# prime-slam/octreelib

Hardware: AMD Instinct MI355X
Metric: Mpoints/s insert+subdivide+RANSAC (higher is better)
Workload: dtype f64; 1 GPU; BASELINE config 3: Grid 1 m voxels, 10000000 planar points per GPU (scene 32x32x32 voxels), insert + subdivide(len>64) + map_leaf_points_cuda_ransac(H=1024, k=6, thr=0.01, poses_per_batch=10) incl. apply_mask; points_per_gpu=10000000, K=64, hypotheses=1024, leaves=575543

## Files before the change

### include/octreelib_hip.h

```cpp
#ifndef OCTREELIB_HIP_H
#define OCTREELIB_HIP_H

#include <stdint.h>

#ifdef __cplusplus
extern "C" {
#endif

#define OCTL_ABI_VERSION 1

enum {
  OCTL_OK = 0,
  OCTL_E_INVALID = -1,
  OCTL_E_HIP = -2,
  OCTL_E_NOMEM = -3,
  OCTL_E_DOMAIN = -4,
  OCTL_E_DEPTH = -5,
  OCTL_E_STATE = -6,
  OCTL_E_COMM = -7
};

typedef struct octl_ctx octl_ctx;
typedef struct octl_forest octl_forest;

// ... 145 lines not shown
                                           const double origin[3], int32_t min_points, double max_variance,
                                           double max_distance, double huber_delta, double* sys_dev,
                                           int64_t* counts_dev, int32_t* node_dev, int32_t* row_dev,
                                           double* residual_dev);
int octl_forest_point_registration_system(octl_forest* f, const double* xyz, int64_t n, const double T[12],
                                          const double origin[3], double max_distance, double huber_delta,
                                          const uint8_t* slot_sel, int32_t n_sel, double sys[28], int64_t counts[2],
                                          int32_t* slot, int64_t* index, double* distance2);
int octl_forest_point_registration_system_device(octl_forest* f, const double* xyz_dev, int64_t n, const double T[12],
                                                 const double origin[3], double max_distance, double huber_delta,
                                                 const uint8_t* slot_sel, int32_t n_sel, double* sys_dev,
                                                 int64_t* counts_dev, int32_t* slot_dev, int64_t* index_dev,
                                                 double* distance2_dev);
int octl_forest_nearest_plane_registration_system(octl_forest* f, const double* xyz, int64_t n, const double T[12],
                                                  const double origin[3], double max_distance, double huber_delta,
                                                  const uint8_t* slot_sel, int32_t n_sel, int32_t min_points,
                                                  double max_variance, double sys[28], int64_t counts[2],
                                                  int32_t* slot, int64_t* index, double* distance2, int32_t* node,
                                                  int32_t* row, double* residual);
int octl_forest_nearest_plane_registration_system_device(octl_forest* f, const double* xyz_dev, int64_t n,
                                                         const double T[12], const double origin[3],
                                                         double max_distance, double huber_delta,
                                                         const uint8_t* slot_sel, int32_t n_sel, int32_t min_points,
                                                         double max_variance, double* sys_dev, int64_t* counts_dev,
                                                         int32_t* slot_dev, int64_t* index_dev, double* distance2_dev,
                                                         int32_t* node_dev, int32_t* row_dev, double* residual_dev);
int octl_forest_adjustment_system(octl_forest* f, const uint8_t* slot_sel, int32_t n_sel, const double* transforms,
                                  const double origin[3], int32_t min_points, int32_t min_poses, double max_variance,
                                  double* sums, int64_t* counts, int64_t n_leaves[2]);
int octl_forest_adjustment_tables(octl_forest* f, int64_t cap_leaves, int32_t* node, int64_t* count, double* mean,
                                  double* normal, double* lambda0, uint8_t* used, int64_t* n_leaves,
                                  int64_t cap_blocks, int32_t* blk_node, int32_t* blk_slot, double* blk_moments,
                                  int64_t* n_blocks);
int octl_forest_transform_poses(octl_forest* f, const uint8_t* slot_sel, int32_t n_sel, const double* transforms);
int octl_forest_remove_poses(octl_forest* f, const uint8_t* slot_sel, int32_t n_sel, int32_t* new_slot,
                             int64_t* n_removed);
int octl_forest_store_size(octl_forest* f, int64_t* n_store, int64_t* n_alive, int32_t* n_poses);
typedef struct {
  int64_t nodes_before, nodes_after, voxels_before, voxels_after, internal_after, collapsed;
} octl_prune_info;
int octl_forest_prune(octl_forest* f, int64_t cap_nodes, int32_t* node_map, int32_t* old_node, octl_prune_info* info);
int octl_debug_sym3_eigen(octl_ctx* ctx, const double* cov6, int64_t n, double* eigval, double* eigvec);


int octl_forest_ransac(octl_forest* f, const int32_t* block_order, int64_t nb,
                       const double* hypotheses, int32_t H, int32_t k, double threshold,
                       float* plane, int32_t* best_count, int32_t* best_index);
int octl_forest_reference_order(octl_forest* f, const int32_t* e0, int32_t n_e0, int64_t cap,
                                int32_t* order, int64_t* n_blocks);
int octl_forest_ransac_all(octl_forest* f, int32_t poses_per_batch, const int32_t* e0,
                           int32_t n_e0, const double* hypotheses, int32_t H, int32_t k,
                           double threshold);
int octl_forest_get_mask(octl_forest* f, int64_t cap, uint8_t* mask, int64_t* n);
int octl_forest_apply_mask(octl_forest* f, int64_t* n_alive);
int octl_forest_apply_mask_async(octl_forest* f);
int octl_forest_settle(octl_forest* f, int64_t* n_alive);
int octl_forest_filter_count(octl_forest* f, const uint8_t* slot_sel, int32_t n_sel, int64_t lo,
                             int64_t hi, int64_t* n_alive);
int octl_forest_apply_host_mask(octl_forest* f, const uint8_t* mask, int64_t n,
                                int64_t* n_alive);


int octl_ransac_evaluate(octl_ctx* ctx, const double* point_cloud, int64_t M,
                         const int32_t* block_sizes, int64_t B, const double* hypotheses,
                         int32_t H, int32_t k, double threshold, uint8_t* mask_out,
                         float* planes_out, int32_t* best_count_out, int32_t* best_index_out);


int32_t octl_voxel_owner(int64_t qx, int64_t qy, int64_t qz, int32_t n_ranks);
#define OCTL_UNIQUE_ID_BYTES 128
int octl_comm_unique_id(uint8_t id[OCTL_UNIQUE_ID_BYTES]);
int octl_comm_init(octl_ctx* ctx, int32_t n_ranks, int32_t rank,
                   const uint8_t id[OCTL_UNIQUE_ID_BYTES]);
int octl_comm_destroy(octl_ctx* ctx);
int octl_route_points(octl_ctx* ctx, const double* xyz_dev, const int64_t* gidx_dev,
                      int64_t n, int64_t index_base, const double corner[3], double L,
                      int64_t* n_recv, int64_t* send_counts );
int octl_forest_add_pose_routed(octl_forest* f, int32_t* slot);
int octl_forest_add_pose_routed_from(octl_forest* f, octl_ctx* route_ctx, int32_t* slot);
int octl_route_get_gidx(octl_ctx* ctx, int64_t cap, int64_t* gidx, int64_t* n);
int octl_debug_host_syncs(uint64_t* count);
int octl_debug_launches(uint64_t* count);
int octl_debug_spec_finish(uint64_t* held, uint64_t* missed);

int octl_debug_route_partition(octl_ctx* ctx, const double* xyz, int64_t n, int64_t index_base,
                               double L, int32_t n_ranks, int64_t* counts, double* xyz_out,
                               int64_t* gidx_out);
int octl_comm_allreduce_i64(octl_ctx* ctx, int64_t* inout_host, int32_t n);

int octl_dev_alloc(octl_ctx* ctx, int64_t bytes, void** dptr);
int octl_dev_free(octl_ctx* ctx, void* dptr);
int octl_dev_upload(octl_ctx* ctx, void* dptr, const void* src, int64_t bytes);
int octl_dev_download(octl_ctx* ctx, void* dst, const void* dptr, int64_t bytes);
int octl_host_alloc(octl_ctx* ctx, int64_t bytes, void** p);
int octl_host_free(octl_ctx* ctx, void* p);
int octl_dev_upload_async(octl_ctx* ctx, void* dptr, const void* src, int64_t bytes);
int octl_ctx_sync_uploads(octl_ctx* ctx);
int octl_dev_copy_bandwidth(octl_ctx* ctx, int64_t bytes, int iters, double* bytes_per_s);

int octl_debug_fail_alloc(int64_t nth, int64_t* seen);

int octl_comm_info(octl_ctx* ctx, int32_t* n_ranks, int32_t* user_rank, int32_t* version);
int octl_device_identity(octl_ctx* ctx, char pci_bus_id[32], uint8_t uuid[16], int32_t* cus);

int octl_debug_set_option(octl_ctx* ctx, const char* name, int64_t value);

int octl_debug_key_geometry(const int32_t tb[6], uint64_t want, int64_t n_alive, uint32_t target, int32_t margin,
                            int32_t bb_out[6], uint32_t* width, uint32_t* n_buckets, int32_t* valid,
                            int64_t* mismatches);

int octl_debug_exclusive_scan(octl_ctx* ctx, const uint32_t* in, int64_t n, uint32_t* out,
                              uint32_t* total);
int octl_debug_radix_sort(octl_ctx* ctx, uint64_t* keys, uint32_t* vals, int64_t n,
                          int key_bits);
int octl_debug_plane_arith(octl_ctx* ctx, const double* num3, const double* den, const double* c,
                           int32_t kdiv, int64_t n, double* q3, double* ck, double* sq);
int octl_debug_plane_arith_certified(octl_ctx* ctx, const double* num3, const double* den, const double* c,
                                     int32_t kdiv, int64_t n, double* q3, double* ck, double* sq);

#ifdef __cplusplus
}
#endif
#endif
```

### octreelib_amd/_native.py

```python

import ctypes as C
import os
import threading

import numpy as np

_LIB_PATH = os.environ.get(
    "OCTREELIB_AMD_LIB",
    os.path.join(os.path.dirname(os.path.abspath(__file__)), "lib", "liboctree_hip.so"),
)

OCTL_OK = 0
OCTL_E_INVALID = -1
OCTL_E_HIP = -2
OCTL_E_NOMEM = -3
OCTL_E_DOMAIN = -4
OCTL_E_DEPTH = -5
OCTL_E_STATE = -6
OCTL_E_COMM = -7
UNIQUE_ID_BYTES = 128


class NativeLibraryError(RuntimeError):
    """liboctree_hip.so is missing / not loadable, or no HIP device is visible."""
# ... 58 lines not shown
    "octl_forest_build": (C.c_int, [_p, _i64, _p, _i32, _i32, _i32, C.POINTER(BuildInfo)]),
    "octl_forest_build_planar": (C.c_int, [_p, _i64, _f64, _i32, _i32, _p, _i32, _i32, C.POINTER(BuildInfo)]),
    "octl_forest_get_split_stats": (C.c_int, [_p, _i64, _p, _p, _pi64]),
    "octl_forest_set_scheme": (C.c_int, [_p, _p, _p, _i64, _i32]),
    "octl_forest_get_nodes": (C.c_int, [_p, _i64, _p, _p, _p, _p, _p, _p, _p, _pi64]),
    "octl_forest_get_voxels": (C.c_int, [_p, _i64, _p, _pi64]),
    "octl_forest_get_blocks": (C.c_int, [_p, _i64, _p, _p, _p, _p, _pi64]),
    "octl_forest_get_slot_voxels": (C.c_int, [_p, _i32, _i64, _p, _pi64]),
    "octl_forest_slot_counts": (C.c_int, [_p, _i32, _pi64, _pi64]),
    "octl_forest_internal_per_voxel": (C.c_int, [_p, _i64, _p, _pi64]),
    "octl_forest_get_perm": (C.c_int, [_p, _i64, _p, _pi64]),
    "octl_forest_get_points": (C.c_int, [_p, _i64, _i64, _p]),
    "octl_forest_gather_blocks": (C.c_int, [_p, _p, _i64, _i64, _p, _pi64]),
    "octl_forest_leaf_stats": (C.c_int, [_p, _p, _i64, _p, _p, _p, _p, _p]),
    "octl_forest_pooled_leaf_stats": (C.c_int, [_p, _p, _i32, _i64, _p, _p, _p, _p, _p, _p, _pi64]),
    "octl_forest_locate": (C.c_int, [_p, _p, _i64, _p]),
    "octl_forest_locate_device": (C.c_int, [_p, _p, _i64, _p]),
    "octl_forest_point_to_plane": (C.c_int, [_p, _p, _i64, _i32, _f64, _p, _p, _p]),
    "octl_forest_point_to_plane_device": (C.c_int, [_p, _p, _i64, _i32, _f64, _p, _p, _p]),
    "octl_forest_nearest": (C.c_int, [_p, _p, _i64, _i32, _f64, _p, _i32, _p, _p, _p, _p]),
    "octl_forest_nearest_device": (C.c_int, [_p, _p, _i64, _i32, _f64, _p, _i32, _p, _p, _p, _p]),
    "octl_forest_raycast": (C.c_int, [_p, _p, _p, _p, _p, _i64, _p, _i32, _i32, _i32, _f64, _p, _p, _p]),
    "octl_forest_raycast_device": (C.c_int, [_p, _p, _p, _p, _p, _i64, _p, _i32, _i32, _i32, _f64, _p, _p, _p]),
    "octl_forest_ray_evidence": (C.c_int, [_p, _p, _p, _p, _p, _p, _i64, _i64, _p, _p, _pi64]),
    "octl_forest_ray_evidence_device": (C.c_int, [_p, _p, _p, _p, _p, _p, _i64, _p, _p, _i64]),
    "octl_forest_carve": (C.c_int, [_p, _p, _p, _i64, _p, _i32, _i64, _i64, _pi64]),
    "octl_forest_carve_device": (C.c_int, [_p, _p, _p, _i64, _p, _i32, _i64, _i64, _pi64]),
    "octl_forest_radius_count": (C.c_int, [_p, _p, _i64, _f64, _i32, _p, _i32, _p]),
    "octl_forest_radius_count_device": (C.c_int, [_p, _p, _i64, _f64, _i32, _p, _i32, _p]),
    "octl_forest_remove_sparse": (C.c_int, [_p, _f64, _i32, _p, _i32, _p, _i32, _pi64]),
    "octl_forest_cell_count": (C.c_int, [_p, _p, _i64, _f64, _i32, _p, _i32, _p]),
    "octl_forest_cell_count_device": (C.c_int, [_p, _p, _i64, _f64, _i32, _p, _i32, _p]),
    "octl_forest_thin": (C.c_int, [_p, _f64, _i32, _p, _i32, _p, _i32, _pi64]),
    "octl_forest_neighbourhood_stats": (C.c_int, [_p, _p, _i64, _f64, _p, _i32, _p, _p, _p, _p, _p]),
    "octl_forest_neighbourhood_stats_device": (C.c_int, [_p, _p, _i64, _f64, _p, _i32, _p, _p, _p, _p, _p]),
    "octl_forest_point_stats": (C.c_int, [_p, _f64, _p, _i32, _p, _i32, _i64, _pi64, _p, _p, _p, _p, _p, _p, _p]),
    "octl_forest_plane_segments": (C.c_int, [_p, _p, _i32, _i32, _f64, _f64, _f64, _i64, _i64, _p, _p, _p, _p, _p, _p,
                                             _p, _p, _p, _pi64, _pi64]),
    "octl_forest_registration_system": (C.c_int, [_p, _p, _i64, _p, _p, _i32, _f64, _f64, _f64, _p, _p, _p, _p, _p]),
    "octl_forest_registration_system_device": (C.c_int,
                                               [_p, _p, _i64, _p, _p, _i32, _f64, _f64, _f64, _p, _p, _p, _p, _p]),
    "octl_forest_point_registration_system": (C.c_int,
                                              [_p, _p, _i64, _p, _p, _f64, _f64, _p, _i32, _p, _p, _p, _p, _p]),
    "octl_forest_point_registration_system_device": (C.c_int,
                                                     [_p, _p, _i64, _p, _p, _f64, _f64, _p, _i32, _p, _p, _p, _p, _p]),
    "octl_forest_nearest_plane_registration_system": (C.c_int,
                                                      [_p, _p, _i64, _p, _p, _f64, _f64, _p, _i32, _i32, _f64, _p, _p,
                                                       _p, _p, _p, _p, _p, _p]),
    "octl_forest_nearest_plane_registration_system_device": (C.c_int,
                                                             [_p, _p, _i64, _p, _p, _f64, _f64, _p, _i32, _i32, _f64,
                                                              _p, _p, _p, _p, _p, _p, _p, _p]),
    "octl_forest_adjustment_system": (C.c_int, [_p, _p, _i32, _p, _p, _i32, _i32, _f64, _p, _p, _p]),
    "octl_forest_adjustment_tables": (C.c_int, [_p, _i64, _p, _p, _p, _p, _p, _p, _pi64, _i64, _p, _p, _p, _pi64]),
    "octl_forest_transform_poses": (C.c_int, [_p, _p, _i32, _p]),
    "octl_forest_remove_poses": (C.c_int, [_p, _p, _i32, _p, _pi64]),
    "octl_forest_store_size": (C.c_int, [_p, _pi64, _pi64, _pi32]),
    "octl_forest_prune": (C.c_int, [_p, _i64, _p, _p, _p]),
    "octl_forest_ransac": (C.c_int, [_p, _p, _i64, _p, _i32, _i32, _f64, _p, _p, _p]),
    "octl_forest_reference_order": (C.c_int, [_p, _p, _i32, _i64, _p, _pi64]),
    "octl_forest_ransac_all": (C.c_int, [_p, _i32, _p, _i32, _p, _i32, _i32, _f64]),
    "octl_forest_get_mask": (C.c_int, [_p, _i64, _p, _pi64]),
    "octl_forest_apply_mask": (C.c_int, [_p, _pi64]),
    "octl_forest_apply_mask_async": (C.c_int, [_p]),
    "octl_forest_settle": (C.c_int, [_p, _pi64]),
    "octl_forest_apply_host_mask": (C.c_int, [_p, _p, _i64, _pi64]),
    "octl_forest_filter_count": (C.c_int, [_p, _p, _i32, _i64, _i64, _pi64]),
    "octl_ransac_evaluate": (
        C.c_int,
        [_p, _p, _i64, _p, _i64, _p, _i32, _i32, _f64, _p, _p, _p, _p],
    ),
    "octl_voxel_owner": (_i32, [_i64, _i64, _i64, _i32]),
    "octl_comm_unique_id": (C.c_int, [_p]),
    "octl_comm_init": (C.c_int, [_p, _i32, _i32, _p]),
    "octl_comm_destroy": (C.c_int, [_p]),
    "octl_comm_info": (C.c_int, [_p, _pi32, _pi32, _pi32]),
    "octl_device_identity": (C.c_int, [_p, C.c_char_p, _p, _pi32]),
    "octl_route_points": (C.c_int, [_p, _p, _p, _i64, _i64, _p, _f64, _pi64, _p]),
    "octl_forest_add_pose_routed": (C.c_int, [_p, _pi32]),
    "octl_forest_add_pose_routed_from": (C.c_int, [_p, _p, _pi32]),
    "octl_debug_route_partition": (C.c_int, [_p, _p, _i64, _i64, C.c_double, C.c_int32, _p, _p, _p]),
    "octl_debug_host_syncs": (C.c_int, [C.POINTER(C.c_uint64)]),
    "octl_debug_launches": (C.c_int, [C.POINTER(C.c_uint64)]),
    "octl_debug_spec_finish": (C.c_int, [C.POINTER(C.c_uint64), C.POINTER(C.c_uint64)]),
    "octl_debug_fail_alloc": (C.c_int, [_i64, _pi64]),
    "octl_debug_set_option": (C.c_int, [_p, C.c_char_p, _i64]),
    "octl_debug_key_geometry": (C.c_int, [_p, C.c_uint64, _i64, C.c_uint32, _i32, _p, _p, _p, _p, _p]),
    "octl_route_get_gidx": (C.c_int, [_p, _i64, _p, _pi64]),
    "octl_comm_allreduce_i64": (C.c_int, [_p, _p, _i32]),
    "octl_dev_alloc": (C.c_int, [_p, _i64, C.POINTER(_p)]),
    "octl_dev_free": (C.c_int, [_p, _p]),
    "octl_dev_upload": (C.c_int, [_p, _p, _p, _i64]),
    "octl_dev_download": (C.c_int, [_p, _p, _p, _i64]),
    "octl_host_alloc": (C.c_int, [_p, _i64, C.POINTER(_p)]),
    "octl_host_free": (C.c_int, [_p, _p]),
    "octl_dev_upload_async": (C.c_int, [_p, _p, _p, _i64]),
    "octl_ctx_sync_uploads": (C.c_int, [_p]),
    "octl_dev_copy_bandwidth": (C.c_int, [_p, _i64, C.c_int, C.POINTER(_f64)]),
    "octl_debug_exclusive_scan": (C.c_int, [_p, _p, _i64, _p, _p]),
    "octl_debug_radix_sort": (C.c_int, [_p, _p, _p, _i64, C.c_int]),
    "octl_debug_plane_arith": (C.c_int, [_p, _p, _p, _p, C.c_int32, _i64, _p, _p, _p]),
    "octl_debug_plane_arith_certified": (C.c_int, [_p, _p, _p, _p, C.c_int32, _i64, _p, _p, _p]),
    "octl_debug_sym3_eigen": (C.c_int, [_p, _p, _i64, _p, _p]),
}

_lib = None
_lib_lock = threading.Lock()


def lib_path() -> str:
    return _LIB_PATH


def load():
    global _lib
    with _lib_lock:
        if _lib is not None:
            return _lib
        if not os.path.exists(_LIB_PATH):
            raise NativeLibraryError(
                f"{_LIB_PATH} is missing: build it with `make` (or __graft_entry__.build()). "
                "octreelib_amd has no CPU fallback."
            )
        try:
            lib = C.CDLL(_LIB_PATH)
        except OSError as e:
            raise NativeLibraryError(f"cannot load {_LIB_PATH}: {e}") from e
        for name, (res, args) in SIGNATURES.items():
            fn = getattr(lib, name)
            fn.restype = res
            fn.argtypes = args
        _lib = lib
        return lib


def ptr(a):
    if a is None:
        return None
    return a.ctypes.data_as(C.c_void_p)


class Context:

    def __init__(self, device: int = 0):
        self.lib = load()
        n = C.c_int(0)
        self.lib.octl_device_count(C.byref(n))
        if n.value <= 0:
            raise NativeLibraryError(
                "no HIP device is visible: octreelib_amd runs on an MI355X only (no CPU fallback)"
            )
        h = C.c_void_p()
        rc = self.lib.octl_ctx_create(int(device), C.byref(h))
        if rc != OCTL_OK or not h.value:
            raise NativeLibraryError(f"octl_ctx_create(device={device}) failed with code {rc}")
        self.handle = h
        self.device = int(device)

    def check(self, rc: int):
        if rc == OCTL_OK:
            return
        msg = self.lib.octl_last_error(self.handle)
        msg = msg.decode("utf-8", "replace") if msg else f"error {rc}"
        if rc == OCTL_E_INVALID:
            raise ValueError(msg)
        if rc == OCTL_E_NOMEM:
            raise MemoryError(msg)
        if rc == OCTL_E_DOMAIN:
            raise DomainError(msg)
        if rc == OCTL_E_DEPTH:
            raise RecursionError(msg)
        raise RuntimeError(msg)

    def sync(self):
        self.check(self.lib.octl_ctx_sync(self.handle))

    def set_option(self, name: str, value=1):
        v = 0 if value is None or value is False else int(value)
        self.check(self.lib.octl_debug_set_option(self.handle, name.encode(), v))
        touched = self.__dict__.setdefault("_options_touched", set())
        touched.add(name)

    def reset_options(self):
        for name in list(self.__dict__.get("_options_touched", ())):
            self.lib.octl_debug_set_option(self.handle, name.encode(), 0)
        self.__dict__["_options_touched"] = set()

    def set_profiling(self, enabled: bool):
        self.check(self.lib.octl_ctx_set_profiling(self.handle, int(enabled)))

    def timings(self):
        cap, stride = 64, 48
        names = C.create_string_buffer(cap * stride)
        ms = (C.c_float * cap)()
        launches = (C.c_int64 * cap)()
        n = C.c_int(0)
        self.check(
            self.lib.octl_ctx_get_timings(
                self.handle, C.cast(names, C.c_void_p), stride, C.cast(ms, C.c_void_p),
                C.cast(launches, C.c_void_p), cap, C.byref(n),
            )
        )
        out = {}
        for i in range(min(n.value, cap)):
            name = names.raw[i * stride : (i + 1) * stride].split(b"\0", 1)[0].decode()
            out[name] = (float(ms[i]), int(launches[i]))
        return out

    def close(self):
        if getattr(self, "handle", None) is not None and self.handle.value:
            self.lib.octl_ctx_destroy(self.handle)
            self.handle = C.c_void_p()

    def __del__(self):
        try:
            self.close()
        except Exception:
            pass


_default_ctx = {}


def default_device() -> int:
    for var in ("OCTREELIB_AMD_DEVICE", "LOCAL_RANK"):
        v = os.environ.get(var)
        if v is not None and v.strip().lstrip("-").isdigit():
            return int(v)
    return 0


_thread_ctx = threading.local()


class use_context:

    def __init__(self, ctx: Context):
        self.ctx = ctx

    def __enter__(self):
        self._prev = getattr(_thread_ctx, "ctx", None)
        _thread_ctx.ctx = self.ctx
        return self.ctx

    def __exit__(self, *exc):
        _thread_ctx.ctx = self._prev


def get_context(device=None) -> Context:
    if device is None:
        ctx = getattr(_thread_ctx, "ctx", None)
        if ctx is not None:
            return ctx
    device = default_device() if device is None else int(device)
    ctx = _default_ctx.get(device)
    if ctx is None:
        ctx = Context(device)
        _default_ctx[device] = ctx
    return ctx


def as_points(points) -> np.ndarray:
    a = np.ascontiguousarray(np.asarray(points, dtype=np.float64))
    if a.size == 0:
        return a.reshape(0, 3)
    if a.ndim != 2 or a.shape[1] != 3:
        raise ValueError(f"expected an (n, 3) point cloud, got shape {a.shape}")
    return a
# ... 12 lines not shown
```

### octreelib_amd/csrc/api.hip

```cpp
#include <unordered_map>

#include "forest.h"

namespace {

__global__ __launch_bounds__(256) void k_slot_counts(const int32_t* __restrict__ blk_slot,
                                                     const int32_t* __restrict__ blk_size, int64_t nb,
                                                     int32_t slot, unsigned long long* __restrict__ out) {
  __shared__ unsigned long long part[2][4];
  unsigned long long pts = 0, lv = 0;
  for (int64_t b = (int64_t)blockIdx.x * blockDim.x + threadIdx.x; b < nb; b += (int64_t)gridDim.x * blockDim.x) {
    if (blk_slot[b] == slot) {
      pts += (unsigned long long)blk_size[b];
      lv += 1;
    }
  }
#pragma unroll
  for (int off = 32; off > 0; off >>= 1) {
    pts += __shfl_xor(pts, off);
    lv += __shfl_xor(lv, off);
  }
  if ((threadIdx.x & 63) == 0) {
    part[0][threadIdx.x >> 6] = pts;
    part[1][threadIdx.x >> 6] = lv;
// ... 35 lines not shown
}


__global__ __launch_bounds__(256) void k_gather_sizes(const int32_t* __restrict__ ids, int64_t m,
                                                      const int32_t* __restrict__ blk_size, uint32_t* __restrict__ out) {
  const int64_t i = (int64_t)blockIdx.x * blockDim.x + threadIdx.x;
  if (i < m) out[i] = (uint32_t)blk_size[ids[i]];
}
__global__ __launch_bounds__(256) void k_gather_rows(const int32_t* __restrict__ ids, int64_t m,
                                                     const uint32_t* __restrict__ blk_start,
                                                     const int32_t* __restrict__ blk_size,
                                                     const uint32_t* __restrict__ offs, const double* __restrict__ xyz,
                                                     double* __restrict__ out) {
  const int64_t i = (int64_t)blockIdx.x * 4 + (threadIdx.x >> 6);
  if (i >= m) return;
  const int32_t b = ids[i];
  const double* src = xyz + 3 * (size_t)blk_start[b];
  double* dst = out + 3 * (size_t)offs[i];
  const int n3 = 3 * blk_size[b];
  for (int j = threadIdx.x & 63; j < n3; j += 64) dst[j] = src[j];
}

}

void forest_reset_scheme(octl_forest* f) {
  forest_forget_pending(f);
  f->max_block_hint = INT64_MAX;
  f->displaced_rows = false;
  f->store_dirty = true;
  f->nodes[0].n = f->nodes[1].n = 0;
  f->cur = 0;
  f->epoch = 0;
  f->built = false;
  f->vkeys.clear();
  f->vkeys_stale = false;
  f->vorg_set = false;
  f->vcode_valid = false;
  f->fast_order_valid = false;
  f->built_store = 0;
  f->built_poses = 0;
  f->append_only = true;
  f->n_voxels = 0;
  f->level_segs.clear();
  f->n_internal = 0;
  f->max_depth_reached = 0;
  f->n_ord = 0;
  f->n_blocks = 0;
  f->mask_valid = false;
  f->split_stats_valid = false;
  forest_contents_changed(f);
}

extern "C" {

int octl_forest_create(octl_ctx* ctx, int mode, const double corner[3], double edge,
                       octl_forest** out) {
  if (!ctx || !out || !corner) return OCTL_E_INVALID;
  *out = nullptr;
  if (mode != 0 && mode != 1) return octl_set_error(ctx, OCTL_E_INVALID, "mode must be 0 or 1");
  if (!(edge > 0.0)) return octl_set_error(ctx, OCTL_E_INVALID, "edge length must be positive");
  if (mode == 0) {
    if (corner[0] != 0.0 || corner[1] != 0.0 || corner[2] != 0.0)
      return octl_set_error(ctx, OCTL_E_INVALID,
                            "a non-zero grid corner is outside the parity domain: the reference "
                            "places its octrees relative to the corner but subtracts absolute "
                            "points (grid.py:96-105 vs octree.py:74)");
    if (edge != (double)(int64_t)edge)
      return octl_set_error(ctx, OCTL_E_INVALID,
                            "voxel_edge_length must be integer valued: the reference truncates "
                            "voxel coordinates with astype(int) (grid.py:72-76)");
  }
  octl_forest* f = new octl_forest();
  f->ctx = ctx;
  f->mode = mode;
  for (int a = 0; a < 3; ++a) f->corner[a] = corner[a];
  f->edge = edge;
  *out = f;
  return OCTL_OK;
}

void octl_forest_destroy(octl_forest* f) {
  if (!f) return;
  forest_forget_pending(f);
  (void)hipSetDevice(f->ctx->device);
  (void)hipStreamSynchronize(f->ctx->stream);
  nodes_free(f->ctx, f->nodes[0]);
  nodes_free(f->ctx, f->nodes[1]);
  if (f->store_borrowed) {
    f->xyz = f->xyz_own;
    f->xyz_own = DevBuf{};
    f->store_borrowed = false;
  }
  for (DevBuf* b :
       {&f->bbox_dev, &f->part_xyz[0], &f->part_xyz[1], &f->bk_table, &f->bk_tot, &f->bk_chunks, &f->bk_vox, &f->bk_node, &f->leafinfo,
        &f->xyz, &f->alive, &f->alive2, &f->ord_idx, &f->xyz_ord, &f->pos_node, &f->blk_node, &f->blk_slot,
        &f->blk_start, &f->blk_size, &f->blk_node2, &f->blk_slot2, &f->blk_start2, &f->blk_size2, &f->mask, &f->blk_eval, &f->rs_scratch, &f->rs_order, &f->fast_order,
        &f->rs_hyp, &f->rs_plane, &f->rs_count, &f->rs_index, &f->ord_idx2, &f->xyz_ord2,
        &f->vkey, &f->path, &f->lin[0], &f->lin[1], &f->val[0], &f->val[1],
        &f->hist, &f->idxbuf[0], &f->idxbuf[1], &f->pathbuf[0], &f->pathbuf[1], &f->flags,
        &f->entries, &f->split[0], &f->split[1], &f->split_tiles[0], &f->split_tiles[1],
        &f->child_sc, &f->pose_off_dev, &f->scheme_dev, &f->root_up, &f->vlin_dev, &f->vcode_dev[0],
        &f->vcode_dev[1], &f->split_lambda, &f->split_n, &f->pl_rows, &f->pl_plane, &f->pl_node_row, &f->grp_scratch,
        &f->pl_hist, &f->q_stage, &f->rg_rows, &f->adj_tab, &f->adj_call, &f->nn_tab, &f->seg_tab, &f->seg_out,
        &f->seg_sort, &f->xf_tab})
    devbuf_release(f->ctx, *b);
  delete f;
}

int octl_forest_clear(octl_forest* f) {
  if (!f) return OCTL_E_INVALID;
  f->bbox_stale = true;
  f->alive_stale = false;
  if (f->store_borrowed) {
    f->xyz = f->xyz_own;
    f->xyz_own = DevBuf{};
    f->store_borrowed = false;
  }
  f->bbox_pending = false;
  f->pose_off.assign(1, 0);
  f->n_store = f->n_alive = 0;
  forest_reset_scheme(f);
  return OCTL_OK;
}

static void forest_drop_scheme(octl_forest* f) {
  f->built = false;
  f->n_ord = 0;
  f->n_blocks = 0;
  f->n_internal = 0;
  f->mask_valid = false;
  f->store_dirty = true;
  f->split_stats_valid = false;
  forest_contents_changed(f);
}

int octl_forest_build(octl_forest* f, int64_t K, const uint8_t* scheme_mask, int32_t n_mask,
                      int32_t keep_scheme, int32_t max_depth, octl_build_info* info) {
  if (!f) return OCTL_E_INVALID;
  OCTL_TRY(forest_settle(f));
  const int64_t nodes_before = f->built ? f->nodes[f->cur].n : -1, voxels_before = f->n_voxels;
  const int rc = forest_build(f, K, scheme_mask, n_mask, keep_scheme, max_depth, info);
  if (rc != OCTL_OK && rc != OCTL_E_INVALID && rc != OCTL_E_STATE) forest_drop_scheme(f);
  if (rc == OCTL_OK && (!keep_scheme || f->nodes[f->cur].n != nodes_before || f->n_voxels != voxels_before))
    f->split_stats_valid = false;
  return rc;
}

int octl_forest_build_planar(octl_forest* f, int64_t K, double max_variance, int32_t min_points, int32_t ddof,
                             const uint8_t* scheme_mask, int32_t n_mask, int32_t max_depth, octl_build_info* info) {
  if (!f) return OCTL_E_INVALID;
  OCTL_TRY(forest_settle(f));
  octl_ctx* ctx = f->ctx;
  if (!(max_variance > 0.0) || !(max_variance <= 1.7976931348623157e308))
    return octl_set_error(ctx, OCTL_E_INVALID, "build_planar: max_variance must be finite and > 0 (got %g)",
                          max_variance);
  if (min_points < 4)
    return octl_set_error(ctx, OCTL_E_INVALID, "build_planar: min_points must be >= 4 (got %d)", min_points);
  if (ddof != 0 && ddof != 1)
    return octl_set_error(ctx, OCTL_E_INVALID, "build_planar: ddof must be 0 or 1 (got %d)", ddof);
  const PlanarRule rule{max_variance, min_points, ddof};
  f->split_stats_valid = false;
  const int rc = forest_build(f, K, scheme_mask, n_mask, 0, max_depth, info, &rule);
  if (rc != OCTL_OK && rc != OCTL_E_INVALID && rc != OCTL_E_STATE) forest_drop_scheme(f);
  return rc;
}

// ... 609 lines not shown
```

### octreelib_amd/csrc/bucket_build.hip

```cpp
#include "build_common.h"
#include "ref_arith.h"
#include "lookback.h"
#include "wave_utils.h"

namespace {

constexpr int PT_THREADS = 256;
constexpr int PT_BITS = 12;
constexpr int PT_BINS = 1 << PT_BITS;

constexpr int BB_THREADS = 512;
constexpr int BB_IPT = 8;
constexpr int BB_WGS = 4;
#define BB_LEAF_UNROLL 2
#define BB_KEEP_ROUNDS 7
constexpr int BB_KEEP = BB_KEEP_ROUNDS < BB_IPT ? BB_KEEP_ROUNDS : BB_IPT;
constexpr int BB_CAP = BB_THREADS * BB_IPT;
static_assert(BB_CAP == 4096, "leaf words, 16-bit item ids and the chunk plan assume 4096 points per piece");
constexpr int BB_LEVELS = 7;
constexpr uint32_t PATH_MASK = 0x1FFFFFu;

enum { BK_NVOX = 0, BK_NINT = 1 , BK_NBLK = 8, BK_ROWS = 9 };
constexpr int LC_DIGIT = 16, LC_DEPTH = 19;
constexpr uint32_t LI_VHEAD = 1u << 24;
// ... 1962 lines not shown
#pragma unroll
      for (int off = 1; off < 64; off <<= 1) {
        const uint32_t t = __shfl_up(inc, off);
        if (tid >= off) inc += t;
      }
      s_hc[tid] = inc - v;
      if (tid == 63) s_hc[64] = inc;
    }
    __syncthreads();
#pragma unroll 2
    for (int r = 0; r < FR; ++r) {
      const int f = r * 256 + tid;
      if (r * 256 >= n) break;
      const unsigned long long bal = s_bal[r * 4 + wave];
      const bool bhead = ((bal >> lane) & 1ull) != 0ull;
      uint32_t size = 0;
      if (bhead) {
        int q = r * 4 + wave;
        unsigned long long rest = bal & ~lt & ~(1ull << lane);
        while (rest == 0ull && ++q < FR * 4) rest = s_bal[q];
        const int next = rest ? q * 64 + (__ffsll((long long)rest) - 1) : n;
        size = (uint32_t)(next - f);
      }
      if (f < n && (bhead || P.write_pos))
        emit(f, leafinfo[(size_t)start + f], bhead, s_hc[r * 4 + wave] + (uint32_t)__popcll(bal & lt), size);
    }
    brun = s_hc[64];
  } else {
    uint32_t open_blk = ~0u, open_pos = 0;
    for (int f0 = 0; f0 < n; f0 += 256) {
      const int f = f0 + tid;
      const uint32_t li = f < n ? leafinfo[(size_t)start + f] : 0u;
      const bool bhead = f < n && (li & LI_BHEAD);
      uint32_t tot;
      const uint32_t pre = block_excl_add(bhead ? 1u : 0u, &tot, s_scr);
      if (bhead) s_hp[pre] = (uint32_t)f;
      if (f < n && (bhead || P.write_pos)) emit(f, li, bhead, brun + pre, ~0u);
      __syncthreads();
      if (tot > 0) {
        if (bhead && pre + 1 < tot) blk_size[bbase + brun + pre] = (int32_t)(s_hp[pre + 1] - (uint32_t)f);
        if (tid == 0 && open_blk != ~0u) blk_size[bbase + open_blk] = (int32_t)(s_hp[0] - open_pos);
        open_blk = brun + tot - 1;
        open_pos = s_hp[tot - 1];
      }
      __syncthreads();
      brun += tot;
    }
    if (tid == 0 && open_blk != ~0u) blk_size[bbase + open_blk] = (int32_t)((uint32_t)n - open_pos);
  }
  BB_STAMP(7);
  if (want_order) {
    __syncthreads();
    for (uint32_t j = tid; j < brun; j += 256) {
      const uint32_t key = s_bkey[j], vox = key >> 13;
      uint32_t lo = j;
      while (lo > 0 && (s_bkey[lo - 1] >> 13) == vox) --lo;
      uint32_t rk = lo;
      for (uint32_t i = lo; i < brun && (s_bkey[i] >> 13) == vox; ++i) rk += s_bkey[i] < key ? 1u : 0u;
      P.order_out[bbase + rk] = (int32_t)(bbase + j);
    }
  }
  BB_STAMP(8);
  pre_vox += nvox;
  pre_blk += cko.y ? nblk_piece : brun;
#pragma unroll
  for (int l = 0; l < BB_LEVELS; ++l) pre_lvl[l] += lvl_cnt[l];
  __syncthreads();
  }
}

#define OCTL_PT_IPT 8
#define OCTL_PT_WGS 2
constexpr int PT_IPT = OCTL_PT_IPT;
constexpr int PT_TILE = PT_THREADS * PT_IPT;

int domain_error(octl_ctx* ctx) {
  return octl_set_error(ctx, OCTL_E_DOMAIN,
                        "a point has a non-finite coordinate or a top-level voxel index outside +-%d", OCTL_VOX_ABS_LIMIT);
}
uint32_t supertiles(octl_ctx* ctx, int64_t items, int wgs, int* tiles) {
  *tiles = (int)std::min<int64_t>(16, std::max<int64_t>(1, ceil_div(ceil_div(items, PT_TILE), (int64_t)octl_ctx_cus(ctx) * wgs)));
  return (uint32_t)ceil_div(items, (int64_t)*tiles * PT_TILE);
}
int part_table_reserve(octl_forest* f, size_t cells, size_t tail_words, size_t* elems) {
  *elems = (cells + 1 + 15) & ~(size_t)15;
  return devbuf_reserve(f->ctx, f->bk_table, (2 * *elems + tail_words + 16) * 4);
}
bool tables_fused(const octl_ctx* ctx, uint32_t nst) { return !ctx->opt.no_fused_tables && nst <= TS_MAX_ROWS; }

struct PartPass {
  const PartRec* recs = nullptr;
  int64_t n = 0;
  const uint8_t* alive = nullptr;
  const uint8_t* scheme = nullptr;
  LinParams lp;
  GeomDev* gdev = nullptr;
  int validate = 0;
  const GeomAsk* ask = nullptr;
  int32_t* bad_flag = nullptr;
  uint32_t nst = 0, nd = 0;
  int tiles = 1;
  size_t tab_elems = 0;
  bool own_scan = false;
  PartRec* out = nullptr;
  const char *t_hist = nullptr, *t_scan = nullptr, *t_scatter = nullptr;
};

hipError_t transpose_u32(hipStream_t st, const uint32_t* in, uint32_t R, uint32_t Cc, uint32_t* out) {
  OCTL_LAUNCH(k_transpose_u32, dim3((Cc + 63) / 64, (R + 63) / 64), dim3(256), 0, st, in, R, Cc, out);
  return hipGetLastError();
}

int partition_scan(octl_forest* f, const PartPass& p, bool fused) {
  octl_ctx* ctx = f->ctx;
  uint32_t *table = f->bk_table.as<uint32_t>(), *table_dm = table + p.tab_elems;
  if (fused) {
    const unsigned g = (p.nd + TS_COLS - 1) / TS_COLS;
    uint64_t* status = nullptr;
    uint32_t epoch = 0;
    OCTL_TRY(octl_scan_status_acquire(ctx, g, &status, &epoch));
    OCTL_LAUNCH(k_table_scan, dim3(g), dim3(TS_THREADS), 0, ctx->stream, table, p.nst, p.nd, table_dm, status, epoch,
                       p.validate, p.ask ? (const int32_t*)f->bbox_dev.as<int32_t>() : (const int32_t*)nullptr,
                       p.ask ? *p.ask : GeomAsk{0, 0, 0, 0}, p.lp, p.gdev);
    HIP_TRY(ctx, hipGetLastError());
  } else {
    HIP_TRY(ctx, transpose_u32(ctx->stream, table, p.nst, p.nd, table_dm));
    OCTL_TRY(octl_exclusive_scan_u32(ctx, table_dm, table_dm, (int64_t)p.nd * p.nst, nullptr));
    HIP_TRY(ctx, transpose_u32(ctx->stream, table_dm, p.nd, p.nst, table));
  }
  return OCTL_OK;
}

int partition_pass(octl_forest* f, const PartPass& p, const uint32_t** bstart, uint32_t* bstride) {
  octl_ctx* ctx = f->ctx;
  hipStream_t st = ctx->stream;
  const uint32_t nst = p.nst, nd = p.nd;
  const bool fused = tables_fused(ctx, nst);
  uint32_t *table = f->bk_table.as<uint32_t>(), *table_dm = table + p.tab_elems;
  const int32_t* bbox = p.ask ? (const int32_t*)f->bbox_dev.as<int32_t>() : nullptr;
  {
    KTimer t(ctx, p.t_hist);
    if (p.recs) {
      OCTL_LAUNCH(k_part_hist_rec, dim3(nst), dim3(PH_THREADS), 0, st, (const uint4*)p.recs, p.n, p.lp,
                         (const GeomDev*)p.gdev, nst, nd, (int64_t)p.tiles * PT_TILE, table);
    } else {
      const bool lone = f->edge == 1.0;
      auto kh = p.validate ? (lone ? k_part_hist<true, true> : k_part_hist<true, false>)
                           : (lone ? k_part_hist<false, true> : k_part_hist<false, false>);
      OCTL_LAUNCH(kh, dim3(nst), dim3(PH_THREADS), 0, st, (const double*)f->xyz.as<double>(), p.alive, p.n, p.lp,
                         (const GeomDev*)p.gdev, nst, nd, (int64_t)p.tiles * PT_TILE, table,
                         p.validate ? f->bbox_dev.as<int32_t>() : p.bad_flag);
    }
    HIP_TRY(ctx, hipGetLastError());
    if (p.validate) {
      f->bbox_pending = false;
      if (fused) {
      } else if (p.validate == 1)
        OCTL_LAUNCH(k_geom_validate, dim3(1), dim3(64), 0, st, bbox, *p.ask, p.lp, p.gdev);
      else
        OCTL_LAUNCH(k_geom_validate2, dim3(1), dim3(64), 0, st, bbox, *p.ask, p.gdev);
      HIP_TRY(ctx, hipGetLastError());
    }
    if (!p.t_scan) OCTL_TRY(partition_scan(f, p, fused));
  }
  if (p.t_scan && !p.own_scan) {
    KTimer t(ctx, p.t_scan);
    OCTL_TRY(partition_scan(f, p, fused));
  }
  {
    KTimer t(ctx, p.t_scatter);
    ScatterOwnScan own;
    std::memset(&own, 0, sizeof(own));
    if (p.own_scan) own = ScatterOwnScan{table_dm, p.validate, bbox, *p.ask, p.lp, p.gdev};
    if (!p.recs) {
      auto ks = p.own_scan ? k_part_scatter<PT_IPT, false, 8, true>
                           : (nd <= 256u ? k_part_scatter<PT_IPT, false, 8> : k_part_scatter<PT_IPT, false, PT_BITS>);
      OCTL_LAUNCH(ks, dim3(nst), dim3(PT_THREADS), 0, st, (const double*)f->xyz.as<double>(), p.alive, p.n, p.lp,
                         (const GeomDev*)p.gdev, nst, nd, p.tiles, (const uint32_t*)table,
                         (const int64_t*)f->pose_off_dev.as<int64_t>(), (int)f->pose_off.size() - 1, p.scheme, p.out, own);
    } else {
      auto ks = nd <= 256u ? k_part_scatter<PT_IPT, true, 8> : k_part_scatter<PT_IPT, true, PT_BITS>;
      OCTL_LAUNCH(ks, dim3(nst), dim3(PT_THREADS), 0, st, (const double*)p.recs, (const uint8_t*)nullptr, p.n, p.lp,
                         (const GeomDev*)p.gdev, nst, nd, p.tiles, (const uint32_t*)table, (const int64_t*)nullptr, 0,
                         (const uint8_t*)nullptr, p.out, own);
    }
    HIP_TRY(ctx, hipGetLastError());
  }
  *bstart = table_dm;
  *bstride = fused ? 1u : nst;
  return OCTL_OK;
}

enum BuildVerdict { BV_GO, BV_GENERAL, BV_AGAIN_ASYNC, BV_AGAIN_HOST };

struct BucketBuild {
  octl_forest* f;
  octl_ctx* ctx;
  hipStream_t st;
  uint32_t* small;
  GeomAsk ask;
  bool async_geom;
  bool hinted;
  bool hinted2;
  GeomDev hint;
  int bb[6], tb[6];
  uint64_t ny, nz;
  int s, bits_a;
  uint32_t nb, nd_a, nd_b, nst_a, nst_b;
  int tiles_a, tiles_b;
  bool two_pass;
  LinParams lp, lp_pass1;
  size_t tab_elems;
  GeomDev* gdev;
  const PartRec* recs;
  const uint32_t* bstart;
  uint32_t bstride;
  uint32_t *bk_tot, *bk_scan, *ck_tot;
  ChunkDesc* ck_desc;
  uint2* ck_of_bucket;
  BkParams bp;
  NodeParams np;
  bool chunks_beside;
  bool spec_want, spec_own_scan, spec_order, spec_launched;
  int64_t spec_node_cap, spec_vox_cap, spec_blk_cap;
  uint32_t sm[64];
};
int mirror_words(const BucketBuild& b) {
  static_assert(SM_GEOM == 64, "the geometry record is read back together with the 64 scalars in front of it");
  return (int)(64 + (b.gdev ? sizeof(GeomDev) / 4 : 0));
}

bool hint_load(const octl_ctx* ctx, const octl_forest* f, uint64_t want, GeomDev* hint) {
  std::memcpy(hint, ctx->geom_hint, sizeof(*hint));
  return ctx->geom_hint_valid && ctx->geom_hint_want == want && hint->lp.mode == f->mode && hint->lp.L == f->edge &&
         hint->lp.c0x == f->corner[0] && hint->lp.c0y == f->corner[1] && hint->lp.c0z == f->corner[2] &&
         !ctx->opt.no_geom_hint && hint->lp.exact_digits == (ctx->opt.no_exact_digits ? 0 : 1);
}
void hint_store(octl_ctx* ctx, const GeomDev& g, bool two_pass, uint64_t want) {
  static_assert(sizeof(GeomDev) <= sizeof(octl_ctx::geom_hint), "hint storage");
  std::memset(ctx->geom_hint, 0, sizeof(ctx->geom_hint));
  std::memcpy(ctx->geom_hint, &g, sizeof(g));
  ctx->geom_hint_valid = g.valid != 0;
  ctx->geom_hint_two_pass = two_pass;
  ctx->geom_hint_want = want;
}
int geom_read(octl_ctx* ctx, GeomDev* g, BuildVerdict* v) {
  std::memcpy(g, static_cast<char*>(ctx->small_host) + SM_GEOM * 4, sizeof(*g));
  *v = BV_GO;
  if (g->valid) return OCTL_OK;
  if (g->reason == GEOM_DOMAIN) return domain_error(ctx);
  *v = g->reason == GEOM_EMPTY ? BV_GENERAL : (g->reason == GEOM_REHASH ? BV_AGAIN_ASYNC : BV_AGAIN_HOST);
  return OCTL_OK;
}

int plan_geometry(BucketBuild& b, bool force_sync, BuildVerdict* v) {
  octl_forest* f = b.f;
  octl_ctx* ctx = b.ctx;
  const int64_t n_alive = f->n_alive;
  *v = BV_GO;
  const uint64_t target = ctx->opt.bucket_points > 0 ? (uint64_t)ctx->opt.bucket_points
                                                     : (n_alive <= 400000 ? 1280 : 2560);
  uint64_t want = 1;
  while (want < ((uint64_t)PT_BINS << PT_BITS) && want * target < (uint64_t)n_alive) want <<= 1;
  b.async_geom = !force_sync && !ctx->geom_sparse && want <= (uint64_t)PT_BINS && !ctx->opt.sync_geom;
  const int margin = f->mode != 0 ? 0
                                  : (ctx->opt.geom_margin == 0 ? 1 : (int)std::min<int64_t>(64, std::max<int64_t>(0, ctx->opt.geom_margin)));
  b.ask = GeomAsk{want, n_alive, (uint32_t)target, margin};
  if (f->bbox_pending) {
    const bool usable = hint_load(ctx, f, want, &b.hint);
    b.hinted = b.async_geom && usable && !ctx->geom_hint_two_pass;
    b.hinted2 = !b.async_geom && !force_sync && usable && ctx->geom_hint_two_pass && f->mode == 0;
    if (!b.hinted && !b.hinted2) OCTL_TRY(store_compute_bbox(f));
  }
  if (f->n_alive != f->n_store) OCTL_TRY(alive_ensure(f));
  b.ny = b.nz = 1;
  b.nb = b.async_geom ? (uint32_t)geom_bucket_cap(want) : (uint32_t)PT_BINS;
  if (!b.async_geom) {
    int *bb = b.bb, *tb = b.tb;
    *v = BV_GENERAL;
    if (b.hinted2) {
      std::memcpy(bb, b.hint.bb, sizeof(b.bb));
      std::memcpy(tb, b.hint.tb, sizeof(b.tb));
    } else {
      int32_t* bbox_host = reinterpret_cast<int32_t*>(static_cast<char*>(ctx->small_host) + MIRROR_BBOX_WORD * 4);
      HIP_TRY(ctx, hipMemcpyAsync(bbox_host, f->bbox_dev.p, 32, hipMemcpyDeviceToHost, b.st));
      HIP_TRY(ctx, hipStreamSynchronize(b.st));
      std::memcpy(tb, bbox_host, sizeof(b.tb));
      if (bbox_host[6]) return domain_error(ctx);
      if (tb[0] > tb[3]) return OCTL_OK;
      geom_pad_box(tb, margin, bb);
    }
    if (bb[0] > bb[3]) return OCTL_OK;
    const uint64_t nx = (uint64_t)(bb[3] - bb[0] + 1);
    b.ny = (uint64_t)(bb[4] - bb[1] + 1);
    b.nz = (uint64_t)(bb[5] - bb[2] + 1);
    if (nx * b.ny > (1ull << 32) || nx * b.ny * b.nz >= (1ull << 32)) return OCTL_OK;
    const uint64_t R = nx * b.ny * b.nz;
    const uint64_t Rt = (uint64_t)((int64_t)tb[3] - tb[0] + 1) * (uint64_t)((int64_t)tb[4] - tb[1] + 1) *
                        (uint64_t)((int64_t)tb[5] - tb[2] + 1);
    b.s = std::min(12, std::max(0, geom_ceil_log2(Rt) - geom_ceil_log2(want)));
    if (((R - 1) >> b.s) + 1 > ((uint64_t)PT_BINS << PT_BITS)) return OCTL_OK;
    b.nb = (uint32_t)(((R - 1) >> b.s) + 1);
    b.two_pass = b.nb > (uint32_t)PT_BINS;
    if (b.hinted2 && !b.two_pass) {
      *v = BV_AGAIN_HOST;
      return OCTL_OK;
    }
    ctx->geom_sparse = ((Rt - 1) >> b.s) + 1 > (uint64_t)PT_BINS && want <= (uint64_t)PT_BINS;
    if (b.two_pass && (uint64_t)f->n_alive * 2 < (uint64_t)b.nb * target) return OCTL_OK;
    *v = BV_GO;
  }
  const int wgs = b.two_pass ? std::max(OCTL_PT_WGS, 3) : OCTL_PT_WGS;
  b.nst_a = supertiles(ctx, f->n_store, wgs, &b.tiles_a);
  b.nst_b = b.two_pass ? supertiles(ctx, n_alive, wgs, &b.tiles_b) : 0;
  b.bits_a = b.two_pass ? std::min(PT_BITS, (geom_ceil_log2(b.nb) + 1) / 2) : 0;
  b.nd_a = b.two_pass ? (1u << b.bits_a) : b.nb;
  b.nd_b = b.two_pass ? ((b.nb - 1) >> b.bits_a) + 1 : 0;
  LinParams& lp = b.lp;
  lp.mode = f->mode, lp.L = f->edge;
  lp.c0x = f->corner[0], lp.c0y = f->corner[1], lp.c0z = f->corner[2];
  lp.minx = b.bb[0], lp.miny = b.bb[1], lp.minz = b.bb[2];
  lp.ny = (uint32_t)b.ny, lp.nz = (uint32_t)b.nz;
  lp.shift = lp.dshift = b.s;
  lp.dmask = b.two_pass ? (b.nd_a - 1u) : 0xFFFFFFFFu, lp.raw_vp = b.two_pass ? 1 : 0;
  lp.exact_digits = ctx->opt.no_exact_digits ? 0 : 1;
  lp.width = 1u << b.s;
  lp.winv = lp.whalf = 0.0;
  b.lp_pass1 = lp;
  return OCTL_OK;
}

int partition(BucketBuild& b, const BucketBuildArgs& a) {
  octl_forest* f = b.f;
  octl_ctx* ctx = b.ctx;
  const int64_t n_alive = f->n_alive;
  OCTL_TRY(devbuf_reserve(ctx, f->part_xyz[0], (size_t)n_alive * sizeof(PartRec)));
  if (b.two_pass) OCTL_TRY(devbuf_reserve(ctx, f->part_xyz[1], (size_t)n_alive * sizeof(PartRec)));
  OCTL_TRY(part_table_reserve(f, std::max((size_t)b.nd_a * b.nst_a, (size_t)b.nd_b * b.nst_b),
                              b.two_pass ? b.nb + 1 : 0, &b.tab_elems));
  const size_t tot_elems = (((size_t)BK_ROWS * b.nb + 8) + 15) & ~(size_t)15;
  OCTL_TRY(devbuf_reserve(ctx, f->bk_tot, 2 * tot_elems * 4));
  const std::pair<DevBuf*, int> per_point[] = {
      {&f->bk_vox, 12},  {&f->bk_node, 12}, {&f->leafinfo, 4}, {&f->ord_idx, 4},   {&f->xyz_ord, 24},
      {&f->pos_node, 4}, {&f->blk_node, 4}, {&f->blk_slot, 4}, {&f->blk_start, 4}, {&f->blk_size, 4}};
  for (const auto& pp : per_point) OCTL_TRY(devbuf_reserve(ctx, *pp.first, (size_t)n_alive * pp.second));
  b.bk_tot = f->bk_tot.as<uint32_t>();
  b.bk_scan = b.bk_tot + tot_elems;
  if (b.async_geom || b.hinted2) b.gdev = reinterpret_cast<GeomDev*>(b.small + SM_GEOM);
  if (b.async_geom) {
    if (b.hinted) {
      if (!ctx->geom_hint_staged) OCTL_LAUNCH(k_geom_set, dim3(1), dim3(64), 0, b.st, b.hint, b.gdev);
    } else {
      OCTL_LAUNCH(k_bucket_geom, dim3(1), dim3(64), 0, b.st, (const int32_t*)f->bbox_dev.as<int32_t>(), b.ask, b.lp,
                         b.gdev);
    }
    HIP_TRY(ctx, hipGetLastError());
  } else if (b.hinted2) {
    GeomDev g2;
    std::memset(&g2, 0, sizeof(g2));
    g2.lp = b.lp_pass1;
    std::memcpy(g2.bb, b.bb, sizeof(b.bb));
    std::memcpy(g2.tb, b.tb, sizeof(b.tb));
    g2.valid = 1;
    OCTL_LAUNCH(k_geom_set, dim3(1), dim3(64), 0, b.st, g2, b.gdev);
    HIP_TRY(ctx, hipGetLastError());
  }
  PartPass p;
  p.n = f->n_store;
  p.alive = f->n_alive == f->n_store ? nullptr : f->alive.as<uint8_t>();
  p.scheme = a.scheme_dev;
  p.lp = b.lp, p.gdev = b.gdev, p.ask = &b.ask;
  p.validate = b.hinted ? 1 : (b.hinted2 ? 2 : 0);
  p.nst = b.nst_a, p.nd = b.nd_a, p.tiles = b.tiles_a, p.tab_elems = b.tab_elems;
  p.own_scan = tables_fused(ctx, b.nst_a) && !b.two_pass && !b.hinted2 && b.nd_a <= 256u && b.nst_a <= PS_OWN_MAX_ROWS;
  p.out = f->part_xyz[0].as<PartRec>();
  p.t_hist = "part_hist", p.t_scan = "part_scan", p.t_scatter = "part_scatter";
  OCTL_TRY(partition_pass(f, p, &b.bstart, &b.bstride));
  b.recs = p.out;
  if (!b.two_pass) return OCTL_OK;
  b.lp.dshift = b.s + b.bits_a, b.lp.dmask = 0xFFFFFFFFu, b.lp.raw_vp = 0;
  p.recs = b.recs, p.n = n_alive;
  p.alive = p.scheme = nullptr;
  p.lp = b.lp;
  p.validate = 0, p.own_scan = false;
  p.nst = b.nst_b, p.nd = b.nd_b, p.tiles = b.tiles_b;
  p.out = f->part_xyz[1].as<PartRec>();
  OCTL_TRY(partition_pass(f, p, &b.bstart, &b.bstride));
  uint32_t* bounds = f->bk_table.as<uint32_t>() + 2 * b.tab_elems;
  KTimer t(ctx, "bucket_bounds");
  OCTL_LAUNCH(k_bucket_bounds, dim3((unsigned)ceil_div((int64_t)b.nb + 1, 256)), dim3(256), 0, b.st,
                     (const uint4*)f->part_xyz[1].as<uint4>(), (uint32_t)n_alive, b.lp, (const GeomDev*)b.gdev, b.nb, bounds);
  HIP_TRY(ctx, hipGetLastError());
  b.recs = p.out, b.bstart = bounds, b.bstride = 1;
  return OCTL_OK;
}

int launch_chunks(BucketBuild& b, hipStream_t on) {
  octl_forest* f = b.f;
  OCTL_LAUNCH(k_bucket_plan, dim3(b.nb), dim3(BB_THREADS), 0, on, b.recs, b.bstart, b.bp, (const GeomDev*)b.gdev,
                     b.ck_desc, b.ck_of_bucket, b.bk_tot, b.small);
  HIP_TRY(b.ctx, hipGetLastError());
  OCTL_LAUNCH(k_bucket_chunks, dim3((unsigned)std::min<int64_t>(2 * (int64_t)octl_ctx_cus(b.ctx), CK_CAP)),
                     dim3(BB_THREADS), 0, on, b.recs, b.bstart, b.bp, (const GeomDev*)b.gdev,
                     (const ChunkDesc*)b.ck_desc, b.ck_tot, (const int64_t*)f->pose_off_dev.as<int64_t>(),
                     f->ord_idx.as<uint32_t>(), f->xyz_ord.as<double>(), f->leafinfo.as<uint32_t>(),
                     f->bk_vox.as<uint32_t>(), f->bk_node.as<uint32_t>(), b.bk_tot, b.small);
  HIP_TRY(b.ctx, hipGetLastError());
  return OCTL_OK;
}

int build_buckets(BucketBuild& b, const BucketBuildArgs& a) {
  octl_forest* f = b.f;
  octl_ctx* ctx = b.ctx;
  b.bp = BkParams{b.lp, a.K, b.bstride, b.nb, (uint32_t)f->n_alive, (int)f->pose_off.size() - 1, a.scheme_dev ? 0 : 1};
  const size_t ck_off_tot = (size_t)CK_CAP * sizeof(ChunkDesc);
  const size_t ck_off_bkt = ck_off_tot + (size_t)CK_CAP * BK_ROWS * 4;
  OCTL_TRY(devbuf_reserve(ctx, f->bk_chunks, ck_off_bkt + (size_t)b.nb * 8 + 16));
  b.ck_desc = reinterpret_cast<ChunkDesc*>(f->bk_chunks.p);
  b.ck_tot = reinterpret_cast<uint32_t*>(static_cast<char*>(f->bk_chunks.p) + ck_off_tot);
  b.ck_of_bucket = reinterpret_cast<uint2*>(static_cast<char*>(f->bk_chunks.p) + ck_off_bkt);
  b.chunks_beside = ctx->had_chunks;
  {
    KTimer t(ctx, "bucket_build");
    hipStream_t side = b.st;
    bool on_side = false;
    if (b.chunks_beside && octl_ctx_side_stream(ctx) && hipEventRecord(ctx->self_gate, b.st) == hipSuccess &&
        hipStreamWaitEvent(ctx->self_stream, ctx->self_gate, 0) == hipSuccess) {
      side = ctx->self_stream;
      on_side = true;
    }
    if (b.chunks_beside) OCTL_TRY(launch_chunks(b, side));
    OCTL_LAUNCH(k_bucket_build, dim3(b.nb), dim3(BB_THREADS), 0, b.st, b.recs, b.bstart, b.bp, (const GeomDev*)b.gdev,
                       (const int64_t*)f->pose_off_dev.as<int64_t>(), f->ord_idx.as<uint32_t>(), f->xyz_ord.as<double>(),
                       f->leafinfo.as<uint32_t>(), f->bk_vox.as<uint32_t>(), f->bk_node.as<uint32_t>(), b.bk_tot, b.small,
                       b.chunks_beside ? 0 : 1);
    HIP_TRY(ctx, hipGetLastError());
    if (on_side) {
      HIP_TRY(ctx, hipEventRecord(ctx->self_done, side));
      HIP_TRY(ctx, hipStreamWaitEvent(b.st, ctx->self_done, 0));
    }
  }
  NodeParams& np = b.np;
  np.lp = b.lp;
  np.bstride = b.bstride, np.nb = b.nb, np.n_alive = (uint32_t)f->n_alive;
  np.n_poses = b.bp.n_poses, np.all_scheme = b.bp.all_scheme, np.cur_epoch = a.cur_epoch;
  np.old_fc = a.old_fc, np.old_epoch = a.old_epoch, np.old_vcode = a.old_vcode, np.old_voxels = a.old_voxels;
  b.spec_order = np.n_poses == 1 && !ctx->opt.no_fast_order;
  b.spec_want = b.async_geom && b.gdev && !a.old_fc && !a.old_vcode && ctx->spec_nodes > 0 && !ctx->opt.no_spec_finish;
  b.spec_own_scan = b.spec_want && !ctx->opt.no_fused_tables && (uint32_t)BK_ROWS * b.nb <= (uint32_t)BF_SCAN_MAX;
  return OCTL_OK;
}

int launch_finish(const BucketBuild& b, NodeTable& nt, const NodeParams& np, bool with_chunk_map, uint32_t own_scan_seq) {
  octl_forest* f = b.f;
  KTimer t(b.ctx, "bucket_nodes");
  const size_t lds = own_scan_seq ? ((size_t)BK_ROWS * b.nb + 1) * 4 : 0;
  auto kern = own_scan_seq ? k_bucket_finish<true> : k_bucket_finish<false>;
  OCTL_LAUNCH(kern, dim3(b.nb), dim3(256), lds, b.st, node_ptrs(nt), np, b.bstart,
                     (const uint32_t*)b.bk_scan, (const uint32_t*)(b.small + SM_BK_TOTAL),
                     (const uint32_t*)f->leafinfo.as<uint32_t>(), (const uint32_t*)f->ord_idx.as<uint32_t>(),
// ... 73 lines not shown
    std::memset(&g, 0, sizeof(g));
    g.lp = b.lp_pass1;
    geom_pad_box(b.tb, b.ask.margin, g.bb);
    std::memcpy(g.tb, b.tb, sizeof(b.tb));
    g.valid = 1;
    hint_store(ctx, g, true, b.ask.want);
  }
  if (b.async_geom) {
    OCTL_TRY(geom_read(ctx, &g, v));
    if (*v != BV_GO) return OCTL_OK;
    GeomDev nh;
    geom_from_box(g.tb, false, b.ask, b.lp, nh);
    hint_store(ctx, nh, false, b.ask.want);
    b.lp = g.lp;
    std::memcpy(b.bb, g.bb, sizeof(b.bb));
    std::memcpy(b.tb, g.tb, sizeof(b.tb));
    b.ny = b.lp.ny, b.nz = b.lp.nz;
  }
  return OCTL_OK;
}

int finish_and_commit(BucketBuild& b, const BucketBuildArgs& a, NodeTable& nt, bool overfull, BucketBuildResult* r) {
  octl_forest* f = b.f;
  octl_ctx* ctx = b.ctx;
  const uint32_t* sm = b.sm;
  if (sm[SM_BK_FLAGS]) return OCTL_OK;
  const int64_t V = sm[SM_NVOX];
  int64_t n_int = 0;
  int depth = 0;
  r->segs.assign(1, octl_forest::LevelSeg{0, V, 0});
  for (int l = 0; l < BB_LEVELS; ++l) {
    if (sm[SM_BK_LEVEL + l] == 0) break;
    n_int += sm[SM_BK_LEVEL + l];
    depth = l + 1;
    r->segs.push_back(octl_forest::LevelSeg{V + 8 * (n_int - (int64_t)sm[SM_BK_LEVEL + l]), V + 8 * n_int, l + 1});
  }
  if (depth > a.max_depth) return octl_set_error(ctx, OCTL_E_DEPTH, "maximum depth %d exceeded", a.max_depth);
  const int64_t total = V + 8 * n_int;
  if (total >= ((int64_t)1 << 31)) return octl_set_error(ctx, OCTL_E_NOMEM, "more than 2^31 scheme nodes");
  const bool fast_order = b.np.n_poses == 1 && !a.old_fc && sm[SM_BK_TODO] == 0 && sm[SM_BK_NOORDER] == 0 &&
                          !ctx->opt.no_fast_order;
  const bool spec_held = b.spec_launched && sm[SM_BK_TODO] == 0 && sm[SM_BK_NOORDER] == 0 &&
                         (b.chunks_beside || !overfull) && V <= b.spec_vox_cap &&
                         (int64_t)sm[SM_NBLOCKS] <= b.spec_blk_cap && total <= b.spec_node_cap;
  ctx->spec_points = f->n_alive, ctx->spec_nodes = total, ctx->spec_vox = V, ctx->spec_blocks = sm[SM_NBLOCKS];
  if (b.spec_launched) (spec_held ? g_octl_spec_held : g_octl_spec_missed).fetch_add(1, std::memory_order_relaxed);
  if (!spec_held) {
    OCTL_TRY(nodes_reserve(ctx, nt, total));
    OCTL_TRY(devbuf_reserve(ctx, f->vlin_dev, (size_t)std::max<int64_t>(V, 1) * 8));
    NodeParams& np = b.np;
    np.lp = b.lp, np.node_cap = nt.cap, np.org = f->vorg;
    np.write_pos = sm[SM_BK_TODO] > 0;
    np.order_out = nullptr;
    if (fast_order) {
      OCTL_TRY(devbuf_reserve(ctx, f->fast_order, (size_t)std::max<uint32_t>(sm[SM_NBLOCKS], 1) * 4));
      np.order_out = f->fast_order.as<int32_t>();
    }
    OCTL_TRY(launch_finish(b, nt, np, overfull || b.chunks_beside, 0));
  }
  if (a.old_vcode && a.old_voxels > 0) {
    HIP_TRY(ctx, hipMemsetAsync(b.small + SM_BK_MISSING, 0, 4, b.st));
    OCTL_LAUNCH(k_old_voxels_missing, dim3((unsigned)ceil_div(a.old_voxels, 256)), dim3(256), 0, b.st,
                       a.old_vcode, a.old_voxels, (const uint64_t*)f->vlin_dev.as<uint64_t>(), V, b.lp,
                       b.bb[3] - b.bb[0] + 1, f->vorg, b.small + SM_BK_MISSING);
    HIP_TRY(ctx, hipGetLastError());
    uint32_t missing = 0;
    OCTL_TRY(octl_readback(ctx, b.small + SM_BK_MISSING, 1, &missing));
    if (missing) return OCTL_OK;
  }
  nt.n = total;
  r->n_internal = n_int, r->levels = depth, r->n_voxels = V;
  r->n_blocks = sm[SM_NBLOCKS], r->pending = sm[SM_BK_TODO];
  for (int k = 0; k < 3; ++k) r->geom.min[k] = b.bb[k];
  r->geom.ny = b.ny, r->geom.nz = b.nz, r->geom.order_done = fast_order;
  r->done = 1;
  return OCTL_OK;
}

}

int forest_bucket_build(octl_forest* f, const BucketBuildArgs& a, NodeTable& nt, BucketBuildResult* r) {
  octl_ctx* ctx = f->ctx;
  r->done = 0;
  if (f->n_alive <= 0 || !f->bbox_dev.p || ctx->opt.no_bucket_build) return OCTL_OK;
  if (f->mode == 1 && f->n_alive > 65535) return OCTL_OK;
  bool force_sync = false;
  for (int attempt = 0; attempt < 4; ++attempt) {
    BucketBuild b{f, ctx, ctx->stream, ctx->small.as<uint32_t>()};
    BuildVerdict v = BV_GO;
    OCTL_TRY(plan_geometry(b, force_sync, &v));
    if (v == BV_AGAIN_HOST) {
      force_sync = true;
      continue;
    }
    if (v != BV_GO) return OCTL_OK;
    OCTL_TRY(partition(b, a));
    OCTL_TRY(build_buckets(b, a));
    OCTL_TRY(scan_totals(b, nt, b.spec_want));
    OCTL_TRY(interpret_geometry(b, &v));
    if (v == BV_AGAIN_ASYNC || v == BV_AGAIN_HOST) {
      force_sync = v == BV_AGAIN_HOST;
      continue;
    }
    if (v != BV_GO) return OCTL_OK;
    if (f->mode == 0) OCTL_TRY(forest_fix_origin(f, b.tb));
    const bool overfull = b.sm[SM_BK_OVERFULL] > 0;
    if (overfull && !b.chunks_beside && !b.sm[SM_BK_FLAGS]) {
      {
        KTimer t(ctx, "bucket_build");
        OCTL_TRY(launch_chunks(b, ctx->stream));
      }
      OCTL_TRY(scan_totals(b, nt, false));
    }
    ctx->had_chunks = overfull;
    return finish_and_commit(b, a, nt, overfull, r);
  }
  return octl_set_error(ctx, OCTL_E_STATE, "bucket build: the geometry retries do not terminate");
}

int forest_prefix_partition(octl_forest* f, int pm, const void** recs_out, const uint32_t** bstart, uint32_t* bstride,
                            const uint32_t** bad_flag) {
  octl_ctx* ctx = f->ctx;
  const int64_t N = f->n_store;
  PartPass p;
  LinParams& lp = p.lp;
  std::memset(&lp, 0, sizeof(lp));
  lp.mode = 2, lp.pm = pm, lp.L = f->edge;
  lp.c0x = f->corner[0], lp.c0y = f->corner[1], lp.c0z = f->corner[2];
  lp.ny = lp.nz = 1;
  lp.dmask = 0xFFFFFFFFu;
  lp.exact_digits = ctx->opt.no_exact_digits ? 0 : 1;
  p.n = N, p.nd = 1u << (3 * pm);
  p.nst = supertiles(ctx, N, OCTL_PT_WGS, &p.tiles);
  OCTL_TRY(devbuf_reserve(ctx, f->part_xyz[0], (size_t)N * sizeof(PartRec)));
  OCTL_TRY(part_table_reserve(f, (size_t)p.nd * p.nst, 0, &p.tab_elems));
  uint32_t* flag = f->bk_table.as<uint32_t>() + 2 * p.tab_elems;
  HIP_TRY(ctx, hipMemsetAsync(flag, 0, 4, ctx->stream));
  p.bad_flag = reinterpret_cast<int32_t*>(flag);
  p.out = f->part_xyz[0].as<PartRec>();
  p.t_hist = "prefix_hist", p.t_scatter = "prefix_scatter";
  OCTL_TRY(partition_pass(f, p, bstart, bstride));
  *recs_out = f->part_xyz[0].p;
  *bad_flag = flag;
  return OCTL_OK;
}

#ifdef BB_STAMPS
extern "C" int octl_debug_bb_stamps(octl_ctx* ctx, unsigned long long out[16], int reset) {
  if (!ctx || !out) return OCTL_E_INVALID;
  HIP_TRY(ctx, hipStreamSynchronize(ctx->stream));
  HIP_TRY(ctx, hipMemcpyFromSymbol(out, HIP_SYMBOL(g_bb_stamps), sizeof(unsigned long long) * 16));
  if (reset) {
    unsigned long long z[16] = {0};
    HIP_TRY(ctx, hipMemcpyToSymbol(HIP_SYMBOL(g_bb_stamps), z, sizeof(z)));
  }
  return OCTL_OK;
}
#endif


extern "C" int octl_debug_key_geometry(const int32_t tb[6], uint64_t want, int64_t n_alive, uint32_t target,
                                       int32_t margin, int32_t bb_out[6], uint32_t* width, uint32_t* n_buckets,
                                       int32_t* valid, int64_t* mismatches) {
  if (!tb || !bb_out || !width || !n_buckets || !valid || !mismatches || margin < 0 || margin > 64)
    return OCTL_E_INVALID;
  GeomAsk ask;
  ask.want = want;
  ask.n_alive = n_alive;
  ask.target = target;
  ask.margin = margin;
  LinParams base;
  std::memset(&base, 0, sizeof(base));
  base.L = 1.0;
  GeomDev g;
  geom_from_box(tb, false, ask, base, g);
  for (int a = 0; a < 6; ++a) bb_out[a] = g.bb[a];
  *valid = g.valid ? 1 : -(int32_t)g.reason;
  *width = 0;
  *n_buckets = 0;
  *mismatches = 0;
  if (!g.valid) return OCTL_OK;
  const uint64_t R = (uint64_t)(g.bb[3] - g.bb[0] + 1) * (uint64_t)(g.bb[4] - g.bb[1] + 1) * (uint64_t)(g.bb[5] - g.bb[2] + 1);
  *width = g.lp.width;
  *n_buckets = (uint32_t)((R + g.lp.width - 1) / g.lp.width);
  int64_t bad = 0;
  for (uint64_t lin = 0; lin < R; ++lin)
    bad += (uint32_t)std::fma((double)lin, g.lp.winv, g.lp.whalf) != (uint32_t)(lin / g.lp.width);
  *mismatches = bad;
  return OCTL_OK;
}
```

### octreelib_amd/csrc/build.hip

```cpp
#include <algorithm>
#include <chrono>
#include <cstdlib>

#include "build_common.h"
#include "forest.h"
#include "ref_arith.h"
#include "wave_utils.h"

struct BuildTrace {
  bool on = false;
  std::chrono::steady_clock::time_point t = std::chrono::steady_clock::now();
  void mark(const char* what) {
    if (!on) return;
    const auto now = std::chrono::steady_clock::now();
    fprintf(stderr, "[build] %-28s %8.3f ms\n", what, std::chrono::duration<double, std::milli>(now - t).count());
    t = now;
  }
};

namespace {

constexpr int LV_THREADS = 256;
constexpr int LV_WAVES = LV_THREADS / 64;
#ifndef OCTL_LV_IPT
// ... 1164 lines not shown
  return OCTL_OK;
}

int forest_fix_origin(octl_forest* f, const int bb[6]) {
  if (f->mode != 0 || bb[0] > bb[3]) return OCTL_OK;
  if (!f->vorg_set) {
    f->vorg.x = bb[0];
    f->vorg.y = bb[1];
    f->vorg.z = bb[2];
    f->vorg_set = true;
  }
  if (!vkey_in_window(bb[0], bb[1], bb[2], f->vorg) || !vkey_in_window(bb[3], bb[4], bb[5], f->vorg))
    return octl_set_error(f->ctx, OCTL_E_DOMAIN,
                          "the scene has moved more than %d voxels away from where it started (voxel box "
                          "[%d..%d] x [%d..%d] x [%d..%d], origin %d %d %d): the packed voxel keys cannot hold it",
                          OCTL_VOX_BIAS, bb[0], bb[3], bb[1], bb[4], bb[2], bb[5], f->vorg.x, f->vorg.y, f->vorg.z);
  return OCTL_OK;
}

static int forest_ensure_origin(octl_forest* f) {
  if (f->mode != 0 || f->vorg_set || f->n_store == 0) return OCTL_OK;
  octl_ctx* ctx = f->ctx;
  if (f->bbox_pending) OCTL_TRY(store_compute_bbox(f));
  if (!f->bbox_dev.p) return OCTL_OK;
  int32_t* host = reinterpret_cast<int32_t*>(static_cast<char*>(ctx->small_host) + MIRROR_BBOX_WORD * 4);
  HIP_TRY(ctx, hipMemcpyAsync(host, f->bbox_dev.p, 32, hipMemcpyDeviceToHost, ctx->stream));
  HIP_TRY(ctx, hipStreamSynchronize(ctx->stream));
  int bb[6];
  std::memcpy(bb, host, sizeof(bb));
  if (host[6]) return OCTL_OK;
  return forest_fix_origin(f, bb);
}

namespace {

struct BuildRequest {
  int64_t K;
  int keep_scheme;
  int max_depth;
  const PlanarRule* planar;
  bool all_scheme;
  const uint8_t* scheme_dev;
  int n_poses;
  int64_t N;
  int64_t n_alive;
  int cur_epoch;
};

struct BuildOutcome {
  NodeTable* nt = nullptr;
  int64_t n_voxels = 0, n_internal = 0, n_blocks = 0;
  int levels = 0;
  std::vector<octl_forest::LevelSeg> segs;
  bool blocks_made = false;
  bool fresh_keys = false;
  int vl_min[3] = {0, 0, 0};
  uint64_t vl_ny = 1, vl_nz = 1;
  std::vector<uint64_t> new_vkeys;
  bool uniform_epoch = true;
  bool fast_order_valid = false;
  int64_t max_block_hint = INT64_MAX;
  bool publish_split_stats = false;
};

int build_validate(octl_forest* f, const BuildRequest& rq, const uint8_t* scheme_mask, int32_t n_mask) {
  octl_ctx* ctx = f->ctx;
  if (rq.N >= ((int64_t)1 << 31))
    return octl_set_error(ctx, OCTL_E_INVALID, "more than 2^31-1 points in one forest");
  if (rq.keep_scheme && !f->built)
    return octl_set_error(ctx, OCTL_E_STATE, "keep_scheme build without a previous scheme");
  if (rq.keep_scheme && rq.planar) return octl_set_error(ctx, OCTL_E_INVALID, "a planar build makes its own scheme");
  if (scheme_mask && n_mask != rq.n_poses)
    return octl_set_error(ctx, OCTL_E_INVALID, "scheme mask has %d entries for %d poses", n_mask,
                          rq.n_poses);
  if (f->displaced_rows && !rq.keep_scheme)
    return octl_set_error(ctx, OCTL_E_DOMAIN,
                          "map_leaf_points left points outside the cube of their leaf: the reference keeps them "
                          "there and raises IndexError when such a leaf is subdivided (octree.py:94-98)");
  return OCTL_OK;
}

int build_begin(octl_forest* f, BuildRequest& rq, const uint8_t* scheme_mask) {
  octl_ctx* ctx = f->ctx;
  hipStream_t st = ctx->stream;
  const int n_poses = rq.n_poses;
  {
    uint32_t init[32];
    std::memset(init, 0, sizeof(init));
    int* bb = reinterpret_cast<int*>(init + SM_BBOX);
    bb[0] = bb[1] = bb[2] = 1 << 30;
    bb[3] = bb[4] = bb[5] = -(1 << 30);
    std::memcpy(ctx->small_host, init, sizeof(init));
    int hint_words = 0;
    ctx->geom_hint_staged = false;
    if (f->bbox_pending && !rq.keep_scheme && ctx->geom_hint_valid && !ctx->geom_hint_two_pass &&
        !ctx->opt.no_geom_hint) {
      static_assert(sizeof(ctx->geom_hint) == 192, "hint words");
      std::memcpy(static_cast<char*>(ctx->small_host) + SM_GEOM * 4, ctx->geom_hint, sizeof(ctx->geom_hint));
      hint_words = (int)(sizeof(ctx->geom_hint) / 4);
      ctx->geom_hint_staged = true;
    }
    int32_t* box = nullptr;
    if (f->bbox_pending && f->bbox_stale && f->bbox_dev.p) {
      box = f->bbox_dev.as<int32_t>();
      f->bbox_stale = false;
    }
    OCTL_LAUNCH(k_build_begin, dim3(1), dim3(128), 0, st, static_cast<const uint32_t*>(ctx->small_host),
                       ctx->small.as<uint32_t>(), hint_words, box);
    HIP_TRY(ctx, hipGetLastError());
  }

  {
    const void* before = f->pose_off_dev.p;
    OCTL_TRY(devbuf_reserve(ctx, f->pose_off_dev, (size_t)(n_poses + 1) * 8));
    if (f->pose_off_dev.p != before) f->pose_off_uploaded.clear();
  }
  rq.scheme_dev = nullptr;
  const size_t off_bytes = (size_t)(n_poses + 1) * 8;
  const bool fits = off_bytes + (size_t)n_poses <= OCTL_PINNED_BYTES / 2;
  char* pin = static_cast<char*>(ctx->pinned);
  const void* src_off = f->pose_off.data();
  if (fits) {
    std::memcpy(pin, f->pose_off.data(), off_bytes);
    src_off = pin;
  }
  if (f->pose_off_uploaded != f->pose_off) {
    if (fits)
      OCTL_TRY(octl_copy_from_pinned(ctx, f->pose_off_dev.p, src_off, off_bytes));
    else
      HIP_TRY(ctx, hipMemcpyAsync(f->pose_off_dev.p, src_off, off_bytes, hipMemcpyHostToDevice, st));
    f->pose_off_uploaded = f->pose_off;
  }
  if (!rq.all_scheme) {
    OCTL_TRY(devbuf_reserve(ctx, f->scheme_dev, (size_t)n_poses));
    const void* src_m = scheme_mask;
    if (fits) {
      std::memcpy(pin + off_bytes, scheme_mask, (size_t)n_poses);
      src_m = pin + off_bytes;
    }
    HIP_TRY(ctx, hipMemcpyAsync(f->scheme_dev.p, src_m, (size_t)n_poses, hipMemcpyHostToDevice, st));
    rq.scheme_dev = f->scheme_dev.as<uint8_t>();
  }
  if (!fits) HIP_TRY(ctx, hipStreamSynchronize(st));
  return OCTL_OK;
}

int build_try_incremental(octl_forest* f, const BuildRequest& rq, BuildTrace& trace, octl_build_info* info, int* done) {
  *done = 0;
  const bool unsplit_again = !rq.keep_scheme && !rq.planar && rq.K < 0 && f->built && f->n_internal == 0;
  if (!rq.keep_scheme && !unsplit_again) return OCTL_OK;
  OCTL_TRY(forest_insert_incremental(f, done, info));
  trace.mark("incremental insertion");
  if (*done) {
    if (unsplit_again) f->epoch += 1;
    return OCTL_OK;
  }
  if (f->displaced_rows)
    return octl_set_error(f->ctx, OCTL_E_DOMAIN,
                          "map_leaf_points left points outside the cube of their leaf and the stored poses have "
                          "to be placed again (a pose was extended or the scheme replaced since): the points "
                          "cannot be kept in their leaves, as the reference does (octree.py:114-123)");
  return OCTL_OK;
}

int build_block_table(octl_forest* f, int64_t n_alive, int64_t* n_blocks) {
  const int64_t n_ord_before = f->n_ord;
  f->n_ord = n_alive;
  OCTL_TRY(forest_make_blocks(f));
  uint32_t e = 0;
  OCTL_TRY(forest_finish_blocks(f, &e));
  *n_blocks = f->n_blocks;
  if (e) {
    f->n_ord = n_ord_before;
    f->n_blocks = 0;
    f->built = false;
    return octl_set_error(f->ctx, OCTL_E_DOMAIN,
                          "a point lies outside the cube of a node that is being subdivided "
                          "(the reference raises IndexError or picks a wrong child here)");
  }
  return OCTL_OK;
}

int build_commit(octl_forest* f, const BuildRequest& rq, BuildOutcome& o, octl_build_info* info) {
  octl_ctx* ctx = f->ctx;
  NodeTable& nt = *o.nt;
  f->cur ^= 1;
  f->n_voxels = o.n_voxels;
  if (o.fresh_keys) {
    f->vkeys.clear();
    f->vkeys_stale = true;
    f->vl_min[0] = o.vl_min[0]; f->vl_min[1] = o.vl_min[1]; f->vl_min[2] = o.vl_min[2];
    f->vl_ny = o.vl_ny;
    f->vl_nz = o.vl_nz;
  } else {
    f->vkeys.swap(o.new_vkeys);
    f->vkeys_stale = false;
  }
  f->level_segs.swap(o.segs);
  f->built = true;
  f->epoch = rq.cur_epoch;
  f->n_ord = rq.n_alive;
  f->n_blocks = o.n_blocks;
  f->n_internal = o.n_internal;
  f->uniform_epoch = o.uniform_epoch;
  f->max_depth_reached = o.levels;
  f->mask_valid = false;
  f->store_dirty = false;
  f->vcode_valid = false;
  f->fast_order_valid = o.fast_order_valid;
  f->max_block_hint = o.max_block_hint;
  f->built_store = f->n_store;
  f->built_poses = rq.n_poses;
  f->append_only = true;
  if (o.publish_split_stats) {
    OCTL_TRY(devbuf_reserve(ctx, f->split_n, (size_t)std::max<int64_t>(nt.n, 1) * 4));
    if (nt.n > 0)
      HIP_TRY(ctx, hipMemcpyAsync(f->split_n.p, nt.scount.p, (size_t)nt.n * 4, hipMemcpyDeviceToDevice, ctx->stream));
    f->split_stats_nodes = nt.n;
    f->split_stats_valid = true;
  }
  if (info) {
    info->n_points = rq.n_alive;
    info->n_voxels = o.n_voxels;
    info->n_nodes = nt.n;
    info->n_internal = o.n_internal;
    info->n_blocks = o.n_blocks;
    info->max_depth = o.levels;
    info->n_levels = o.levels;
  }
  return OCTL_OK;
}


// ... 388 lines not shown
int general_level_loop(octl_forest* f, const BuildRequest& rq, GeneralBuild& g, BuildOutcome& o) {
  NodeTable& old = f->nodes[f->cur];
  const int32_t* old_fc = g.have_old ? old.first_child.as<int32_t>() : nullptr;
  const int32_t* old_epoch = g.have_old ? old.epoch.as<int32_t>() : nullptr;
  o.segs = {{0, g.V, 0}};
  LevelLoop L{f, g.nt, rq.K, (int)rq.keep_scheme, rq.all_scheme, rq.scheme_dev, old_fc, old_epoch, rq.cur_epoch,
              rq.max_depth, rq.n_alive, false, 0, g.V, 0, 0, &o.segs};
  L.planar = rq.planar;
  if (g.pm) {
    for (int d = 1; d <= g.pm; ++d) o.segs.push_back({top_base(d), top_base(d + 1), d});
    L.first_new = top_base(g.pm);
    L.n_new = (int64_t)1 << (3 * g.pm);
    L.n_internal = top_base(g.pm);
    L.level = g.pm;
    L.gx = static_cast<const double*>(g.pre_recs);
    L.xs = PART_REC_DOUBLES;
  }
  OCTL_TRY(run_level_loop(L));
  o.n_internal = L.n_internal;
  o.levels = L.level;
  return OCTL_OK;
}

int general_finalize(octl_forest* f, const BuildRequest& rq, GeneralBuild& g) {
  octl_ctx* ctx = f->ctx;
  hipStream_t st = ctx->stream;
  const int64_t n_alive = rq.n_alive;
  if (n_alive <= 0) return OCTL_OK;
  NodePtrs nd = node_ptrs(*g.nt);
  OCTL_TRY(devbuf_reserve(ctx, f->ord_idx, (size_t)n_alive * 4));
  OCTL_TRY(devbuf_reserve(ctx, f->xyz_ord, (size_t)n_alive * 24));
  KTimer t(ctx, "finalize");
  if (g.pm)
    OCTL_LAUNCH(k_finalize_rec, dim3(grid_for(n_alive)), dim3(256), 0, st,
                       (const int32_t*)g.pos_node, (const int32_t*)nd.depth,
                       (const uint32_t*)f->idxbuf[0].as<uint32_t>(),
                       (const uint32_t*)f->idxbuf[1].as<uint32_t>(), static_cast<const uint4*>(g.pre_recs),
                       n_alive, f->ord_idx.as<uint32_t>(), f->xyz_ord.as<double>());
  else
    OCTL_LAUNCH(k_finalize, dim3(grid_for(n_alive)), dim3(256), 0, st,
                       (const int32_t*)g.pos_node, (const int32_t*)nd.depth,
                       (const uint32_t*)f->idxbuf[0].as<uint32_t>(),
                       (const uint32_t*)f->idxbuf[1].as<uint32_t>(),
                       (const double*)f->xyz.as<double>(), n_alive, f->ord_idx.as<uint32_t>(),
                       f->xyz_ord.as<double>());
  HIP_TRY(ctx, hipGetLastError());
  return OCTL_OK;
}

int build_general_route(octl_forest* f, const BuildRequest& rq, BuildTrace& trace, BuildOutcome& o) {
  OCTL_TRY(forest_sync_vkeys(f));
  trace.mark("sync_vkeys");
  GeneralBuild g;
  OCTL_TRY(general_keys(f, rq, g));
  trace.mark("keys + bbox readback");
  OCTL_TRY(general_sort(f, rq, g));
  trace.mark("sort (enqueue)");
  OCTL_TRY(general_roots(f, rq, g, trace));
  const int64_t old_internal = g.have_old ? f->n_internal : 0;
  OCTL_TRY(general_level0(f, rq, g));
  trace.mark("level-0 buffers");
  OCTL_TRY(general_level_loop(f, rq, g, o));
  trace.mark("level loop");
  OCTL_TRY(general_finalize(f, rq, g));
  trace.mark("finalize (enqueue)");
  o.nt = g.nt;
  o.n_voxels = g.V;
  o.blocks_made = false;
  o.fresh_keys = g.fresh;
  if (g.fresh) {
    o.vl_min[0] = g.bb[0]; o.vl_min[1] = g.bb[1]; o.vl_min[2] = g.bb[2];
    o.vl_ny = g.ny;
    o.vl_nz = g.nz;
  } else {
    o.new_vkeys.swap(g.new_vkeys);
  }
  o.uniform_epoch = rq.keep_scheme ? f->uniform_epoch : !(g.have_old && old_internal > 0);
  o.fast_order_valid = false;
  o.max_block_hint = INT64_MAX;
  o.publish_split_stats = rq.planar != nullptr;
  return OCTL_OK;
}

}

int forest_build(octl_forest* f, int64_t K, const uint8_t* scheme_mask, int32_t n_mask,
                 int32_t keep_scheme, int32_t max_depth, octl_build_info* info, const PlanarRule* planar) {
  octl_ctx* ctx = f->ctx;
  HIP_TRY(ctx, hipSetDevice(ctx->device));
  BuildRequest rq{};
  rq.K = K;
  rq.keep_scheme = keep_scheme;
  rq.max_depth = max_depth <= 0 ? 63 : max_depth;
  rq.planar = planar;
  rq.N = f->n_store;
  rq.n_poses = (int)f->pose_off.size() - 1;
  OCTL_TRY(build_validate(f, rq, scheme_mask, n_mask));
  rq.all_scheme = true;
  if (scheme_mask && !keep_scheme)
    for (int p = 0; p < rq.n_poses; ++p) rq.all_scheme = rq.all_scheme && scheme_mask[p];
  f->fast_order_valid = false;
  forest_contents_changed(f);
  f->max_block_hint = INT64_MAX;
  BuildTrace trace;
  trace.on = ctx->opt.trace_build != 0;

  OCTL_TRY(build_begin(f, rq, scheme_mask));
  int placed = 0;
  OCTL_TRY(build_try_incremental(f, rq, trace, info, &placed));
  if (placed) return OCTL_OK;
  rq.n_alive = f->n_alive;
  rq.cur_epoch = f->epoch + (keep_scheme ? 0 : 1);

  BuildOutcome out;
  bool bucket_built = false;
  OCTL_TRY(build_bucket_route(f, rq, trace, out, &bucket_built));
  if (!bucket_built) OCTL_TRY(build_general_route(f, rq, trace, out));
  if (!out.blocks_made) OCTL_TRY(build_block_table(f, rq.n_alive, &out.n_blocks));
  if (!bucket_built) trace.mark("blocks + final sync");
  return build_commit(f, rq, out, info);
}
```

### octreelib_amd/csrc/build_common.h

```cpp
#pragma once
#include "forest.h"

constexpr uint32_t IDX_MASK = 0x7FFFFFFFu;

struct NodePtrs {
  uint32_t *start, *count, *scount;
  int32_t *depth, *voxel, *parent, *first_child, *old_id, *epoch;
  double *corner, *edge;
};

static inline NodePtrs node_ptrs(NodeTable& t) {
  NodePtrs p;
  p.start = t.start.as<uint32_t>();
  p.count = t.count.as<uint32_t>();
  p.scount = t.scount.as<uint32_t>();
  p.depth = t.depth.as<int32_t>();
  p.voxel = t.voxel.as<int32_t>();
  p.parent = t.parent.as<int32_t>();
  p.first_child = t.first_child.as<int32_t>();
  p.old_id = t.old_id.as<int32_t>();
  p.epoch = t.epoch.as<int32_t>();
  p.corner = t.corner.as<double>();
  p.edge = t.edge.as<double>();
  return p;
}

struct BucketBuildArgs {
  int64_t K;
  const uint8_t* scheme_dev;
  int cur_epoch;
  int max_depth;
  const int32_t* old_fc = nullptr;
  const int32_t* old_epoch = nullptr;
  const uint64_t* old_vcode = nullptr;
  int64_t old_voxels = 0;
};
struct BucketBuildGeom {
  int min[3];
  uint64_t ny, nz;
  bool order_done = false;
};
struct BucketBuildResult {
  int done = 0;
  std::vector<octl_forest::LevelSeg> segs;
  int64_t n_internal = 0;
  int levels = 0;
  int64_t n_voxels = 0, n_blocks = 0;
  int64_t pending = 0;
  BucketBuildGeom geom;
};
int forest_bucket_build(octl_forest* f, const BucketBuildArgs& a, NodeTable& nt, BucketBuildResult* r);

constexpr int PART_REC_BYTES = 32;
constexpr int PART_REC_QUADS = PART_REC_BYTES / 16;
constexpr int PART_REC_DOUBLES = PART_REC_BYTES / 8;
constexpr int PART_REC_VP_WORD = 6;
constexpr int PART_REC_IDX_WORD = 7;
constexpr int PART_VP_DIGITS = 6;
constexpr int PART_VP_DIGIT_BITS = 3 * PART_VP_DIGITS;
constexpr int PART_VP_DIGIT_SHIFT = 1;
constexpr uint32_t PART_VP_DIGIT_MASK = (1u << PART_VP_DIGIT_BITS) - 1u;
constexpr uint32_t PART_VP_BAD = 1u;
int forest_prefix_partition(octl_forest* f, int pm, const void** recs_out, const uint32_t** bstart, uint32_t* bstride,
                            const uint32_t** bad_flag);
```

### octreelib_amd/csrc/common.h

```cpp
#pragma once

#include <hip/hip_runtime.h>
#include <stdint.h>

#include <cstdio>
#include <cstring>
#include <map>
#include <string>
#include <vector>

#include "../../include/octreelib_hip.h"

#include <atomic>
extern std::atomic<uint64_t> g_octl_host_syncs;
static inline hipError_t octl_counted_stream_sync(hipStream_t s) {
  g_octl_host_syncs.fetch_add(1, std::memory_order_relaxed);
  return hipStreamSynchronize(s);
}
static inline hipError_t octl_counted_event_sync(hipEvent_t e) {
  g_octl_host_syncs.fetch_add(1, std::memory_order_relaxed);
  return hipEventSynchronize(e);
}
#define hipStreamSynchronize(s) octl_counted_stream_sync(s)
#define hipEventSynchronize(e) octl_counted_event_sync(e)
extern std::atomic<uint64_t> g_octl_launches;
extern std::atomic<uint64_t> g_octl_spec_held, g_octl_spec_missed;
#define OCTL_LAUNCH(...)                                                      \
  do {                                                                        \
    g_octl_launches.fetch_add(1, std::memory_order_relaxed);                  \
    hipLaunchKernelGGL(__VA_ARGS__);                                          \
  } while (0)
#define hipMemsetAsync(...) (g_octl_launches.fetch_add(1, std::memory_order_relaxed), hipMemsetAsync(__VA_ARGS__))

#if !defined(OCTL_EXPERIMENTS) && \
    (defined(PS_DUP_KEYS) || defined(PS_DUP_STORE) || defined(RS_COUNTS) || defined(BB_STAMPS))
#error "PS_DUP_* / RS_COUNTS / BB_STAMPS are experiments: build them with tools/build_variant.sh (-DOCTL_EXPERIMENTS)"
#endif

#define OCTL_WAVE 64
#define OCTL_PINNED_BYTES (256 * 1024)

struct KernelTiming {
  double ms = 0.0;
  int64_t launches = 0;
};

struct PendingEvent {
  std::string name;
  hipEvent_t start, stop;
};

struct DevBuf {
  void* p = nullptr;
  size_t cap = 0;
  template <typename T>
  T* as() const {
    return reinterpret_cast<T*>(p);
  }
};

struct OctlOptions {
  int64_t no_bucket_build = 0;
  int64_t bucket_points = 0;
  int64_t sync_geom = 0;
  int64_t no_geom_hint = 0;
  int64_t no_exact_digits = 0;
  int64_t no_fast_order = 0;
  int64_t no_bucket_history = 0;
  int64_t no_cube_fast = 0;
  int64_t no_cube_prefix = 0;
  int64_t cube_prefix_min = 0;
  int64_t no_incremental = 0;
  int64_t route_self_sendrecv = 0;
  int64_t trace_build = 0;
  int64_t scan_mode = 0;
  int64_t no_fused_tables = 0;
  int64_t no_spin_wait = 0;
  int64_t ransac_waves = 0;
  int64_t geom_margin = 0;
  int64_t no_ransac_prescreen = 0;
  int64_t no_spec_finish = 0;
};
int64_t* octl_option_field(OctlOptions& o, const char* name);

struct octl_ctx {
  int device = 0;
  OctlOptions opt;
  hipStream_t stream = nullptr;
  std::string err;
  int profiling = 0;
  std::map<std::string, KernelTiming> timings;
  std::vector<PendingEvent> pending;
  std::vector<hipEvent_t> event_pool;
  DevBuf scan_tmp[3];
  DevBuf scan_status;
  uint32_t scan_epoch = 0;
  int cus = 0;
  DevBuf small;
  void* small_host = nullptr;
  void* pinned = nullptr;
  hipEvent_t pin_event[3] = {nullptr, nullptr, nullptr};
  hipEvent_t handoff_event = nullptr;
  hipStream_t copy_stream = nullptr;
  hipEvent_t copy_gate = nullptr;
  hipStream_t self_stream = nullptr;
  hipEvent_t self_gate = nullptr, self_done = nullptr;
  struct Upload { const char* dst; size_t bytes; hipEvent_t done; };
  std::vector<Upload> uploads;
  std::vector<DevBuf> pool;
  size_t pool_bytes = 0;
  std::map<void*, size_t> user_blocks;
  unsigned char geom_hint[192] = {0};
  bool geom_hint_valid = false;
  bool geom_hint_staged = false;
  struct octl_forest* pending_mask_forest = nullptr;
  uint64_t geom_hint_want = 0;
  bool geom_hint_two_pass = false;
  bool geom_sparse = false;
  bool had_chunks = false;
  int64_t spec_points = 0, spec_nodes = 0, spec_vox = 0, spec_blocks = 0;
  DevBuf hyp_dev;
  DevBuf f32_stage;
  DevBuf xf_stage;
  std::vector<char> xf_host;
  hipEvent_t xf_event = nullptr;
  bool xf_inflight = false;
  DevBuf ls_buf;
  DevBuf rs_counters;
  int rs_parity = 0;
  uint32_t wait_seq = 0;
  bool rs_counters_dirty = false;
  std::vector<double> hyp_host;
  void* comm = nullptr;
  int n_ranks = 1, rank = 0;
  DevBuf routed_xyz, routed_gidx;
  bool routed_taken = false;
  DevBuf rt_hist, rt_counts, rt_matrix, rt_send_xyz, rt_send_gidx;
  int64_t routed_n = 0;
};

int octl_set_error(octl_ctx* ctx, int code, const char* fmt, ...);
enum { MIRROR_COPY_WORDS = 512, MIRROR_BBOX_WORD = 896, MIRROR_RS_VIOLATION = 990, MIRROR_MASK_TOTALS = 992,
       MIRROR_FLAG_BUILD = 1000, MIRROR_FLAG_MASK0 = 1001, MIRROR_FLAG_MASK1 = 1002 };
static_assert(MIRROR_COPY_WORDS <= MIRROR_BBOX_WORD && MIRROR_BBOX_WORD + 8 <= MIRROR_RS_VIOLATION &&
              MIRROR_RS_VIOLATION < MIRROR_MASK_TOTALS &&
              MIRROR_MASK_TOTALS + 2 <= MIRROR_FLAG_BUILD && MIRROR_FLAG_MASK1 < 1024, "mirror layout");
enum {
  SM_ERR = 0,
  SM_BBOX = 4,
  SM_NVOX = 12,
  SM_NSPLIT = 13,
  SM_NTILES = 14,
  SM_ETOTAL = 15,
  SM_NBLOCKS = 16,
  SM_BK_TICKET = 17,
  SM_BK_OVERFULL = 18,
  SM_SLOT_VOXELS = 21,
  SM_MASK_TOTAL = 22,
  SM_BK_NOORDER = 23,
  SM_DEBUG_TOTAL = 24,
  SM_BK_FLAGS = 25,
  SM_BK_TOTAL = 26,
  SM_BK_TODO = 27,
  SM_BK_MISSING = 28,
  SM_CK_COUNT = 29,
  SM_INC_MISS = 28,
  SM_INC_BAD = 29,
  SM_INC_DEAD = 30,
  SM_INC_NEWVOX = 31,
  SM_SLOT_COUNTS = 28,
  SM_BUILD_WORDS = 32,
  SM_BK_LEVEL = 40,
  SM_GEOM = 64,
  SM_SLOT_HIST = 64,
  SM_ALLREDUCE = 512,
  SM_WORDS = 1024
};
static_assert(SM_ERR < SM_BUILD_WORDS && SM_BBOX + 6 <= SM_BUILD_WORDS && SM_NVOX < SM_BUILD_WORDS &&
                  SM_NSPLIT < SM_BUILD_WORDS && SM_NTILES < SM_BUILD_WORDS && SM_ETOTAL < SM_BUILD_WORDS &&
                  SM_NBLOCKS < SM_BUILD_WORDS && SM_BK_TICKET < SM_BUILD_WORDS && SM_BK_OVERFULL < SM_BUILD_WORDS &&
                  SM_SLOT_VOXELS < SM_BUILD_WORDS && SM_MASK_TOTAL < SM_BUILD_WORDS &&
                  SM_BK_NOORDER < SM_BUILD_WORDS && SM_DEBUG_TOTAL < SM_BUILD_WORDS && SM_BK_FLAGS < SM_BUILD_WORDS &&
                  SM_BK_TOTAL < SM_BUILD_WORDS && SM_BK_TODO < SM_BUILD_WORDS && SM_BK_MISSING < SM_BUILD_WORDS &&
                  SM_CK_COUNT < SM_BUILD_WORDS && SM_INC_NEWVOX < SM_BUILD_WORDS &&
                  SM_SLOT_COUNTS + 4 <= SM_BUILD_WORDS,
              "single words of the scalar block lie among the words k_build_begin resets");
static_assert(SM_BUILD_WORDS <= SM_BK_LEVEL && SM_BK_LEVEL + 7 <= SM_GEOM && SM_GEOM + 192 / 4 <= SM_ALLREDUCE &&
                  SM_SLOT_HIST + 256 <= SM_ALLREDUCE && SM_ALLREDUCE + 2 * 256 <= SM_WORDS,
              "scalar block regions");
uint32_t octl_wait_next_seq(octl_ctx* ctx);
int octl_wait_mirror_flags(octl_ctx* ctx, const int* words, int n_words, uint32_t seq, int64_t budget_us);
__device__ __forceinline__ void mirror_publish(uint32_t* mirror, int word, uint32_t seq) {
  __threadfence_system();
  __hip_atomic_store(&mirror[word], seq, __ATOMIC_RELEASE, __HIP_MEMORY_SCOPE_SYSTEM);
}
int ctx_wait_uploads(octl_ctx* ctx, const void* p = nullptr, size_t bytes = 0);

#define HIP_TRY(ctx, expr)                                                                 \
  do {                                                                                     \
    hipError_t _e = (expr);                                                                \
    if (_e != hipSuccess)                                                                  \
      return octl_set_error((ctx), OCTL_E_HIP, "%s failed: %s (%s:%d)", #expr,             \
                            hipGetErrorString(_e), __FILE__, __LINE__);                    \
  } while (0)

#define OCTL_TRY(expr)        \
  do {                        \
    int _r = (expr);          \
    if (_r != OCTL_OK) return _r; \
  } while (0)

int pin_region_wait(octl_ctx* ctx, int r);
int pin_region_mark(octl_ctx* ctx, int r);
int octl_copy_from_pinned(octl_ctx* ctx, void* dst_dev, const void* src_pinned, size_t bytes);

int devbuf_reserve(octl_ctx* ctx, DevBuf& b, size_t bytes, int keep = 0);
void devbuf_free(DevBuf& b);
void devbuf_release(octl_ctx* ctx, DevBuf& b);

struct KTimer {
  octl_ctx* ctx;
  int idx = -1;
  KTimer(octl_ctx* c, const char* name);
  ~KTimer();
};
int octl_collect_timings(octl_ctx* ctx);

static inline int64_t ceil_div(int64_t a, int64_t b) { return (a + b - 1) / b; }
static inline constexpr size_t align256(size_t x) { return (x + 255) & ~(size_t)255; }
struct Carve {
  template <typename T>
  struct Part {
    size_t off = 0;
  };
  size_t total = 0;
  template <typename T>
  constexpr Part<T> add(size_t count) {
    const Part<T> part{total};
    total += align256(count * sizeof(T));
    return part;
  }
  template <typename T>
  static T* at(DevBuf& b, Part<T> part) {
    return reinterpret_cast<T*>(static_cast<char*>(b.p) + part.off);
  }
};
static inline unsigned grid_for(int64_t n) { return (unsigned)ceil_div(n, 256); }
static inline int bits_for(uint64_t max_value) {
  int b = 0;
  while (b < 64 && (max_value >> b) != 0) ++b;
  return b;
}
static inline int octl_readback(octl_ctx* ctx, const void* src_dev, int64_t count, void* out) {
  HIP_TRY(ctx, hipMemcpyAsync(ctx->small_host, src_dev, (size_t)count * 4, hipMemcpyDeviceToHost, ctx->stream));
  HIP_TRY(ctx, hipStreamSynchronize(ctx->stream));
  std::memcpy(out, ctx->small_host, (size_t)count * 4);
  return OCTL_OK;
}

template <typename T>
static inline hipError_t octl_download(octl_ctx* ctx, T* dst, DevBuf& src, Carve::Part<T> part, size_t count,
                                       bool* any) {
  if (!dst || count == 0) return hipSuccess;
  *any = true;
  return hipMemcpyAsync(dst, Carve::at(src, part), count * sizeof(T), hipMemcpyDeviceToHost, ctx->stream);
}

int octl_ctx_cus(octl_ctx* ctx);
bool octl_ctx_side_stream(octl_ctx* ctx);
int octl_exclusive_scan_u32(octl_ctx* ctx, const uint32_t* in, uint32_t* out, int64_t n,
                            uint32_t* total_dev);
int octl_scan_status_acquire(octl_ctx* ctx, int64_t tiles, uint64_t** status, uint32_t* epoch);
int octl_scan_status_reserve(octl_ctx* ctx, int64_t tiles);
int octl_exclusive_scan_reserve(octl_ctx* ctx, int64_t n);
int octl_radix_sort_u64_u32(octl_ctx* ctx, uint64_t* keys[2], uint32_t* vals[2], int64_t n,
                            int key_bits, DevBuf& hist_scratch, int* result);
```

### octreelib_amd/csrc/ctx.hip

```cpp
#include <chrono>
#include <cstdarg>
#include <cstdlib>

#include <algorithm>

#include "common.h"

int octl_set_error(octl_ctx* ctx, int code, const char* fmt, ...) {
  char buf[1024];
  va_list ap;
  va_start(ap, fmt);
  vsnprintf(buf, sizeof(buf), fmt, ap);
  va_end(ap);
  if (ctx) ctx->err = buf;
  return code;
}

std::atomic<uint64_t> g_octl_host_syncs{0};

namespace {
struct OptName { const char* name; int64_t OctlOptions::*field; };
const OptName kOptions[] = {
    {"NO_BUCKET_BUILD", &OctlOptions::no_bucket_build},     {"BUCKET_POINTS", &OctlOptions::bucket_points},
    {"SYNC_GEOM", &OctlOptions::sync_geom},                 {"NO_GEOM_HINT", &OctlOptions::no_geom_hint},
    {"NO_EXACT_DIGITS", &OctlOptions::no_exact_digits},     {"NO_FAST_ORDER", &OctlOptions::no_fast_order},
    {"NO_BUCKET_HISTORY", &OctlOptions::no_bucket_history}, {"NO_CUBE_FAST", &OctlOptions::no_cube_fast},
    {"NO_CUBE_PREFIX", &OctlOptions::no_cube_prefix},       {"CUBE_PREFIX_MIN", &OctlOptions::cube_prefix_min},
    {"NO_INCREMENTAL", &OctlOptions::no_incremental},       {"ROUTE_SELF_SENDRECV", &OctlOptions::route_self_sendrecv},
    {"TRACE_BUILD", &OctlOptions::trace_build},             {"SCAN", &OctlOptions::scan_mode},
    {"NO_FUSED_TABLES", &OctlOptions::no_fused_tables},     {"NO_SPIN_WAIT", &OctlOptions::no_spin_wait},
    {"NO_SPEC_FINISH", &OctlOptions::no_spec_finish},       {"RANSAC_WAVES", &OctlOptions::ransac_waves},
    {"GEOM_MARGIN", &OctlOptions::geom_margin},             {"NO_RANSAC_PRESCREEN", &OctlOptions::no_ransac_prescreen},
};
}

int64_t* octl_option_field(OctlOptions& o, const char* name) {
  if (!name) return nullptr;
  if (std::strncmp(name, "OCTL_", 5) == 0) name += 5;
  for (const OptName& e : kOptions)
    if (std::strcmp(e.name, name) == 0) return &(o.*(e.field));
  return nullptr;
}

static void options_from_environment(OctlOptions& o) {
  char var[64];
  for (const OptName& e : kOptions) {
    std::snprintf(var, sizeof(var), "OCTL_%s", e.name);
    const char* v = getenv(var);
    if (!v) continue;
    char* end = nullptr;
    const long long x = std::strtoll(v, &end, 10);
    o.*(e.field) = (end != v) ? (int64_t)x : 1;
  }
}

extern "C" int octl_debug_set_option(octl_ctx* ctx, const char* name, int64_t value) {
  if (!ctx) return OCTL_E_INVALID;
  int64_t* f = octl_option_field(ctx->opt, name);
  if (!f) return octl_set_error(ctx, OCTL_E_INVALID, "no such option: %s", name ? name : "(null)");
  *f = value;
  return OCTL_OK;
}

std::atomic<uint64_t> g_octl_launches{0};

extern "C" int octl_debug_launches(uint64_t* count) {
  if (!count) return OCTL_E_INVALID;
  *count = g_octl_launches.load(std::memory_order_relaxed);
  return OCTL_OK;
}

std::atomic<uint64_t> g_octl_spec_held{0}, g_octl_spec_missed{0};

extern "C" int octl_debug_spec_finish(uint64_t* held, uint64_t* missed) {
  if (!held || !missed) return OCTL_E_INVALID;
  *held = g_octl_spec_held.load(std::memory_order_relaxed);
  *missed = g_octl_spec_missed.load(std::memory_order_relaxed);
  return OCTL_OK;
}

extern "C" int octl_debug_host_syncs(uint64_t* count) {
  if (!count) return OCTL_E_INVALID;
  *count = g_octl_host_syncs.load(std::memory_order_relaxed);
  return OCTL_OK;
}

static inline void octl_cpu_relax() {
#if defined(__x86_64__) || defined(__i386__)
  __builtin_ia32_pause();
#elif defined(__aarch64__) || defined(__arm__)
  __asm__ __volatile__("yield");
#else
  std::atomic_signal_fence(std::memory_order_seq_cst);
#endif
}

uint32_t octl_wait_next_seq(octl_ctx* ctx) {
  if (++ctx->wait_seq == 0) ++ctx->wait_seq;
  return ctx->wait_seq;
}

static int mirror_check_violation(octl_ctx* ctx) {
  volatile uint32_t* m = static_cast<volatile uint32_t*>(ctx->small_host);
  if (!m[MIRROR_RS_VIOLATION]) return OCTL_OK;
  m[MIRROR_RS_VIOLATION] = 0;
  return octl_set_error(ctx, OCTL_E_STATE,
                        "RANSAC: a block is larger than the launch's size bound (the kernels for larger blocks were not "
                        "launched, its mask is stale): the block table changed without resetting the bound");
}

int octl_wait_mirror_flags(octl_ctx* ctx, const int* words, int n_words, uint32_t seq, int64_t budget_us) {
  volatile uint32_t* m = static_cast<volatile uint32_t*>(ctx->small_host);
  auto all_there = [&]() {
    for (int i = 0; i < n_words; ++i)
      if (m[words[i]] != seq) return false;
    return true;
  };
  if (!ctx->opt.no_spin_wait && budget_us > 0) {
    g_octl_host_syncs.fetch_add(1, std::memory_order_relaxed);
    const auto t0 = std::chrono::steady_clock::now();
    for (;;) {
      for (int spin = 0; spin < 64; ++spin) {
        if (all_there()) {
          std::atomic_thread_fence(std::memory_order_acquire);
          return mirror_check_violation(ctx);
        }
        octl_cpu_relax();
      }
      if (std::chrono::duration_cast<std::chrono::microseconds>(std::chrono::steady_clock::now() - t0).count() > budget_us)
        break;
    }
    g_octl_host_syncs.fetch_sub(1, std::memory_order_relaxed);
  }
  HIP_TRY(ctx, hipStreamSynchronize(ctx->stream));
  if (!all_there())
    return octl_set_error(ctx, OCTL_E_HIP, "a kernel did not publish its results (mirror flag %d)", words[0]);
  return mirror_check_violation(ctx);
}

bool octl_ctx_side_stream(octl_ctx* ctx) {
  if (ctx->self_stream) return true;
  hipStream_t st = nullptr;
  hipEvent_t gate = nullptr, done = nullptr;
  if (hipStreamCreateWithFlags(&st, hipStreamNonBlocking) == hipSuccess &&
      hipEventCreateWithFlags(&gate, hipEventDisableTiming) == hipSuccess &&
      hipEventCreateWithFlags(&done, hipEventDisableTiming) == hipSuccess) {
    ctx->self_stream = st;
    ctx->self_gate = gate;
    ctx->self_done = done;
    return true;
  }
  if (done) (void)hipEventDestroy(done);
  if (gate) (void)hipEventDestroy(gate);
  if (st) (void)hipStreamDestroy(st);
  (void)hipGetLastError();
  return false;
}

int octl_ctx_cus(octl_ctx* ctx) {
  if (ctx->cus <= 0) {
    hipDeviceProp_t prop;
    ctx->cus = (hipGetDeviceProperties(&prop, ctx->device) == hipSuccess && prop.multiProcessorCount > 0)
                   ? prop.multiProcessorCount
                   : 256;
  }
  return ctx->cus;
}

static std::atomic<int64_t> g_fail_alloc_at{0};
static std::atomic<int64_t> g_alloc_growths{0};

extern "C" int octl_debug_fail_alloc(int64_t nth, int64_t* seen) {
  if (seen) *seen = g_alloc_growths.load(std::memory_order_relaxed);
  g_alloc_growths.store(0, std::memory_order_relaxed);
  g_fail_alloc_at.store(nth > 0 ? nth : 0, std::memory_order_relaxed);
  return OCTL_OK;
}

int devbuf_reserve(octl_ctx* ctx, DevBuf& b, size_t bytes, int keep) {
  if (bytes <= b.cap) return OCTL_OK;
  {
    const int64_t k = g_alloc_growths.fetch_add(1, std::memory_order_relaxed) + 1;
    const int64_t at = g_fail_alloc_at.load(std::memory_order_relaxed);
    if (at > 0 && k == at)
      return octl_set_error(ctx, OCTL_E_NOMEM, "hipMalloc(%zu) failed: injected by octl_debug_fail_alloc (growth %lld)",
                            bytes, (long long)k);
  }
  size_t want = bytes + bytes / 4 + 256;
  if (keep && b.p && b.cap) want = std::max(want, 2 * b.cap);
  void* np = nullptr;
  hipError_t e = hipSuccess;
  int best = -1;
  for (int i = 0; i < (int)ctx->pool.size(); ++i)
    if (ctx->pool[i].cap >= bytes && ctx->pool[i].cap <= 2 * want &&
        (best < 0 || ctx->pool[i].cap < ctx->pool[best].cap))
      best = i;
  if (best >= 0) {
    np = ctx->pool[best].p;
    want = ctx->pool[best].cap;
    ctx->pool_bytes -= want;
    ctx->pool.erase(ctx->pool.begin() + best);
  } else {
    e = hipMalloc(&np, want);
    if (e != hipSuccess && !ctx->pool.empty()) {
      for (auto& pb : ctx->pool) (void)hipFree(pb.p);
      ctx->pool.clear();
      ctx->pool_bytes = 0;
      e = hipMalloc(&np, want);
    }
  }
  if (e != hipSuccess)
    return octl_set_error(ctx, OCTL_E_NOMEM, "hipMalloc(%zu) failed: %s", want,
                          hipGetErrorString(e));
  if (keep && b.p && b.cap) {
    e = hipMemcpyAsync(np, b.p, b.cap, hipMemcpyDeviceToDevice, ctx->stream);
    if (e == hipSuccess) e = hipStreamSynchronize(ctx->stream);
    if (e != hipSuccess) {
      (void)hipFree(np);
      return octl_set_error(ctx, OCTL_E_HIP, "devbuf copy failed: %s", hipGetErrorString(e));
    }
  } else if (b.p) {
    (void)hipStreamSynchronize(ctx->stream);
  }
  if (b.p) devbuf_release(ctx, b);
  b.p = np;
  b.cap = want;
  return OCTL_OK;
}

void devbuf_release(octl_ctx* ctx, DevBuf& b) {
  if (!b.p) return;
  if (ctx && ctx->pool_bytes + b.cap <= ((size_t)48 << 30) && ctx->pool.size() < 2048) {
    ctx->pool.push_back(b);
    ctx->pool_bytes += b.cap;
  } else {
    (void)hipFree(b.p);
  }
  b.p = nullptr;
  b.cap = 0;
}

int pin_region_wait(octl_ctx* ctx, int r) {
  if (ctx->pin_event[r] && hipEventQuery(ctx->pin_event[r]) != hipSuccess) {
    (void)hipGetLastError();
    HIP_TRY(ctx, hipEventSynchronize(ctx->pin_event[r]));
  }
  return OCTL_OK;
}

int pin_region_mark(octl_ctx* ctx, int r) {
  if (!ctx->pin_event[r])
    HIP_TRY(ctx, hipEventCreateWithFlags(&ctx->pin_event[r], hipEventDisableTiming));
  HIP_TRY(ctx, hipEventRecord(ctx->pin_event[r], ctx->stream));
  return OCTL_OK;
}

namespace {
__global__ __launch_bounds__(256) void k_copy_u64(const uint64_t* __restrict__ src, uint64_t* __restrict__ dst, size_t n) {
  for (size_t i = (size_t)blockIdx.x * blockDim.x + threadIdx.x; i < n; i += (size_t)gridDim.x * blockDim.x) dst[i] = src[i];
}
}

int octl_copy_from_pinned(octl_ctx* ctx, void* dst_dev, const void* src_pinned, size_t bytes) {
  const size_t n = bytes / 8;
  if (n == 0) return OCTL_OK;
  const unsigned grid = (unsigned)std::min<size_t>(64, (n + 255) / 256);
  OCTL_LAUNCH(k_copy_u64, dim3(grid), dim3(256), 0, ctx->stream, static_cast<const uint64_t*>(src_pinned),
                     static_cast<uint64_t*>(dst_dev), n);
  HIP_TRY(ctx, hipGetLastError());
  return OCTL_OK;
}

void devbuf_free(DevBuf& b) {
  if (b.p) (void)hipFree(b.p);
  b.p = nullptr;
  b.cap = 0;
}

KTimer::KTimer(octl_ctx* c, const char* name) : ctx(c) {
  if (!ctx->profiling) return;
  if (ctx->profiling == 2 && std::strcmp(name, "ransac") != 0) return;
  PendingEvent pe;
  pe.name = name;
  for (hipEvent_t* ev : {&pe.start, &pe.stop}) {
    if (!ctx->event_pool.empty()) {
      *ev = ctx->event_pool.back();
      ctx->event_pool.pop_back();
    } else if (hipEventCreate(ev) != hipSuccess) {
      return;
    }
  }
  (void)hipEventRecord(pe.start, ctx->stream);
  idx = (int)ctx->pending.size();
  ctx->pending.push_back(pe);
}

KTimer::~KTimer() {
  if (idx >= 0) (void)hipEventRecord(ctx->pending[idx].stop, ctx->stream);
}

int octl_collect_timings(octl_ctx* ctx) {
  if (ctx->pending.empty()) return OCTL_OK;
  HIP_TRY(ctx, hipStreamSynchronize(ctx->stream));
  for (auto& pe : ctx->pending) {
    float ms = 0.f;
    if (hipEventElapsedTime(&ms, pe.start, pe.stop) == hipSuccess) {
      auto& t = ctx->timings[pe.name];
      t.ms += ms;
      t.launches += 1;
    }
    ctx->event_pool.push_back(pe.start);
    ctx->event_pool.push_back(pe.stop);
  }
  ctx->pending.clear();
  return OCTL_OK;
}

int ctx_wait_uploads(octl_ctx* ctx, const void* p, size_t bytes) {
  const char* a = static_cast<const char*>(p);
  for (auto& u : ctx->uploads) {
    if (a && (a + bytes <= u.dst || u.dst + u.bytes <= a)) continue;
    HIP_TRY(ctx, hipStreamWaitEvent(ctx->stream, u.done, 0));
  }
  return OCTL_OK;
}

extern "C" {

int octl_abi_version(void) { return OCTL_ABI_VERSION; }

int octl_device_count(int* count) {
  if (!count) return OCTL_E_INVALID;
  int n = 0;
  hipError_t e = hipGetDeviceCount(&n);
  *count = (e == hipSuccess) ? n : 0;
  return e == hipSuccess ? OCTL_OK : OCTL_E_HIP;
}

int octl_ctx_create(int device_id, octl_ctx** out) {
  if (!out) return OCTL_E_INVALID;
  *out = nullptr;
  int n = 0;
  if (hipGetDeviceCount(&n) != hipSuccess || n <= 0 || device_id < 0 || device_id >= n)
    return OCTL_E_HIP;
  if (hipSetDevice(device_id) != hipSuccess) return OCTL_E_HIP;
  octl_ctx* ctx = new octl_ctx();
  ctx->device = device_id;
  options_from_environment(ctx->opt);
  if (hipStreamCreateWithFlags(&ctx->stream, hipStreamNonBlocking) != hipSuccess) {
    delete ctx;
    return OCTL_E_HIP;
  }
  if (hipMalloc(&ctx->small.p, 4096) != hipSuccess ||
      hipHostMalloc(&ctx->small_host, 4096, hipHostMallocDefault) != hipSuccess ||
      hipHostMalloc(&ctx->pinned, OCTL_PINNED_BYTES, hipHostMallocDefault) != hipSuccess) {
    if (ctx->small.p) (void)hipFree(ctx->small.p);
    (void)hipStreamDestroy(ctx->stream);
    delete ctx;
    return OCTL_E_NOMEM;
  }
  ctx->small.cap = 4096;
  std::memset(ctx->small_host, 0, 4096);
  (void)hipMemsetAsync(ctx->small.p, 0, 4096, ctx->stream);
  (void)hipStreamSynchronize(ctx->stream);
  *out = ctx;
  return OCTL_OK;
}

int octl_comm_destroy(octl_ctx* ctx);

void octl_ctx_destroy(octl_ctx* ctx) {
  if (!ctx) return;
  (void)hipSetDevice(ctx->device);
  (void)hipStreamSynchronize(ctx->stream);
  if (ctx->comm) (void)octl_comm_destroy(ctx);
  for (auto& pe : ctx->pending) {
    (void)hipEventDestroy(pe.start);
    (void)hipEventDestroy(pe.stop);
  }
  for (auto ev : ctx->event_pool) (void)hipEventDestroy(ev);
  if (ctx->handoff_event) (void)hipEventDestroy(ctx->handoff_event);
  for (auto ev : ctx->pin_event)
    if (ev) (void)hipEventDestroy(ev);
  for (auto& pb : ctx->pool) (void)hipFree(pb.p);
  ctx->pool.clear();
  for (auto& ub : ctx->user_blocks) (void)hipFree(ub.first);
  ctx->user_blocks.clear();
  for (auto& b : ctx->scan_tmp) devbuf_free(b);
  devbuf_free(ctx->hyp_dev);
  devbuf_free(ctx->f32_stage);
  devbuf_free(ctx->xf_stage);
  if (ctx->xf_event) (void)hipEventDestroy(ctx->xf_event);
  devbuf_free(ctx->ls_buf);
  devbuf_free(ctx->rs_counters);
  devbuf_free(ctx->scan_status);
  devbuf_free(ctx->small);
  devbuf_free(ctx->routed_xyz);
  devbuf_free(ctx->routed_gidx);
  for (DevBuf* b : {&ctx->rt_hist, &ctx->rt_counts, &ctx->rt_matrix, &ctx->rt_send_xyz,
                    &ctx->rt_send_gidx})
    devbuf_free(*b);
  if (ctx->small_host) (void)hipHostFree(ctx->small_host);
  if (ctx->pinned) (void)hipHostFree(ctx->pinned);
  if (ctx->self_stream) {
    (void)hipStreamSynchronize(ctx->self_stream);
    (void)hipStreamDestroy(ctx->self_stream);
    if (ctx->self_gate) (void)hipEventDestroy(ctx->self_gate);
    if (ctx->self_done) (void)hipEventDestroy(ctx->self_done);
  }
  if (ctx->copy_stream) {
    (void)hipStreamSynchronize(ctx->copy_stream);
    (void)hipStreamDestroy(ctx->copy_stream);
  }
  if (ctx->copy_gate) (void)hipEventDestroy(ctx->copy_gate);
  for (auto& u : ctx->uploads) (void)hipEventDestroy(u.done);
  (void)hipStreamDestroy(ctx->stream);
  delete ctx;
}

const char* octl_last_error(const octl_ctx* ctx) { return ctx ? ctx->err.c_str() : "null context"; }

int octl_ctx_sync(octl_ctx* ctx) {
  if (!ctx) return OCTL_E_INVALID;
  HIP_TRY(ctx, hipStreamSynchronize(ctx->stream));
  return mirror_check_violation(ctx);
}

int octl_host_alloc(octl_ctx* ctx, int64_t bytes, void** p) {
  if (!ctx || !p || bytes < 0) return OCTL_E_INVALID;
  (void)hipSetDevice(ctx->device);
  hipError_t e = hipHostMalloc(p, (size_t)(bytes > 0 ? bytes : 1), hipHostMallocDefault);
  if (e != hipSuccess)
    return octl_set_error(ctx, OCTL_E_NOMEM, "hipHostMalloc(%lld) failed: %s", (long long)bytes, hipGetErrorString(e));
  return OCTL_OK;
}

int octl_host_free(octl_ctx* ctx, void* p) {
  if (!ctx) return OCTL_E_INVALID;
  if (ctx->copy_stream) (void)hipStreamSynchronize(ctx->copy_stream);
  if (p) HIP_TRY(ctx, hipHostFree(p));
  return OCTL_OK;
}

int octl_dev_upload_async(octl_ctx* ctx, void* dptr, const void* src, int64_t bytes) {
  if (!ctx || bytes < 0 || (bytes > 0 && (!dptr || !src))) return OCTL_E_INVALID;
  HIP_TRY(ctx, hipSetDevice(ctx->device));
  if (!ctx->copy_stream) {
    HIP_TRY(ctx, hipStreamCreateWithFlags(&ctx->copy_stream, hipStreamNonBlocking));
    HIP_TRY(ctx, hipEventCreateWithFlags(&ctx->copy_gate, hipEventDisableTiming));
  }
  if (bytes == 0) return OCTL_OK;
  HIP_TRY(ctx, hipEventRecord(ctx->copy_gate, ctx->stream));
  HIP_TRY(ctx, hipStreamWaitEvent(ctx->copy_stream, ctx->copy_gate, 0));
  HIP_TRY(ctx, hipMemcpyAsync(dptr, src, (size_t)bytes, hipMemcpyHostToDevice, ctx->copy_stream));
  hipEvent_t ev = nullptr;
  for (size_t i = 0; i < ctx->uploads.size();) {
    if (hipEventQuery(ctx->uploads[i].done) == hipSuccess) {
      if (!ev) ev = ctx->uploads[i].done; else (void)hipEventDestroy(ctx->uploads[i].done);
      ctx->uploads.erase(ctx->uploads.begin() + (long)i);
    } else {
      (void)hipGetLastError();
      ++i;
    }
  }
  if (!ev) HIP_TRY(ctx, hipEventCreateWithFlags(&ev, hipEventDisableTiming));
  HIP_TRY(ctx, hipEventRecord(ev, ctx->copy_stream));
  ctx->uploads.push_back(octl_ctx::Upload{static_cast<const char*>(dptr), (size_t)bytes, ev});
  return OCTL_OK;
}

int octl_ctx_sync_uploads(octl_ctx* ctx) {
  if (!ctx) return OCTL_E_INVALID;
  if (ctx->copy_stream) HIP_TRY(ctx, hipStreamSynchronize(ctx->copy_stream));
  return OCTL_OK;
}

int octl_ctx_set_profiling(octl_ctx* ctx, int enabled) {
  if (!ctx) return OCTL_E_INVALID;
  OCTL_TRY(octl_collect_timings(ctx));
  ctx->profiling = enabled == 2 ? 2 : (enabled != 0 ? 1 : 0);
  ctx->timings.clear();
  return OCTL_OK;
}

int octl_ctx_get_timings(octl_ctx* ctx, char* names, int name_stride, float* ms,
                         int64_t* launches, int cap, int* n) {
  if (!ctx || !n) return OCTL_E_INVALID;
  OCTL_TRY(octl_collect_timings(ctx));
  *n = (int)ctx->timings.size();
  int i = 0;
  for (auto& kv : ctx->timings) {
    if (i >= cap) break;
    if (names && name_stride > 0) {
      std::snprintf(names + (size_t)i * name_stride, name_stride, "%s", kv.first.c_str());
    }
    if (ms) ms[i] = (float)kv.second.ms;
    if (launches) launches[i] = kv.second.launches;
    ++i;
  }
  return OCTL_OK;
}

int octl_dev_alloc(octl_ctx* ctx, int64_t bytes, void** dptr) {
  if (!ctx || !dptr || bytes < 0) return OCTL_E_INVALID;
  (void)hipSetDevice(ctx->device);
  DevBuf b;
  OCTL_TRY(devbuf_reserve(ctx, b, (size_t)(bytes > 0 ? bytes : 1)));
  ctx->user_blocks[b.p] = b.cap;
  *dptr = b.p;
  return OCTL_OK;
}

int octl_dev_free(octl_ctx* ctx, void* dptr) {
  if (!ctx) return OCTL_E_INVALID;
  if (!dptr) return OCTL_OK;
  const char* a = static_cast<const char*>(dptr);
  auto it = ctx->user_blocks.find(dptr);
  const size_t cap = it != ctx->user_blocks.end() ? it->second : 0;
  for (auto& u : ctx->uploads)
    if (!cap || !(a + cap <= u.dst || u.dst + u.bytes <= a)) (void)hipEventSynchronize(u.done);
  (void)hipStreamSynchronize(ctx->stream);
  if (it == ctx->user_blocks.end()) {
    HIP_TRY(ctx, hipFree(dptr));
    return OCTL_OK;
  }
  DevBuf b{dptr, cap};
  ctx->user_blocks.erase(it);
  devbuf_release(ctx, b);
  return OCTL_OK;
}

int octl_dev_upload(octl_ctx* ctx, void* dptr, const void* src, int64_t bytes) {
  if (!ctx || (bytes > 0 && (!dptr || !src))) return OCTL_E_INVALID;
  HIP_TRY(ctx, hipMemcpyAsync(dptr, src, (size_t)bytes, hipMemcpyHostToDevice, ctx->stream));
// ... 43 lines not shown
```

### octreelib_amd/csrc/mask.hip

```cpp
#include "forest.h"
#include "lookback.h"

namespace {

__device__ __forceinline__ void mask_tile_count(const uint8_t* __restrict__ mask, int64_t n,
                                                uint32_t* __restrict__ tilecnt, uint32_t tile,
                                                uint8_t* __restrict__ alive_fill) {
  __shared__ uint32_t s_w[4];
  const int64_t i0 = (int64_t)tile * 2048 + (int64_t)threadIdx.x * 8;
  uint32_t c = 0;
  if (i0 + 8 <= n) {
    const uint64_t w = *reinterpret_cast<const uint64_t*>(mask + i0);
    const uint64_t nz = ((w & 0x7F7F7F7F7F7F7F7Full) + 0x7F7F7F7F7F7F7F7Full) | w;
    c = (uint32_t)__popcll(nz & 0x8080808080808080ull);
    if (alive_fill) *reinterpret_cast<uint64_t*>(alive_fill + i0) = 0x0101010101010101ull;
  } else {
    for (int64_t i = i0; i < n; ++i) {
      c += mask[i] ? 1u : 0u;
      if (alive_fill) alive_fill[i] = 1;
    }
  }
#pragma unroll
  for (int off = 32; off > 0; off >>= 1) c += __shfl_xor(c, off);
  if ((threadIdx.x & 63) == 0) s_w[threadIdx.x >> 6] = c;
// ... 425 lines not shown
  const size_t o_out = (((size_t)n_all + 8) * 4 + 15) & ~(size_t)15;
  OCTL_TRY(devbuf_reserve(ctx, f->flags, 2 * o_out));
  if (!ctx->opt.no_fused_tables && nt + 2 * ceil_div(nb, 256) <= 1024)
    OCTL_TRY(octl_scan_status_reserve(ctx, nt + 2 * ceil_div(nb, 256)));
  else
    OCTL_TRY(octl_exclusive_scan_reserve(ctx, n_all));
  OCTL_TRY(devbuf_reserve(ctx, f->ord_idx2, (size_t)n * 4));
  OCTL_TRY(devbuf_reserve(ctx, f->xyz_ord2, (size_t)n * 24));
  OCTL_TRY(devbuf_reserve(ctx, f->blk_node2, (size_t)n * 4));
  OCTL_TRY(devbuf_reserve(ctx, f->blk_slot2, (size_t)n * 4));
  OCTL_TRY(devbuf_reserve(ctx, f->blk_start2, (size_t)n * 4));
  OCTL_TRY(devbuf_reserve(ctx, f->blk_size2, (size_t)n * 4));
  return OCTL_OK;
}

int mask_retire_slots(octl_forest* f, const uint8_t* sel_dev, unsigned long long* removed_dev) {
  octl_ctx* ctx = f->ctx;
  if (f->n_ord > 0 && f->n_blocks > 0) {
    KTimer t(ctx, "remove_poses");
    OCTL_LAUNCH(k_retire_mask, dim3((unsigned)std::min<int64_t>(ceil_div(f->n_blocks, 4), 2048)), dim3(256), 0, ctx->stream,
                (const uint32_t*)f->blk_start.as<uint32_t>(), (const int32_t*)f->blk_size.as<int32_t>(),
                (const int32_t*)f->blk_slot.as<int32_t>(), f->n_blocks, sel_dev, f->mask_valid ? 0 : 1,
                f->mask.as<uint8_t>(), removed_dev);
    HIP_TRY(ctx, hipGetLastError());
    f->mask_valid = true;
  }
  return apply_device_mask(f, nullptr);
}

int mask_apply(octl_forest* f, int64_t* n_alive) { return apply_device_mask(f, n_alive); }

int forest_settle(octl_forest* f) {
  if (!f->totals_pending) return OCTL_OK;
  octl_ctx* ctx = f->ctx;
  f->totals_pending = false;
  if (ctx->pending_mask_forest == f) ctx->pending_mask_forest = nullptr;
  const int flags[2] = {MIRROR_FLAG_MASK0, MIRROR_FLAG_MASK1};
  const int64_t n = f->totals_n_before;
  OCTL_TRY(octl_wait_mirror_flags(ctx, flags, 2, f->totals_seq, 500 + n / 2000));
  uint32_t res[2];
  std::memcpy(res, static_cast<uint32_t*>(ctx->small_host) + MIRROR_MASK_TOTALS, 8);
  f->n_alive -= (n - (int64_t)res[0]);
  f->n_ord = res[0];
  f->n_blocks = res[1];
  return OCTL_OK;
}

void forest_forget_pending(octl_forest* f) {
  if (!f->totals_pending) return;
  f->totals_pending = false;
  if (f->ctx->pending_mask_forest == f) f->ctx->pending_mask_forest = nullptr;
}

int ensure_mask(octl_forest* f) {
  octl_ctx* ctx = f->ctx;
  if (f->mask_valid) return OCTL_OK;
  OCTL_TRY(devbuf_reserve(ctx, f->mask, (size_t)std::max<int64_t>(f->n_ord, 1)));
  if (f->n_ord > 0)
    HIP_TRY(ctx, hipMemsetAsync(f->mask.p, 1, (size_t)f->n_ord, ctx->stream));
  f->mask_valid = true;
  return OCTL_OK;
}

extern "C" {

int octl_forest_get_mask(octl_forest* f, int64_t cap, uint8_t* mask, int64_t* n_out) {
  if (!f || !n_out) return OCTL_E_INVALID;
  OCTL_TRY(forest_settle(f));
  octl_ctx* ctx = f->ctx;
  if (!f->built) return octl_set_error(ctx, OCTL_E_STATE, "no scheme has been built");
  *n_out = f->n_ord;
  const int64_t n = std::min<int64_t>(cap, f->n_ord);
  if (n <= 0 || !mask) return OCTL_OK;
  OCTL_TRY(ensure_mask(f));
  HIP_TRY(ctx, hipMemcpyAsync(mask, f->mask.p, (size_t)n, hipMemcpyDeviceToHost, ctx->stream));
  HIP_TRY(ctx, hipStreamSynchronize(ctx->stream));
  return OCTL_OK;
}

int octl_forest_apply_mask(octl_forest* f, int64_t* n_alive) {
  if (!f) return OCTL_E_INVALID;
  OCTL_TRY(forest_settle(f));
  if (!f->built) return octl_set_error(f->ctx, OCTL_E_STATE, "apply_mask before build");
  OCTL_TRY(ensure_mask(f));
  return apply_device_mask(f, n_alive);
}

int octl_forest_apply_mask_async(octl_forest* f) {
  if (!f) return OCTL_E_INVALID;
  OCTL_TRY(forest_settle(f));
  if (!f->built) return octl_set_error(f->ctx, OCTL_E_STATE, "apply_mask before build");
  OCTL_TRY(ensure_mask(f));
  return apply_device_mask(f, nullptr, true);
}

int octl_forest_settle(octl_forest* f, int64_t* n_alive) {
  if (!f) return OCTL_E_INVALID;
  OCTL_TRY(forest_settle(f));
  if (n_alive) *n_alive = f->n_ord;
  return OCTL_OK;
}

int octl_forest_filter_count(octl_forest* f, const uint8_t* slot_sel, int32_t n_sel, int64_t lo,
                             int64_t hi, int64_t* n_alive) {
  if (!f || !slot_sel) return OCTL_E_INVALID;
  OCTL_TRY(forest_settle(f));
  octl_ctx* ctx = f->ctx;
  if (!f->built) return octl_set_error(ctx, OCTL_E_STATE, "filter before build");
  const int n_poses = (int)f->pose_off.size() - 1;
  if (n_sel != n_poses) return octl_set_error(ctx, OCTL_E_INVALID, "slot selection has %d entries for %d poses", n_sel, n_poses);
  HIP_TRY(ctx, hipSetDevice(ctx->device));
  hipStream_t st = ctx->stream;
  OCTL_TRY(ensure_mask(f));
  if (f->n_blocks > 0) {
    OCTL_TRY(devbuf_reserve(ctx, f->scheme_dev, (size_t)std::max(n_poses, 1)));
    HIP_TRY(ctx, hipMemcpyAsync(f->scheme_dev.p, slot_sel, (size_t)n_poses, hipMemcpyHostToDevice, st));
    HIP_TRY(ctx, hipStreamSynchronize(st));
    KTimer t(ctx, "filter");
    OCTL_LAUNCH(k_filter_blocks, dim3((unsigned)ceil_div(f->n_blocks, 4)), dim3(256), 0, st,
                       (const uint32_t*)f->blk_start.as<uint32_t>(), (const int32_t*)f->blk_size.as<int32_t>(),
                       (const int32_t*)f->blk_slot.as<int32_t>(), f->n_blocks,
                       (const uint8_t*)f->scheme_dev.as<uint8_t>(), lo, hi, f->mask.as<uint8_t>());
    HIP_TRY(ctx, hipGetLastError());
  }
  return apply_device_mask(f, n_alive);
}

int octl_forest_carve(octl_forest* f, const uint32_t* through, const uint32_t* hits, int64_t n_nodes,
                      const uint8_t* slot_sel, int32_t n_sel, int64_t min_through, int64_t max_hits,
                      int64_t* n_alive) {
  if (!f) return OCTL_E_INVALID;
  return forest_carve(f, through, hits, false, n_nodes, slot_sel, n_sel, min_through, max_hits, n_alive);
}

int octl_forest_carve_device(octl_forest* f, const uint32_t* through_dev, const uint32_t* hits_dev, int64_t n_nodes,
                             const uint8_t* slot_sel, int32_t n_sel, int64_t min_through, int64_t max_hits,
                             int64_t* n_alive) {
  if (!f) return OCTL_E_INVALID;
  return forest_carve(f, through_dev, hits_dev, true, n_nodes, slot_sel, n_sel, min_through, max_hits, n_alive);
}

int octl_forest_apply_host_mask(octl_forest* f, const uint8_t* mask, int64_t n, int64_t* n_alive) {
  if (!f) return OCTL_E_INVALID;
  OCTL_TRY(forest_settle(f));
  octl_ctx* ctx = f->ctx;
  if (!f->built) return octl_set_error(ctx, OCTL_E_STATE, "apply_mask before build");
  if (n != f->n_ord || (n > 0 && !mask))
    return octl_set_error(ctx, OCTL_E_INVALID, "mask has %lld entries for %lld points",
                          (long long)n, (long long)f->n_ord);
  OCTL_TRY(devbuf_reserve(ctx, f->mask, (size_t)std::max<int64_t>(n, 1)));
  if (n > 0) {
    HIP_TRY(ctx, hipMemcpyAsync(f->mask.p, mask, (size_t)n, hipMemcpyHostToDevice, ctx->stream));
    HIP_TRY(ctx, hipStreamSynchronize(ctx->stream));
  }
  f->mask_valid = true;
  return apply_device_mask(f, n_alive);
}

}
```

### octreelib_amd/csrc/order.hip

```cpp
#include <algorithm>

#include "forest.h"

namespace {

__global__ __launch_bounds__(256) void k_sub_up(const int32_t* __restrict__ first_child,
                                                int64_t a, int64_t b,
                                                uint32_t* __restrict__ nint) {
  const int64_t x = a + (int64_t)blockIdx.x * blockDim.x + threadIdx.x;
  if (x >= b) return;
  const int32_t fc = first_child[x];
  uint32_t s = 0;
  if (fc >= 0) {
    s = 1;
#pragma unroll
    for (int j = 0; j < 8; ++j) s += nint[fc + j];
  }
  nint[x] = s;
}

__global__ __launch_bounds__(256) void k_rank_down(const int32_t* __restrict__ first_child,
                                                   int64_t a, int64_t b,
                                                   const uint32_t* __restrict__ nint,
                                                   uint32_t* __restrict__ rank) {
// ... 197 lines not shown
    if ((size_t)n_poses * 4 <= 64 * 1024) {
      char* pin = static_cast<char*>(ctx->pinned) + 192 * 1024;
      OCTL_TRY(pin_region_wait(ctx, 2));
      std::memcpy(pin, e0_host, (size_t)n_poses * 4);
      HIP_TRY(ctx, hipMemcpyAsync(f->scheme_dev.p, pin, (size_t)n_poses * 4, hipMemcpyHostToDevice, st));
      OCTL_TRY(pin_region_mark(ctx, 2));
    } else {
      HIP_TRY(ctx, hipMemcpyAsync(f->scheme_dev.p, e0_host, (size_t)n_poses * 4,
                                  hipMemcpyHostToDevice, st));
      HIP_TRY(ctx, hipStreamSynchronize(st));
    }
    e0_dev = f->scheme_dev.as<int32_t>();
    for (int p = 0; p < n_poses; ++p) max_epoch = std::max(max_epoch, (int)e0_host[p]);
  }
  const int ebits = std::max(1, bits_for((uint64_t)max_epoch));
  const int bits2 = bits_for((uint64_t)n_poses * (uint64_t)V) + ebits;
  if (bits2 > 63) return octl_set_error(ctx, OCTL_E_INVALID, "order key too wide");
  const int bits1 = bits_for((uint64_t)f->n_internal * 8u + 7u);
  for (int b = 0; b < 2; ++b) {
    OCTL_TRY(devbuf_reserve(ctx, f->lin[b], (size_t)nb * 8));
    OCTL_TRY(devbuf_reserve(ctx, f->val[b], (size_t)nb * 4));
  }
  OCTL_TRY(devbuf_reserve(ctx, f->vkey, (size_t)nb * 8));
  uint64_t* keys[2] = {f->lin[0].as<uint64_t>(), f->lin[1].as<uint64_t>()};
  uint32_t* vals[2] = {f->val[0].as<uint32_t>(), f->val[1].as<uint32_t>()};
  uint64_t* key2 = f->vkey.as<uint64_t>();
  OCTL_LAUNCH(k_block_keys, dim3(grid_for(nb)), dim3(256), 0, st,
                     (const int32_t*)f->blk_node.as<int32_t>(),
                     (const int32_t*)f->blk_slot.as<int32_t>(), nb,
                     (const int32_t*)t.parent.as<int32_t>(), fc,
                     (const int32_t*)t.voxel.as<int32_t>(), (const int32_t*)t.epoch.as<int32_t>(),
                     (const uint32_t*)rank, e0_dev, (uint64_t)V, ebits, keys[0], key2, vals[0]);
  HIP_TRY(ctx, hipGetLastError());
  int res = 0;
  OCTL_TRY(octl_radix_sort_u64_u32(ctx, keys, vals, nb, bits1, f->hist, &res));
  uint64_t* keys_b[2] = {keys[res ^ 1], keys[res]};
  uint32_t* vals_b[2] = {vals[res], vals[res ^ 1]};
  OCTL_LAUNCH(k_gather_key2, dim3(grid_for(nb)), dim3(256), 0, st, (const uint64_t*)key2,
                     (const uint32_t*)vals[res], nb, keys_b[0]);
  HIP_TRY(ctx, hipGetLastError());
  int res2 = 0;
  OCTL_TRY(octl_radix_sort_u64_u32(ctx, keys_b, vals_b, nb, bits2, f->hist, &res2));
  OCTL_TRY(devbuf_reserve(ctx, f->rs_order, (size_t)nb * 4));
  HIP_TRY(ctx, hipMemcpyAsync(f->rs_order.p, vals_b[res2], (size_t)nb * 4,
                              hipMemcpyDeviceToDevice, st));
  uint32_t* hist = ctx->small.as<uint32_t>() + SM_SLOT_HIST;
  if (!need_slot_counts) {
  } else if (n_poses <= 256) {
    static_assert(256 <= MIRROR_COPY_WORDS, "the slot counts land in the copy area of the mirror, below its flag words");
    HIP_TRY(ctx, hipMemsetAsync(hist, 0, (size_t)n_poses * 4, st));
    OCTL_LAUNCH(k_slot_hist, dim3((unsigned)ceil_div(nb, 2048)), dim3(256), 0, st,
                       (const int32_t*)f->blk_slot.as<int32_t>(), nb, hist);
    HIP_TRY(ctx, hipGetLastError());
    OCTL_TRY(octl_readback(ctx, hist, n_poses, slot_counts.data()));
  } else {
    std::vector<int32_t> slots((size_t)nb);
    HIP_TRY(ctx, hipMemcpyAsync(slots.data(), f->blk_slot.p, (size_t)nb * 4, hipMemcpyDeviceToHost, st));
    HIP_TRY(ctx, hipStreamSynchronize(st));
    for (int32_t s : slots) slot_counts[(size_t)s] += 1;
  }
  return OCTL_OK;
}

extern "C" int octl_forest_reference_order(octl_forest* f, const int32_t* e0, int32_t n_e0,
                                           int64_t cap, int32_t* order, int64_t* n_blocks) {
  if (!f || !n_blocks) return OCTL_E_INVALID;
  OCTL_TRY(forest_settle(f));
  octl_ctx* ctx = f->ctx;
  if (!f->built) return octl_set_error(ctx, OCTL_E_STATE, "no scheme has been built");
  const int n_poses = (int)f->pose_off.size() - 1;
  if (e0 && n_e0 != n_poses) return octl_set_error(ctx, OCTL_E_INVALID, "e0 size mismatch");
  std::vector<uint32_t> slot_counts;
  OCTL_TRY(forest_reference_order(f, e0, slot_counts, false));
  *n_blocks = f->n_blocks;
  const int64_t n = std::min<int64_t>(cap, f->n_blocks);
  if (n > 0 && order) {
    HIP_TRY(ctx, hipMemcpyAsync(order, f->rs_order.p, (size_t)n * 4, hipMemcpyDeviceToHost,
                                ctx->stream));
    HIP_TRY(ctx, hipStreamSynchronize(ctx->stream));
  }
  return OCTL_OK;
}

static int ransac_all_impl(octl_forest* f, int32_t poses_per_batch, const int32_t* e0, int32_t n_e0,
                           const double* hypotheses, int32_t H, int32_t k, double threshold,
                           bool* mask_fresh);

extern "C" int octl_forest_ransac_all(octl_forest* f, int32_t poses_per_batch, const int32_t* e0,
                                      int32_t n_e0, const double* hypotheses, int32_t H, int32_t k,
                                      double threshold) {
  if (!f || !hypotheses) return OCTL_E_INVALID;
  OCTL_TRY(forest_settle(f));
  bool mask_fresh = false;
  const int rc = ransac_all_impl(f, poses_per_batch, e0, n_e0, hypotheses, H, k, threshold, &mask_fresh);
  if (mask_fresh) f->mask_valid = (rc == OCTL_OK);
  return rc;
}

static int ransac_all_impl(octl_forest* f, int32_t poses_per_batch, const int32_t* e0, int32_t n_e0,
                           const double* hypotheses, int32_t H, int32_t k, double threshold,
                           bool* mask_fresh) {
  octl_ctx* ctx = f->ctx;
  if (!f->built) return octl_set_error(ctx, OCTL_E_STATE, "ransac before build");
  if (poses_per_batch < 1) return octl_set_error(ctx, OCTL_E_INVALID, "poses_per_batch < 1");
  if (H < 1 || H > 1024 || k < 1) return octl_set_error(ctx, OCTL_E_INVALID, "bad H or k");
  OCTL_TRY(ransac_check_table(ctx, hypotheses, H, k));
  const int n_poses = (int)f->pose_off.size() - 1;
  if (e0 && n_e0 != n_poses) return octl_set_error(ctx, OCTL_E_INVALID, "e0 size mismatch");
  HIP_TRY(ctx, hipSetDevice(ctx->device));
  hipStream_t st = ctx->stream;
  if (!f->mask_valid) {
    OCTL_TRY(devbuf_reserve(ctx, f->mask, (size_t)std::max<int64_t>(f->n_ord, 1)));
    *mask_fresh = true;
  }
  if (f->n_blocks == 0) return OCTL_OK;
  const size_t hyp_cap_before = ctx->hyp_dev.cap;
  OCTL_TRY(devbuf_reserve(ctx, ctx->hyp_dev, (size_t)H * k * 8));
  const bool same_table = hyp_cap_before == ctx->hyp_dev.cap && ctx->hyp_host.size() == (size_t)H * k &&
                          std::memcmp(ctx->hyp_host.data(), hypotheses, (size_t)H * k * 8) == 0;
  if (same_table) {
  } else if ((size_t)H * k * 8 <= 64 * 1024) {
    char* pin = static_cast<char*>(ctx->pinned) + 128 * 1024;
    OCTL_TRY(pin_region_wait(ctx, 1));
    std::memcpy(pin, hypotheses, (size_t)H * k * 8);
    OCTL_TRY(octl_copy_from_pinned(ctx, ctx->hyp_dev.p, pin, (size_t)H * k * 8));
    OCTL_TRY(pin_region_mark(ctx, 1));
  } else {
    HIP_TRY(ctx, hipMemcpyAsync(ctx->hyp_dev.p, hypotheses, (size_t)H * k * 8, hipMemcpyHostToDevice, st));
    HIP_TRY(ctx, hipStreamSynchronize(st));
  }
  if (!same_table) ctx->hyp_host.assign(hypotheses, hypotheses + (size_t)H * k);
  const bool one_batch = n_poses <= poses_per_batch;
  std::vector<uint32_t> slot_counts;
  OCTL_TRY(forest_reference_order(f, e0, slot_counts, !one_batch));
  if (one_batch) {
    OCTL_TRY(ransac_launch(ctx, f->xyz_ord.as<double>(), f->n_ord, f->blk_start.as<uint32_t>(),
                           f->blk_size.as<int32_t>(), f->rs_order.as<int32_t>(), f->n_blocks,
                           ctx->hyp_dev.as<double>(), H, k, threshold, f->mask.as<uint8_t>(), nullptr,
                           nullptr, nullptr, nullptr, f->rs_scratch, f->max_block_hint));
    return OCTL_OK;
  }
  int64_t off = 0;
  for (int p0 = 0; p0 < n_poses; p0 += poses_per_batch) {
    int64_t nbatch = 0;
    for (int p = p0; p < std::min(n_poses, p0 + poses_per_batch); ++p) nbatch += slot_counts[p];
    if (nbatch > 0)
      OCTL_TRY(ransac_launch(ctx, f->xyz_ord.as<double>(), f->n_ord, f->blk_start.as<uint32_t>(),
                             f->blk_size.as<int32_t>(), f->rs_order.as<int32_t>() + off, nbatch,
                             ctx->hyp_dev.as<double>(), H, k, threshold, f->mask.as<uint8_t>(),
                             nullptr, nullptr, nullptr, nullptr, f->rs_scratch, f->max_block_hint));
    off += nbatch;
  }
  return OCTL_OK;
}
```

### octreelib_amd/csrc/ransac.hip

```cpp
#include <algorithm>
#include <cstdlib>
#include <type_traits>

#include "forest.h"
#include "lookback.h"
#include "plane_cert.h"
#include "wave_utils.h"

namespace {

__device__ __forceinline__ double div_by_small_int(double c, int k) {
  const double kd = (double)k;
  const double zh = 1.0 / kd;
  const double zl = fma(-kd, zh, 1.0) / kd;
  const double a = fabs(c);
  if (!((int(a > 1e-290) | int(c == 0.0)) & int(a < 1e290))) return c / kd;
  return copysign(fma(c, zh, c * zl), c);
}

__device__ __forceinline__ bool coord_in_fast_range(double v) {
  const uint32_t hi = (uint32_t)__double2hiint(v), lo = (uint32_t)__double2loint(v);
  const uint32_t e = (hi >> 20) & 0x7FFu;
  return (e - (1023u - 30u)) <= 60u || (hi | lo) == 0u;
}
// ... 1591 lines not shown
    d.pstart = pst[r];
    d.n = nn[r];
    d.vstart = (int64_t)pre;
    pre += (uint32_t)nn[r];
    uint32_t sp = d.n > 0 ? d.pstart + (uint32_t)d.n - 1u : d.pstart;
    if (phys[r + 1] >= 0) {
      sp = pst[r + 1];
    } else if (!order) {
      const int64_t e = (int64_t)d.pstart + d.n;
      if (e < n_points) sp = (uint32_t)e;
    }
    d.pspill = sp;
    d.pad[0] = 0;
    d.pad[1] = (uint32_t)b;
    d.pad[2] = 0;
    const int n = d.n;
    d.n = -1;
    if (n < k) {
      for (int i = 0; i < n; ++i) out.mask[(int64_t)d.pstart + i] = 0;
      if (out.plane) {
        out.plane[4 * b + 0] = 0.f; out.plane[4 * b + 1] = 0.f;
        out.plane[4 * b + 2] = 0.f; out.plane[4 * b + 3] = 0.f;
      }
      if (out.count) out.count[b] = 0;
      if (out.index) out.index[b] = -1;
    } else if (n > cap) {
      d.n = n;
      desc[b] = d;
      d.n = -1;
      big_list[atomicAdd(&counters[RC_BIG], 1u)] = (uint32_t)b;
    } else {
      d.n = n;
      rank[r] = atomicAdd(&bins[n], 1u);
    }
    if (n >= k && (int64_t)n > max_block)
      __hip_atomic_store(&mirror[MIRROR_RS_VIOLATION], 1u, __ATOMIC_RELAXED, __HIP_MEMORY_SCOPE_SYSTEM);
  }
  __syncthreads();
  uint32_t cm = 0, incm = 0;
  if (threadIdx.x < 256) {
    cm = bins[255 - threadIdx.x];
    incm = wave_inclusive_add(cm);
    if (lane == 63) s_wave[wave] = incm;
  }
  __syncthreads();
  if (threadIdx.x < 256) {
    uint32_t f = incm - cm;
    for (int w = 0; w < wave; ++w) f += s_wave[w];
    const int m = 255 - (int)threadIdx.x;
    first[m] = f;
    counters[RC_BINS + m] = cm;
    counters[RC_START + m] = f;
    if (m == 0) counters[RC_SORTED] = f + cm;
  }
  __syncthreads();
#pragma unroll
  for (int r = 0; r < BPS_PER_THREAD; ++r)
    if (dd[r].n >= 0) sdesc[first[dd[r].n] + rank[r]] = dd[r];
}

}

int ransac_check_table(octl_ctx* ctx, const double* hyp, int32_t H, int32_t k) {
  const int64_t n = (int64_t)H * k;
  for (int64_t i = 0; i < n; ++i)
    if (!(hyp[i] >= 0.0 && hyp[i] < 1.0))
      return octl_set_error(ctx, OCTL_E_INVALID,
                            "hypothesis table entry %lld = %g is outside [0, 1): the table must hold "
                            "np.random.random draws (cuda_ransac.py:39-41)", (long long)i, hyp[i]);
  return OCTL_OK;
}

int ransac_launch(octl_ctx* ctx, const double* xyz_dev, int64_t n_points,
                  const uint32_t* blk_start, const int32_t* blk_size, const int32_t* order_dev,
                  int64_t nb, const double* hyp_dev, int32_t H, int32_t k, double thr,
                  uint8_t* mask_dev, float* plane_dev, int32_t* count_dev, int32_t* index_dev,
                  uint8_t* evaluated_dev, DevBuf& scratch, int64_t max_block) {
  (void)evaluated_dev;
  if (nb <= 0) return OCTL_OK;
  if (H < 1 || H > 1024) return octl_set_error(ctx, OCTL_E_INVALID, "H must be in [1, 1024]");
  if (k < 1) return octl_set_error(ctx, OCTL_E_INVALID, "initial_points_number must be positive");
  const bool any_k = k > RS_KMAX;
  if (nb >= ((int64_t)1 << 31)) return octl_set_error(ctx, OCTL_E_INVALID, "too many blocks");
  hipStream_t st = ctx->stream;
  const size_t off_d = (((size_t)nb + 8) * 4 + 31) & ~(size_t)31;
  const size_t off_s = off_d + (size_t)nb * sizeof(BlockDesc);
  const size_t off_b = off_s + (size_t)nb * sizeof(BlockDesc);
  const size_t off_c = (off_b + (size_t)nb * 4 + 31) & ~(size_t)31;
  const bool use_tab = !any_k && k >= 3 && k <= 6 && (H > 256 || k == 6);
  const size_t off_t = (off_c + RC_WORDS * 4 + 31) & ~(size_t)31;
  const size_t tab_bytes = (size_t)256 * (size_t)H * sizeof(uint2) + (size_t)RS_TINY_THREADS * (size_t)H * sizeof(uint32_t);
  OCTL_TRY(devbuf_reserve(ctx, scratch, off_t + (use_tab ? tab_bytes : 0)));
  char* base = static_cast<char*>(scratch.p);
  uint32_t* tmp = scratch.as<uint32_t>();
  BlockDesc* desc = reinterpret_cast<BlockDesc*>(base + off_d);
  BlockDesc* sdesc = reinterpret_cast<BlockDesc*>(base + off_s);
  uint32_t* big_list = reinterpret_cast<uint32_t*>(base + off_b);
  uint32_t* counters = reinterpret_cast<uint32_t*>(base + off_c);
  const bool fused = !ctx->opt.no_fused_tables;
  uint32_t* next_counters = nullptr;
  if (fused) {
    if (!ctx->rs_counters.p || ctx->rs_counters_dirty) {
      OCTL_TRY(devbuf_reserve(ctx, ctx->rs_counters, (size_t)2 * RC_WORDS * 4));
      HIP_TRY(ctx, hipMemsetAsync(ctx->rs_counters.p, 0, (size_t)2 * RC_WORDS * 4, st));
      ctx->rs_parity = 0;
    }
    counters = ctx->rs_counters.as<uint32_t>() + (size_t)ctx->rs_parity * RC_WORDS;
    next_counters = ctx->rs_counters.as<uint32_t>() + (size_t)(ctx->rs_parity ^ 1) * RC_WORDS;
    ctx->rs_parity ^= 1;
    ctx->rs_counters_dirty = true;
  }
  uint2* pos_tab = use_tab ? reinterpret_cast<uint2*>(base + off_t) : nullptr;
  const int threads = (H <= 64) ? 64 : (H <= 256 ? 256 : RS_BIG_THREADS);
  RansacOut out{mask_dev, plane_dev, count_dev, index_dev};
  if (fused && nb <= BPS_MAX) {
    KTimer t(ctx, "ransac_prepare");
    const int cap = any_k ? 0 : threads - 1;
    const unsigned n_table = use_tab && cap >= k ? (unsigned)(cap - k + 1) * (unsigned)ceil_div(H, BPS_THREADS) : 0u;
    auto kp = nb <= 2 * BPS_THREADS ? k_block_prepare_small<2>
              : (nb <= 4 * BPS_THREADS ? k_block_prepare_small<4>
                                       : (nb <= 6 * BPS_THREADS ? k_block_prepare_small<6> : k_block_prepare_small<8>));
    OCTL_LAUNCH(kp, dim3(1 + n_table), dim3(BPS_THREADS), 0, st, order_dev, blk_start, blk_size, nb,
                       n_points, cap, (int)k, desc, sdesc, big_list, counters, out, max_block,
                       static_cast<uint32_t*>(ctx->small_host), hyp_dev, (int)H, pos_tab, next_counters);
    HIP_TRY(ctx, hipGetLastError());
    ctx->rs_counters_dirty = false;
  } else {
    KTimer t(ctx, "ransac_prepare");
    if (fused) {
      const unsigned g = (unsigned)ceil_div(nb, 256 * BP_PER_THREAD);
      uint64_t* status = nullptr;
      uint32_t epoch = 0;
      OCTL_TRY(octl_scan_status_acquire(ctx, g, &status, &epoch));
      OCTL_LAUNCH(k_block_prepare, dim3(g), dim3(256), 0, st, order_dev, blk_start, blk_size, nb, n_points,
                         any_k ? 0 : threads - 1, (int)k, desc, big_list, counters, out, status, epoch, max_block,
                         static_cast<uint32_t*>(ctx->small_host));
      HIP_TRY(ctx, hipGetLastError());
    } else {
      const unsigned g = (unsigned)ceil_div(nb, 256);
      OCTL_LAUNCH(k_block_sizes_in_order, dim3(g), dim3(256), 0, st, order_dev, blk_size, nb, tmp, counters);
      HIP_TRY(ctx, hipGetLastError());
      OCTL_TRY(octl_exclusive_scan_u32(ctx, tmp, tmp, nb, nullptr));
      OCTL_LAUNCH(k_block_desc, dim3((unsigned)ceil_div(nb, 256 * BD_PER_THREAD)), dim3(256), 0, st, order_dev,
                         blk_start, blk_size,
                         (const uint32_t*)tmp, nb, n_points, any_k ? 0 : threads - 1, (int)k, desc, big_list,
                         counters, out);
      HIP_TRY(ctx, hipGetLastError());
    }
    const unsigned n_scatter = (unsigned)ceil_div(nb, 256 * BS_PER_THREAD);
    const unsigned n_table = use_tab ? 256u * (unsigned)ceil_div(H, 256) : 0u;
    OCTL_LAUNCH(k_block_scatter, dim3(n_scatter + n_table), dim3(256), 0, st,
                       (const BlockDesc*)desc, nb, any_k ? 0 : threads - 1, (int)k, counters, sdesc, n_scatter, hyp_dev,
                       (int)H, pos_tab, next_counters);
    HIP_TRY(ctx, hipGetLastError());
    ctx->rs_counters_dirty = false;
  }
  const int cus = octl_ctx_cus(ctx);
  KTimer t(ctx, "ransac");
  hipStream_t side = st;
  bool on_side = false;
  int waves_per_block = (int)ctx->opt.ransac_waves;
  if (waves_per_block == 0 && !any_k && H > 256) {
    const int64_t slots = (int64_t)cus * 16;
    if (nb * 2 <= slots) waves_per_block = 4;
    else if (nb <= 6 * slots) waves_per_block = 2;
  }
// ... 181 lines not shown
```

Baseline: 4019 Mpoints/s.

## Run bucket-build front partition pass ahead on a side stream

New measurement: 4163 Mpoints/s (median of 6 runs). +3.6%, better.

```diff
diff --git a/include/octreelib_hip.h b/include/octreelib_hip.h
--- a/include/octreelib_hip.h
+++ b/include/octreelib_hip.h
@@ -251,6 +251,7 @@
 int octl_debug_host_syncs(uint64_t* count);
 int octl_debug_launches(uint64_t* count);
 int octl_debug_spec_finish(uint64_t* held, uint64_t* missed);
+int octl_debug_builds_ahead(uint64_t* count);
 
 int octl_debug_route_partition(octl_ctx* ctx, const double* xyz, int64_t n, int64_t index_base,
                                double L, int32_t n_ranks, int64_t* counts, double* xyz_out,
diff --git a/octreelib_amd/_native.py b/octreelib_amd/_native.py
--- a/octreelib_amd/_native.py
+++ b/octreelib_amd/_native.py
@@ -164,6 +164,7 @@
     "octl_debug_host_syncs": (C.c_int, [C.POINTER(C.c_uint64)]),
     "octl_debug_launches": (C.c_int, [C.POINTER(C.c_uint64)]),
     "octl_debug_spec_finish": (C.c_int, [C.POINTER(C.c_uint64), C.POINTER(C.c_uint64)]),
+    "octl_debug_builds_ahead": (C.c_int, [C.POINTER(C.c_uint64)]),
     "octl_debug_fail_alloc": (C.c_int, [_i64, _pi64]),
     "octl_debug_set_option": (C.c_int, [_p, C.c_char_p, _i64]),
     "octl_debug_key_geometry": (C.c_int, [_p, C.c_uint64, _i64, C.c_uint32, _i32, _p, _p, _p, _p, _p]),
@@ -264,7 +265,8 @@
 
     def reset_options(self):
         for name in list(self.__dict__.get("_options_touched", ())):
-            self.lib.octl_debug_set_option(self.handle, name.encode(), 0)
+            shipped = -1 if name.removeprefix("OCTL_") == "BUILD_AHEAD_MIN_POINTS" else 0
+            self.lib.octl_debug_set_option(self.handle, name.encode(), shipped)
         self.__dict__["_options_touched"] = set()
 
     def set_profiling(self, enabled: bool):
diff --git a/octreelib_amd/csrc/api.hip b/octreelib_amd/csrc/api.hip
--- a/octreelib_amd/csrc/api.hip
+++ b/octreelib_amd/csrc/api.hip
@@ -141,6 +141,10 @@
 void octl_forest_destroy(octl_forest* f) {
   if (!f) return;
   forest_forget_pending(f);
+  if (f->ctx->ahead_forest == f) {
+    f->ctx->ahead_forest = nullptr;
+    f->ctx->ahead_mark_valid = f->ctx->ahead_mark_pending = false;
+  }
   (void)hipSetDevice(f->ctx->device);
   (void)hipStreamSynchronize(f->ctx->stream);
   nodes_free(f->ctx, f->nodes[0]);
diff --git a/octreelib_amd/csrc/bucket_build.hip b/octreelib_amd/csrc/bucket_build.hip
--- a/octreelib_amd/csrc/bucket_build.hip
+++ b/octreelib_amd/csrc/bucket_build.hip
@@ -2068,9 +2068,12 @@
   *tiles = (int)std::min<int64_t>(16, std::max<int64_t>(1, ceil_div(ceil_div(items, PT_TILE), (int64_t)octl_ctx_cus(ctx) * wgs)));
   return (uint32_t)ceil_div(items, (int64_t)*tiles * PT_TILE);
 }
+size_t part_table_bytes(size_t cells, size_t tail_words, size_t* elems) {
+  *elems = (cells + 1 + 15) & ~(size_t)15;
+  return (2 * *elems + tail_words + 16) * 4;
+}
 int part_table_reserve(octl_forest* f, size_t cells, size_t tail_words, size_t* elems) {
-  *elems = (cells + 1 + 15) & ~(size_t)15;
-  return devbuf_reserve(f->ctx, f->bk_table, (2 * *elems + tail_words + 16) * 4);
+  return devbuf_reserve(f->ctx, f->bk_table, part_table_bytes(cells, tail_words, elems));
 }
 bool tables_fused(const octl_ctx* ctx, uint32_t nst) { return !ctx->opt.no_fused_tables && nst <= TS_MAX_ROWS; }
 
@@ -2089,6 +2092,7 @@
   size_t tab_elems = 0;
   bool own_scan = false;
   PartRec* out = nullptr;
+  bool ahead = false;
   const char *t_hist = nullptr, *t_scan = nullptr, *t_scatter = nullptr;
 };
 
@@ -2104,8 +2108,10 @@
     const unsigned g = (p.nd + TS_COLS - 1) / TS_COLS;
     uint64_t* status = nullptr;
     uint32_t epoch = 0;
-    OCTL_TRY(octl_scan_status_acquire(ctx, g, &status, &epoch));
-    OCTL_LAUNCH(k_table_scan, dim3(g), dim3(TS_THREADS), 0, ctx->stream, table, p.nst, p.nd, table_dm, status, epoch,
+    if (p.ahead) OCTL_TRY(octl_ahead_status_acquire(ctx, g, &status, &epoch));
+    else OCTL_TRY(octl_scan_status_acquire(ctx, g, &status, &epoch));
+    OCTL_LAUNCH(k_table_scan, dim3(g), dim3(TS_THREADS), 0, p.ahead ? ctx->ahead_stream : ctx->stream, table, p.nst,
+                       p.nd, table_dm, status, epoch,
                        p.validate, p.ask ? (const int32_t*)f->bbox_dev.as<int32_t>() : (const int32_t*)nullptr,
                        p.ask ? *p.ask : GeomAsk{0, 0, 0, 0}, p.lp, p.gdev);
     HIP_TRY(ctx, hipGetLastError());
@@ -2119,7 +2125,7 @@
 
 int partition_pass(octl_forest* f, const PartPass& p, const uint32_t** bstart, uint32_t* bstride) {
   octl_ctx* ctx = f->ctx;
-  hipStream_t st = ctx->stream;
+  hipStream_t st = p.ahead ? ctx->ahead_stream : ctx->stream;
   const uint32_t nst = p.nst, nd = p.nd;
   const bool fused = tables_fused(ctx, nst);
   uint32_t *table = f->bk_table.as<uint32_t>(), *table_dm = table + p.tab_elems;
@@ -2239,15 +2245,31 @@
   return OCTL_OK;
 }
 
+uint64_t bucket_want(const octl_ctx* ctx, int64_t n_alive, uint64_t* target) {
+  *target = ctx->opt.bucket_points > 0 ? (uint64_t)ctx->opt.bucket_points : (n_alive <= 400000 ? 1280 : 2560);
+  uint64_t want = 1;
+  while (want < ((uint64_t)PT_BINS << PT_BITS) && want * *target < (uint64_t)n_alive) want <<= 1;
+  return want;
+}
+bool front_pass_fits(const octl_forest* f, uint32_t nd, uint32_t nst) {
+  size_t elems = 0;
+  return f->n_alive == f->n_store && tables_fused(f->ctx, nst) &&
+         (int64_t)((nd + TS_COLS - 1) / TS_COLS) <= OCTL_AHEAD_TILES &&
+         f->part_xyz[0].cap >= (size_t)f->n_alive * sizeof(PartRec) &&
+         f->bk_table.cap >= part_table_bytes((size_t)nd * nst, 0, &elems);
+}
+bool front_goes_ahead(const BucketBuild& b, const BucketBuildArgs& a) {
+  return b.ctx->ahead_open && b.hinted && b.async_geom && !b.two_pass && !a.scheme_dev &&
+         front_pass_fits(b.f, b.nd_a, b.nst_a);
+}
+
 int plan_geometry(BucketBuild& b, bool force_sync, BuildVerdict* v) {
   octl_forest* f = b.f;
   octl_ctx* ctx = b.ctx;
   const int64_t n_alive = f->n_alive;
   *v = BV_GO;
-  const uint64_t target = ctx->opt.bucket_points > 0 ? (uint64_t)ctx->opt.bucket_points
-                                                     : (n_alive <= 400000 ? 1280 : 2560);
-  uint64_t want = 1;
-  while (want < ((uint64_t)PT_BINS << PT_BITS) && want * target < (uint64_t)n_alive) want <<= 1;
+  uint64_t target = 0;
+  const uint64_t want = bucket_want(ctx, n_alive, &target);
   b.async_geom = !force_sync && !ctx->geom_sparse && want <= (uint64_t)PT_BINS && !ctx->opt.sync_geom;
   const int margin = f->mode != 0 ? 0
                                   : (ctx->opt.geom_margin == 0 ? 1 : (int)std::min<int64_t>(64, std::max<int64_t>(0, ctx->opt.geom_margin)));
@@ -2320,6 +2342,9 @@
   octl_forest* f = b.f;
   octl_ctx* ctx = b.ctx;
   const int64_t n_alive = f->n_alive;
+  const bool ahead = front_goes_ahead(b, a);
+  if (!ahead) octl_ahead_join(ctx);
+  hipStream_t front = ahead ? ctx->ahead_stream : b.st;
   OCTL_TRY(devbuf_reserve(ctx, f->part_xyz[0], (size_t)n_alive * sizeof(PartRec)));
   if (b.two_pass) OCTL_TRY(devbuf_reserve(ctx, f->part_xyz[1], (size_t)n_alive * sizeof(PartRec)));
   OCTL_TRY(part_table_reserve(f, std::max((size_t)b.nd_a * b.nst_a, (size_t)b.nd_b * b.nst_b),
@@ -2335,7 +2360,7 @@
   if (b.async_geom || b.hinted2) b.gdev = reinterpret_cast<GeomDev*>(b.small + SM_GEOM);
   if (b.async_geom) {
     if (b.hinted) {
-      if (!ctx->geom_hint_staged) OCTL_LAUNCH(k_geom_set, dim3(1), dim3(64), 0, b.st, b.hint, b.gdev);
+      if (!ctx->geom_hint_staged) OCTL_LAUNCH(k_geom_set, dim3(1), dim3(64), 0, front, b.hint, b.gdev);
     } else {
       OCTL_LAUNCH(k_bucket_geom, dim3(1), dim3(64), 0, b.st, (const int32_t*)f->bbox_dev.as<int32_t>(), b.ask, b.lp,
                          b.gdev);
@@ -2361,7 +2386,13 @@
   p.own_scan = tables_fused(ctx, b.nst_a) && !b.two_pass && !b.hinted2 && b.nd_a <= 256u && b.nst_a <= PS_OWN_MAX_ROWS;
   p.out = f->part_xyz[0].as<PartRec>();
   p.t_hist = "part_hist", p.t_scan = "part_scan", p.t_scatter = "part_scatter";
+  p.ahead = ahead;
   OCTL_TRY(partition_pass(f, p, &b.bstart, &b.bstride));
+  if (ahead) {
+    octl_ahead_join(ctx);
+    g_octl_builds_ahead.fetch_add(1, std::memory_order_relaxed);
+  }
+  p.ahead = false;
   b.recs = p.out;
   if (!b.two_pass) return OCTL_OK;
   b.lp.dshift = b.s + b.bits_a, b.lp.dmask = 0xFFFFFFFFu, b.lp.raw_vp = 0;
@@ -2601,6 +2632,10 @@
 int forest_bucket_build(octl_forest* f, const BucketBuildArgs& a, NodeTable& nt, BucketBuildResult* r) {
   octl_ctx* ctx = f->ctx;
   r->done = 0;
+  struct AheadJoin {
+    octl_ctx* ctx;
+    ~AheadJoin() { octl_ahead_join(ctx); }
+  } ahead_join{ctx};
   if (f->n_alive <= 0 || !f->bbox_dev.p || ctx->opt.no_bucket_build) return OCTL_OK;
   if (f->mode == 1 && f->n_alive > 65535) return OCTL_OK;
   bool force_sync = false;
@@ -2608,6 +2643,7 @@
     BucketBuild b{f, ctx, ctx->stream, ctx->small.as<uint32_t>()};
     BuildVerdict v = BV_GO;
     OCTL_TRY(plan_geometry(b, force_sync, &v));
+    if (!b.hinted) octl_ahead_join(ctx);
     if (v == BV_AGAIN_HOST) {
       force_sync = true;
       continue;
@@ -2635,6 +2671,20 @@
     return finish_and_commit(b, a, nt, overfull, r);
   }
   return octl_set_error(ctx, OCTL_E_STATE, "bucket build: the geometry retries do not terminate");
+}
+
+bool forest_bucket_front_fits(const octl_forest* f) {
+  const octl_ctx* ctx = f->ctx;
+  if (f->n_alive <= 0 || f->n_alive != f->n_store || !f->bbox_dev.p || !f->bbox_pending || ctx->opt.no_bucket_build ||
+      (f->mode == 1 && f->n_alive > 65535))
+    return false;
+  uint64_t target = 0;
+  const uint64_t want = bucket_want(ctx, f->n_alive, &target);
+  if (ctx->geom_sparse || want > (uint64_t)PT_BINS || ctx->opt.sync_geom) return false;
+  GeomDev hint;
+  if (!hint_load(ctx, f, want, &hint) || ctx->geom_hint_two_pass) return false;
+  int tiles = 0;
+  return front_pass_fits(f, (uint32_t)geom_bucket_cap(want), supertiles(f->ctx, f->n_store, OCTL_PT_WGS, &tiles));
 }
 
 int forest_prefix_partition(octl_forest* f, int pm, const void** recs_out, const uint32_t** bstart, uint32_t* bstride,
diff --git a/octreelib_amd/csrc/build.hip b/octreelib_amd/csrc/build.hip
--- a/octreelib_amd/csrc/build.hip
+++ b/octreelib_amd/csrc/build.hip
@@ -1270,8 +1270,13 @@
 
 int build_begin(octl_forest* f, BuildRequest& rq, const uint8_t* scheme_mask) {
   octl_ctx* ctx = f->ctx;
-  hipStream_t st = ctx->stream;
   const int n_poses = rq.n_poses;
+  if (!ctx->opt.no_build_ahead && !ctx->profiling && f->store_borrowed && f->bbox_pending && n_poses == 1 &&
+      !rq.keep_scheme && !rq.planar && rq.all_scheme && !f->built && f->vkeys.empty() && !f->vkeys_stale &&
+      f->n_store >= octl_ahead_min_points(ctx) && f->pose_off_dev.cap >= (size_t)(n_poses + 1) * 8 &&
+      octl_ahead_untouched(ctx, f) && forest_bucket_front_fits(f))
+    (void)octl_ahead_open(ctx, f->xyz.p, (size_t)f->n_store * 24);
+  hipStream_t st = octl_front_stream(ctx);
   {
     uint32_t init[32];
     std::memset(init, 0, sizeof(init));
@@ -1314,7 +1319,7 @@
   }
   if (f->pose_off_uploaded != f->pose_off) {
     if (fits)
-      OCTL_TRY(octl_copy_from_pinned(ctx, f->pose_off_dev.p, src_off, off_bytes));
+      OCTL_TRY(octl_copy_from_pinned(ctx, f->pose_off_dev.p, src_off, off_bytes, st));
     else
       HIP_TRY(ctx, hipMemcpyAsync(f->pose_off_dev.p, src_off, off_bytes, hipMemcpyHostToDevice, st));
     f->pose_off_uploaded = f->pose_off;
@@ -1337,6 +1342,7 @@
   *done = 0;
   const bool unsplit_again = !rq.keep_scheme && !rq.planar && rq.K < 0 && f->built && f->n_internal == 0;
   if (!rq.keep_scheme && !unsplit_again) return OCTL_OK;
+  octl_ahead_join(f->ctx);
   OCTL_TRY(forest_insert_incremental(f, done, info));
   trace.mark("incremental insertion");
   if (*done) {
@@ -1891,6 +1897,26 @@
   return OCTL_OK;
 }
 
+int forest_build_steps(octl_forest* f, BuildRequest& rq, const uint8_t* scheme_mask, BuildTrace& trace,
+                       octl_build_info* info) {
+  const int32_t keep_scheme = rq.keep_scheme;
+  OCTL_TRY(build_begin(f, rq, scheme_mask));
+  int placed = 0;
+  OCTL_TRY(build_try_incremental(f, rq, trace, info, &placed));
+  if (placed) return OCTL_OK;
+  rq.n_alive = f->n_alive;
+  rq.cur_epoch = f->epoch + (keep_scheme ? 0 : 1);
+
+  BuildOutcome out;
+  bool bucket_built = false;
+  OCTL_TRY(build_bucket_route(f, rq, trace, out, &bucket_built));
+  octl_ahead_join(f->ctx);
+  if (!bucket_built) OCTL_TRY(build_general_route(f, rq, trace, out));
+  if (!out.blocks_made) OCTL_TRY(build_block_table(f, rq.n_alive, &out.n_blocks));
+  if (!bucket_built) trace.mark("blocks + final sync");
+  return build_commit(f, rq, out, info);
+}
+
 }
 
 int forest_build(octl_forest* f, int64_t K, const uint8_t* scheme_mask, int32_t n_mask,
@@ -1914,18 +1940,12 @@
   BuildTrace trace;
   trace.on = ctx->opt.trace_build != 0;
 
-  OCTL_TRY(build_begin(f, rq, scheme_mask));
-  int placed = 0;
-  OCTL_TRY(build_try_incremental(f, rq, trace, info, &placed));
-  if (placed) return OCTL_OK;
-  rq.n_alive = f->n_alive;
-  rq.cur_epoch = f->epoch + (keep_scheme ? 0 : 1);
-
-  BuildOutcome out;
-  bool bucket_built = false;
-  OCTL_TRY(build_bucket_route(f, rq, trace, out, &bucket_built));
-  if (!bucket_built) OCTL_TRY(build_general_route(f, rq, trace, out));
-  if (!out.blocks_made) OCTL_TRY(build_block_table(f, rq.n_alive, &out.n_blocks));
-  if (!bucket_built) trace.mark("blocks + final sync");
-  return build_commit(f, rq, out, info);
-}
+  struct BuildEnd {
+    octl_forest* f;
+    bool ok = false;
+    ~BuildEnd() { octl_ahead_build_end(f->ctx, f, ok, f->n_store); }
+  } build_end{f};
+  const int rc = forest_build_steps(f, rq, scheme_mask, trace, info);
+  build_end.ok = rc == OCTL_OK;
+  return rc;
+}
diff --git a/octreelib_amd/csrc/build_common.h b/octreelib_amd/csrc/build_common.h
--- a/octreelib_amd/csrc/build_common.h
+++ b/octreelib_amd/csrc/build_common.h
@@ -50,6 +50,7 @@
   BucketBuildGeom geom;
 };
 int forest_bucket_build(octl_forest* f, const BucketBuildArgs& a, NodeTable& nt, BucketBuildResult* r);
+bool forest_bucket_front_fits(const octl_forest* f);
 
 constexpr int PART_REC_BYTES = 32;
 constexpr int PART_REC_QUADS = PART_REC_BYTES / 16;
diff --git a/octreelib_amd/csrc/common.h b/octreelib_amd/csrc/common.h
--- a/octreelib_amd/csrc/common.h
+++ b/octreelib_amd/csrc/common.h
@@ -24,13 +24,19 @@
 #define hipStreamSynchronize(s) octl_counted_stream_sync(s)
 #define hipEventSynchronize(e) octl_counted_event_sync(e)
 extern std::atomic<uint64_t> g_octl_launches;
+extern std::atomic<uint64_t> g_octl_enqueues;
+extern std::atomic<uint64_t> g_octl_builds_ahead;
 extern std::atomic<uint64_t> g_octl_spec_held, g_octl_spec_missed;
 #define OCTL_LAUNCH(...)                                                      \
   do {                                                                        \
     g_octl_launches.fetch_add(1, std::memory_order_relaxed);                  \
+    g_octl_enqueues.fetch_add(1, std::memory_order_relaxed);                  \
     hipLaunchKernelGGL(__VA_ARGS__);                                          \
   } while (0)
-#define hipMemsetAsync(...) (g_octl_launches.fetch_add(1, std::memory_order_relaxed), hipMemsetAsync(__VA_ARGS__))
+#define hipMemsetAsync(...)                                                                                      \
+  (g_octl_launches.fetch_add(1, std::memory_order_relaxed), g_octl_enqueues.fetch_add(1, std::memory_order_relaxed), \
+   hipMemsetAsync(__VA_ARGS__))
+#define hipMemcpyAsync(...) (g_octl_enqueues.fetch_add(1, std::memory_order_relaxed), hipMemcpyAsync(__VA_ARGS__))
 
 #if !defined(OCTL_EXPERIMENTS) && \
     (defined(PS_DUP_KEYS) || defined(PS_DUP_STORE) || defined(RS_COUNTS) || defined(BB_STAMPS))
@@ -80,6 +86,8 @@
   int64_t geom_margin = 0;
   int64_t no_ransac_prescreen = 0;
   int64_t no_spec_finish = 0;
+  int64_t no_build_ahead = 0;
+  int64_t build_ahead_min_points = -1;
 };
 int64_t* octl_option_field(OctlOptions& o, const char* name);
 
@@ -105,6 +113,16 @@
   hipEvent_t copy_gate = nullptr;
   hipStream_t self_stream = nullptr;
   hipEvent_t self_gate = nullptr, self_done = nullptr;
+  hipStream_t ahead_stream = nullptr;
+  hipEvent_t ahead_free = nullptr, ahead_done = nullptr;
+  DevBuf ahead_status;
+  uint32_t ahead_epoch = 0;
+  int ahead_allow_depth = 0;
+  bool ahead_open = false;
+  bool ahead_mark_pending = false;
+  bool ahead_mark_valid = false;
+  const struct octl_forest* ahead_forest = nullptr;
+  uint64_t ahead_mark = 0, ahead_allowed = 0;
   struct Upload { const char* dst; size_t bytes; hipEvent_t done; };
   std::vector<Upload> uploads;
   std::vector<DevBuf> pool;
@@ -156,7 +174,6 @@
   SM_BK_TICKET = 17,
   SM_BK_OVERFULL = 18,
   SM_SLOT_VOXELS = 21,
-  SM_MASK_TOTAL = 22,
   SM_BK_NOORDER = 23,
   SM_DEBUG_TOTAL = 24,
   SM_BK_FLAGS = 25,
@@ -170,22 +187,25 @@
   SM_INC_NEWVOX = 31,
   SM_SLOT_COUNTS = 28,
   SM_BUILD_WORDS = 32,
+  SM_MASK_TOTAL = 33,
   SM_BK_LEVEL = 40,
   SM_GEOM = 64,
-  SM_SLOT_HIST = 64,
+  SM_SLOT_HIST = 128,
   SM_ALLREDUCE = 512,
   SM_WORDS = 1024
 };
 static_assert(SM_ERR < SM_BUILD_WORDS && SM_BBOX + 6 <= SM_BUILD_WORDS && SM_NVOX < SM_BUILD_WORDS &&
                   SM_NSPLIT < SM_BUILD_WORDS && SM_NTILES < SM_BUILD_WORDS && SM_ETOTAL < SM_BUILD_WORDS &&
                   SM_NBLOCKS < SM_BUILD_WORDS && SM_BK_TICKET < SM_BUILD_WORDS && SM_BK_OVERFULL < SM_BUILD_WORDS &&
-                  SM_SLOT_VOXELS < SM_BUILD_WORDS && SM_MASK_TOTAL < SM_BUILD_WORDS &&
+                  SM_SLOT_VOXELS < SM_BUILD_WORDS &&
                   SM_BK_NOORDER < SM_BUILD_WORDS && SM_DEBUG_TOTAL < SM_BUILD_WORDS && SM_BK_FLAGS < SM_BUILD_WORDS &&
                   SM_BK_TOTAL < SM_BUILD_WORDS && SM_BK_TODO < SM_BUILD_WORDS && SM_BK_MISSING < SM_BUILD_WORDS &&
                   SM_CK_COUNT < SM_BUILD_WORDS && SM_INC_NEWVOX < SM_BUILD_WORDS &&
                   SM_SLOT_COUNTS + 4 <= SM_BUILD_WORDS,
-              "single words of the scalar block lie among the words k_build_begin resets");
-static_assert(SM_BUILD_WORDS <= SM_BK_LEVEL && SM_BK_LEVEL + 7 <= SM_GEOM && SM_GEOM + 192 / 4 <= SM_ALLREDUCE &&
+              "the words a build starts from zero lie among the words k_build_begin resets");
+static_assert(SM_MASK_TOTAL >= SM_BUILD_WORDS && SM_MASK_TOTAL < SM_BK_LEVEL,
+              "apply_mask may be in flight beside the next build's front: its word is none of the front's");
+static_assert(SM_BUILD_WORDS <= SM_BK_LEVEL && SM_BK_LEVEL + 7 <= SM_GEOM && SM_GEOM + 192 / 4 <= SM_SLOT_HIST &&
                   SM_SLOT_HIST + 256 <= SM_ALLREDUCE && SM_ALLREDUCE + 2 * 256 <= SM_WORDS,
               "scalar block regions");
 uint32_t octl_wait_next_seq(octl_ctx* ctx);
@@ -212,7 +232,7 @@
 
 int pin_region_wait(octl_ctx* ctx, int r);
 int pin_region_mark(octl_ctx* ctx, int r);
-int octl_copy_from_pinned(octl_ctx* ctx, void* dst_dev, const void* src_pinned, size_t bytes);
+int octl_copy_from_pinned(octl_ctx* ctx, void* dst_dev, const void* src_pinned, size_t bytes, hipStream_t on = nullptr);
 
 int devbuf_reserve(octl_ctx* ctx, DevBuf& b, size_t bytes, int keep = 0);
 void devbuf_free(DevBuf& b);
@@ -270,6 +290,33 @@
 bool octl_ctx_side_stream(octl_ctx* ctx);
 int octl_exclusive_scan_u32(octl_ctx* ctx, const uint32_t* in, uint32_t* out, int64_t n,
                             uint32_t* total_dev);
+constexpr int64_t OCTL_AHEAD_MIN_POINTS = 100000;
+constexpr int64_t OCTL_AHEAD_TILES = 4096;
+static inline int64_t octl_ahead_min_points(const octl_ctx* ctx) {
+  return ctx->opt.build_ahead_min_points >= 0 ? ctx->opt.build_ahead_min_points : OCTL_AHEAD_MIN_POINTS;
+}
+bool octl_ctx_ahead_stream(octl_ctx* ctx);
+bool octl_ahead_untouched(const octl_ctx* ctx, const struct octl_forest* f);
+bool octl_ahead_open(octl_ctx* ctx, const void* cloud, size_t bytes);
+static inline hipStream_t octl_front_stream(const octl_ctx* ctx) { return ctx->ahead_open ? ctx->ahead_stream : ctx->stream; }
+void octl_ahead_join(octl_ctx* ctx);
+void octl_ahead_build_end(octl_ctx* ctx, const struct octl_forest* f, bool ok, int64_t n_points);
+void octl_ahead_arm(octl_ctx* ctx);
+int octl_ahead_status_acquire(octl_ctx* ctx, int64_t tiles, uint64_t** status, uint32_t* epoch);
+struct AheadAllow {
+  octl_ctx* ctx;
+  uint64_t at = 0;
+  explicit AheadAllow(octl_ctx* c) : ctx(c) {
+    if (ctx->ahead_allow_depth++ != 0) return;
+    if (ctx->ahead_mark_pending) octl_ahead_arm(ctx);
+    at = g_octl_enqueues.load(std::memory_order_relaxed);
+  }
+  ~AheadAllow() {
+    if (--ctx->ahead_allow_depth == 0) ctx->ahead_allowed += g_octl_enqueues.load(std::memory_order_relaxed) - at;
+  }
+  AheadAllow(const AheadAllow&) = delete;
+  AheadAllow& operator=(const AheadAllow&) = delete;
+};
 int octl_scan_status_acquire(octl_ctx* ctx, int64_t tiles, uint64_t** status, uint32_t* epoch);
 int octl_scan_status_reserve(octl_ctx* ctx, int64_t tiles);
 int octl_exclusive_scan_reserve(octl_ctx* ctx, int64_t n);
diff --git a/octreelib_amd/csrc/ctx.hip b/octreelib_amd/csrc/ctx.hip
--- a/octreelib_amd/csrc/ctx.hip
+++ b/octreelib_amd/csrc/ctx.hip
@@ -31,6 +31,7 @@
     {"NO_FUSED_TABLES", &OctlOptions::no_fused_tables},     {"NO_SPIN_WAIT", &OctlOptions::no_spin_wait},
     {"NO_SPEC_FINISH", &OctlOptions::no_spec_finish},       {"RANSAC_WAVES", &OctlOptions::ransac_waves},
     {"GEOM_MARGIN", &OctlOptions::geom_margin},             {"NO_RANSAC_PRESCREEN", &OctlOptions::no_ransac_prescreen},
+    {"NO_BUILD_AHEAD", &OctlOptions::no_build_ahead},       {"BUILD_AHEAD_MIN_POINTS", &OctlOptions::build_ahead_min_points},
 };
 }
 
@@ -67,6 +68,14 @@
 extern "C" int octl_debug_launches(uint64_t* count) {
   if (!count) return OCTL_E_INVALID;
   *count = g_octl_launches.load(std::memory_order_relaxed);
+  return OCTL_OK;
+}
+
+std::atomic<uint64_t> g_octl_enqueues{0}, g_octl_builds_ahead{0};
+
+extern "C" int octl_debug_builds_ahead(uint64_t* count) {
+  if (!count) return OCTL_E_INVALID;
+  *count = g_octl_builds_ahead.load(std::memory_order_relaxed);
   return OCTL_OK;
 }
 
@@ -157,6 +166,100 @@
   return false;
 }
 
+bool octl_ctx_ahead_stream(octl_ctx* ctx) {
+  if (ctx->ahead_stream) return true;
+  hipStream_t st = nullptr;
+  hipEvent_t free_ev = nullptr, done = nullptr;
+  const std::string err_before = ctx->err;
+  if (devbuf_reserve(ctx, ctx->ahead_status, (size_t)OCTL_AHEAD_TILES * 8) != OCTL_OK) {
+    ctx->err = err_before;
+    return false;
+  }
+  void* status = ctx->ahead_status.p;
+  if (hipStreamCreateWithFlags(&st, hipStreamNonBlocking) == hipSuccess &&
+      hipEventCreateWithFlags(&free_ev, hipEventDisableTiming) == hipSuccess &&
+      hipEventCreateWithFlags(&done, hipEventDisableTiming) == hipSuccess &&
+      (hipMemsetAsync)(status, 0, (size_t)OCTL_AHEAD_TILES * 8, st) == hipSuccess) {
+    ctx->ahead_stream = st;
+    ctx->ahead_free = free_ev;
+    ctx->ahead_done = done;
+    ctx->ahead_epoch = 0;
+    return true;
+  }
+  if (st) (void)hipStreamSynchronize(st);
+  if (done) (void)hipEventDestroy(done);
+  if (free_ev) (void)hipEventDestroy(free_ev);
+  if (st) (void)hipStreamDestroy(st);
+  (void)hipGetLastError();
+  return false;
+}
+
+bool octl_ahead_untouched(const octl_ctx* ctx, const octl_forest* f) {
+  return ctx->ahead_mark_valid && ctx->ahead_forest == f &&
+         g_octl_enqueues.load(std::memory_order_relaxed) == ctx->ahead_mark + ctx->ahead_allowed;
+}
+
+bool octl_ahead_open(octl_ctx* ctx, const void* cloud, size_t bytes) {
+  if (ctx->ahead_open || !ctx->ahead_stream) return false;
+  bool ok = hipStreamWaitEvent(ctx->ahead_stream, ctx->ahead_free, 0) == hipSuccess;
+  const char* a = static_cast<const char*>(cloud);
+  for (auto& u : ctx->uploads) {
+    if (!ok) break;
+    if (a + bytes <= u.dst || u.dst + u.bytes <= a) continue;
+    ok = hipStreamWaitEvent(ctx->ahead_stream, u.done, 0) == hipSuccess;
+  }
+  if (!ok) {
+    (void)hipGetLastError();
+    return false;
+  }
+  ctx->ahead_open = true;
+  return true;
+}
+
+void octl_ahead_join(octl_ctx* ctx) {
+  if (!ctx->ahead_open) return;
+  ctx->ahead_open = false;
+  if (hipEventRecord(ctx->ahead_done, ctx->ahead_stream) != hipSuccess ||
+      hipStreamWaitEvent(ctx->stream, ctx->ahead_done, 0) != hipSuccess) {
+    (void)hipGetLastError();
+    (void)hipStreamSynchronize(ctx->ahead_stream);
+    ctx->ahead_mark_valid = false;
+  }
+}
+
+void octl_ahead_build_end(octl_ctx* ctx, const octl_forest* f, bool ok, int64_t n_points) {
+  octl_ahead_join(ctx);
+  ctx->ahead_mark_valid = ctx->ahead_mark_pending = false;
+  if (!ok || ctx->opt.no_build_ahead || n_points < octl_ahead_min_points(ctx)) return;
+  ctx->ahead_forest = f;
+  ctx->ahead_mark = g_octl_enqueues.load(std::memory_order_relaxed);
+  ctx->ahead_allowed = 0;
+  ctx->ahead_mark_pending = true;
+}
+
+void octl_ahead_arm(octl_ctx* ctx) {
+  ctx->ahead_mark_pending = false;
+  if (g_octl_enqueues.load(std::memory_order_relaxed) != ctx->ahead_mark || !octl_ctx_ahead_stream(ctx)) return;
+  if (hipEventRecord(ctx->ahead_free, ctx->stream) != hipSuccess) {
+    (void)hipGetLastError();
+    return;
+  }
+  ctx->ahead_mark_valid = true;
+}
+
+int octl_ahead_status_acquire(octl_ctx* ctx, int64_t tiles, uint64_t** status, uint32_t* epoch) {
+  if (!ctx->ahead_open || tiles > OCTL_AHEAD_TILES)
+    return octl_set_error(ctx, OCTL_E_STATE, "ahead stream: no front is open, or a look-back chain of %lld tiles",
+                          (long long)tiles);
+  if (ctx->ahead_epoch >= (1u << 30) - 1) {
+    HIP_TRY(ctx, hipMemsetAsync(ctx->ahead_status.p, 0, (size_t)OCTL_AHEAD_TILES * 8, ctx->ahead_stream));
+    ctx->ahead_epoch = 0;
+  }
+  *epoch = ++ctx->ahead_epoch;
+  *status = ctx->ahead_status.as<uint64_t>();
+  return OCTL_OK;
+}
+
 int octl_ctx_cus(octl_ctx* ctx) {
   if (ctx->cus <= 0) {
     hipDeviceProp_t prop;
@@ -261,11 +364,11 @@
 }
 }
 
-int octl_copy_from_pinned(octl_ctx* ctx, void* dst_dev, const void* src_pinned, size_t bytes) {
+int octl_copy_from_pinned(octl_ctx* ctx, void* dst_dev, const void* src_pinned, size_t bytes, hipStream_t on) {
   const size_t n = bytes / 8;
   if (n == 0) return OCTL_OK;
   const unsigned grid = (unsigned)std::min<size_t>(64, (n + 255) / 256);
-  OCTL_LAUNCH(k_copy_u64, dim3(grid), dim3(256), 0, ctx->stream, static_cast<const uint64_t*>(src_pinned),
+  OCTL_LAUNCH(k_copy_u64, dim3(grid), dim3(256), 0, on ? on : ctx->stream, static_cast<const uint64_t*>(src_pinned),
                      static_cast<uint64_t*>(dst_dev), n);
   HIP_TRY(ctx, hipGetLastError());
   return OCTL_OK;
@@ -394,6 +497,7 @@
   devbuf_free(ctx->ls_buf);
   devbuf_free(ctx->rs_counters);
   devbuf_free(ctx->scan_status);
+  devbuf_free(ctx->ahead_status);
   devbuf_free(ctx->small);
   devbuf_free(ctx->routed_xyz);
   devbuf_free(ctx->routed_gidx);
@@ -408,6 +512,12 @@
     if (ctx->self_gate) (void)hipEventDestroy(ctx->self_gate);
     if (ctx->self_done) (void)hipEventDestroy(ctx->self_done);
   }
+  if (ctx->ahead_stream) {
+    (void)hipStreamSynchronize(ctx->ahead_stream);
+    (void)hipStreamDestroy(ctx->ahead_stream);
+    (void)hipEventDestroy(ctx->ahead_free);
+    (void)hipEventDestroy(ctx->ahead_done);
+  }
   if (ctx->copy_stream) {
     (void)hipStreamSynchronize(ctx->copy_stream);
     (void)hipStreamDestroy(ctx->copy_stream);
@@ -450,6 +560,7 @@
     HIP_TRY(ctx, hipEventCreateWithFlags(&ctx->copy_gate, hipEventDisableTiming));
   }
   if (bytes == 0) return OCTL_OK;
+  AheadAllow allow(ctx);
   HIP_TRY(ctx, hipEventRecord(ctx->copy_gate, ctx->stream));
   HIP_TRY(ctx, hipStreamWaitEvent(ctx->copy_stream, ctx->copy_gate, 0));
   HIP_TRY(ctx, hipMemcpyAsync(dptr, src, (size_t)bytes, hipMemcpyHostToDevice, ctx->copy_stream));
diff --git a/octreelib_amd/csrc/mask.hip b/octreelib_amd/csrc/mask.hip
--- a/octreelib_amd/csrc/mask.hip
+++ b/octreelib_amd/csrc/mask.hip
@@ -531,6 +531,7 @@
   if (!f) return OCTL_E_INVALID;
   OCTL_TRY(forest_settle(f));
   if (!f->built) return octl_set_error(f->ctx, OCTL_E_STATE, "apply_mask before build");
+  AheadAllow allow(f->ctx);
   OCTL_TRY(ensure_mask(f));
   return apply_device_mask(f, n_alive);
 }
@@ -539,6 +540,7 @@
   if (!f) return OCTL_E_INVALID;
   OCTL_TRY(forest_settle(f));
   if (!f->built) return octl_set_error(f->ctx, OCTL_E_STATE, "apply_mask before build");
+  AheadAllow allow(f->ctx);
   OCTL_TRY(ensure_mask(f));
   return apply_device_mask(f, nullptr, true);
 }
diff --git a/octreelib_amd/csrc/order.hip b/octreelib_amd/csrc/order.hip
--- a/octreelib_amd/csrc/order.hip
+++ b/octreelib_amd/csrc/order.hip
@@ -303,38 +303,9 @@
   return OCTL_OK;
 }
 
-static int ransac_all_impl(octl_forest* f, int32_t poses_per_batch, const int32_t* e0, int32_t n_e0,
-                           const double* hypotheses, int32_t H, int32_t k, double threshold,
-                           bool* mask_fresh);
-
-extern "C" int octl_forest_ransac_all(octl_forest* f, int32_t poses_per_batch, const int32_t* e0,
-                                      int32_t n_e0, const double* hypotheses, int32_t H, int32_t k,
-                                      double threshold) {
-  if (!f || !hypotheses) return OCTL_E_INVALID;
-  OCTL_TRY(forest_settle(f));
-  bool mask_fresh = false;
-  const int rc = ransac_all_impl(f, poses_per_batch, e0, n_e0, hypotheses, H, k, threshold, &mask_fresh);
-  if (mask_fresh) f->mask_valid = (rc == OCTL_OK);
-  return rc;
-}
-
-static int ransac_all_impl(octl_forest* f, int32_t poses_per_batch, const int32_t* e0, int32_t n_e0,
-                           const double* hypotheses, int32_t H, int32_t k, double threshold,
-                           bool* mask_fresh) {
-  octl_ctx* ctx = f->ctx;
-  if (!f->built) return octl_set_error(ctx, OCTL_E_STATE, "ransac before build");
-  if (poses_per_batch < 1) return octl_set_error(ctx, OCTL_E_INVALID, "poses_per_batch < 1");
-  if (H < 1 || H > 1024 || k < 1) return octl_set_error(ctx, OCTL_E_INVALID, "bad H or k");
-  OCTL_TRY(ransac_check_table(ctx, hypotheses, H, k));
-  const int n_poses = (int)f->pose_off.size() - 1;
-  if (e0 && n_e0 != n_poses) return octl_set_error(ctx, OCTL_E_INVALID, "e0 size mismatch");
-  HIP_TRY(ctx, hipSetDevice(ctx->device));
+static int ransac_table_upload(octl_ctx* ctx, const double* hypotheses, int32_t H, int32_t k) {
+  AheadAllow allow(ctx);
   hipStream_t st = ctx->stream;
-  if (!f->mask_valid) {
-    OCTL_TRY(devbuf_reserve(ctx, f->mask, (size_t)std::max<int64_t>(f->n_ord, 1)));
-    *mask_fresh = true;
-  }
-  if (f->n_blocks == 0) return OCTL_OK;
   const size_t hyp_cap_before = ctx->hyp_dev.cap;
   OCTL_TRY(devbuf_reserve(ctx, ctx->hyp_dev, (size_t)H * k * 8));
   const bool same_table = hyp_cap_before == ctx->hyp_dev.cap && ctx->hyp_host.size() == (size_t)H * k &&
@@ -351,6 +322,41 @@
     HIP_TRY(ctx, hipStreamSynchronize(st));
   }
   if (!same_table) ctx->hyp_host.assign(hypotheses, hypotheses + (size_t)H * k);
+  return OCTL_OK;
+}
+
+static int ransac_all_impl(octl_forest* f, int32_t poses_per_batch, const int32_t* e0, int32_t n_e0,
+                           const double* hypotheses, int32_t H, int32_t k, double threshold,
+                           bool* mask_fresh);
+
+extern "C" int octl_forest_ransac_all(octl_forest* f, int32_t poses_per_batch, const int32_t* e0,
+                                      int32_t n_e0, const double* hypotheses, int32_t H, int32_t k,
+                                      double threshold) {
+  if (!f || !hypotheses) return OCTL_E_INVALID;
+  OCTL_TRY(forest_settle(f));
+  bool mask_fresh = false;
+  const int rc = ransac_all_impl(f, poses_per_batch, e0, n_e0, hypotheses, H, k, threshold, &mask_fresh);
+  if (mask_fresh) f->mask_valid = (rc == OCTL_OK);
+  return rc;
+}
+
+static int ransac_all_impl(octl_forest* f, int32_t poses_per_batch, const int32_t* e0, int32_t n_e0,
+                           const double* hypotheses, int32_t H, int32_t k, double threshold,
+                           bool* mask_fresh) {
+  octl_ctx* ctx = f->ctx;
+  if (!f->built) return octl_set_error(ctx, OCTL_E_STATE, "ransac before build");
+  if (poses_per_batch < 1) return octl_set_error(ctx, OCTL_E_INVALID, "poses_per_batch < 1");
+  if (H < 1 || H > 1024 || k < 1) return octl_set_error(ctx, OCTL_E_INVALID, "bad H or k");
+  OCTL_TRY(ransac_check_table(ctx, hypotheses, H, k));
+  const int n_poses = (int)f->pose_off.size() - 1;
+  if (e0 && n_e0 != n_poses) return octl_set_error(ctx, OCTL_E_INVALID, "e0 size mismatch");
+  HIP_TRY(ctx, hipSetDevice(ctx->device));
+  if (!f->mask_valid) {
+    OCTL_TRY(devbuf_reserve(ctx, f->mask, (size_t)std::max<int64_t>(f->n_ord, 1)));
+    *mask_fresh = true;
+  }
+  if (f->n_blocks == 0) return OCTL_OK;
+  OCTL_TRY(ransac_table_upload(ctx, hypotheses, H, k));
   const bool one_batch = n_poses <= poses_per_batch;
   std::vector<uint32_t> slot_counts;
   OCTL_TRY(forest_reference_order(f, e0, slot_counts, !one_batch));
diff --git a/octreelib_amd/csrc/ransac.hip b/octreelib_amd/csrc/ransac.hip
--- a/octreelib_amd/csrc/ransac.hip
+++ b/octreelib_amd/csrc/ransac.hip
@@ -1697,6 +1697,7 @@
   if (k < 1) return octl_set_error(ctx, OCTL_E_INVALID, "initial_points_number must be positive");
   const bool any_k = k > RS_KMAX;
   if (nb >= ((int64_t)1 << 31)) return octl_set_error(ctx, OCTL_E_INVALID, "too many blocks");
+  AheadAllow allow(ctx);
   hipStream_t st = ctx->stream;
   const size_t off_d = (((size_t)nb + 8) * 4 + 31) & ~(size_t)31;
   const size_t off_s = off_d + (size_t)nb * sizeof(BlockDesc);
```
